# audeering/opensmile

Measured on AMD Instinct MI355X. Metric: MFCC frames/sec (16kHz, 25ms/10ms), higher is better.
Workload: dtype f32

## Files before the change

include/smilehip.h:

```cpp
#ifndef SMILEHIP_H
#define SMILEHIP_H

#include <stdint.h>

#ifdef __cplusplus
extern "C" {
#endif

#define SMILEHIP_VERSION 0x000100

typedef enum smilehip_status {
  SMILEHIP_OK = 0,
  SMILEHIP_ERR_INVALID = -1,
  SMILEHIP_ERR_NO_DEVICE = -2,
  SMILEHIP_ERR_HIP = -3,
  SMILEHIP_ERR_NOMEM = -4
} smilehip_status;

typedef enum smilehip_winfunc {
  SMILEHIP_WIN_RECT = 0, SMILEHIP_WIN_HANN = 1, SMILEHIP_WIN_HAMM = 2,
  SMILEHIP_WIN_GAUSS = 3, SMILEHIP_WIN_SINE = 4, SMILEHIP_WIN_TRI = 5,
  SMILEHIP_WIN_BARTLETT = 6, SMILEHIP_WIN_LANCZOS = 7
} smilehip_winfunc;

// ... 89 lines not shown
void smilehip_config_plp_0_d_a(smilehip_lld_config *c);
void smilehip_config_compare16_ab(smilehip_lld_config *c);
int smilehip_config_htk_variant(smilehip_lld_config *c, const char *name);
void smilehip_config_compare16_f0(smilehip_lld_config *c);
void smilehip_config_compare16(smilehip_lld_config *c);
void smilehip_config_is13_compare(smilehip_lld_config *c);

void smilehip_config_egemapsv02(smilehip_lld_config *c);
void smilehip_config_egemapsv01a(smilehip_lld_config *c);

int smilehip_specscale_frames(smilehip_plan *plan, const float *d_mag, int64_t ld_src, float *d_dst, int64_t ld_dst,
                              int64_t n_frames, void *stream);
int smilehip_pitchshs_frames(smilehip_plan *plan, const float *d_hps, int64_t ld_src, float *d_dst, int64_t ld_dst,
                             int64_t n_frames, void *stream);

int smilehip_batch_f0_taps(smilehip_batch *b, float *d_hps_dst, const float **d_shs, const float **d_e60);
int smilehip_batch_f0_pending(smilehip_batch *b, const int32_t **d_pending);

#define SMILEHIP_FUNC_MAX          (1u << 0)
#define SMILEHIP_FUNC_MIN          (1u << 1)
#define SMILEHIP_FUNC_RANGE        (1u << 2)
#define SMILEHIP_FUNC_MAXPOS       (1u << 3)
#define SMILEHIP_FUNC_MINPOS       (1u << 4)
#define SMILEHIP_FUNC_AMEAN        (1u << 5)
#define SMILEHIP_FUNC_MAXAMEANDIST (1u << 6)
#define SMILEHIP_FUNC_MINAMEANDIST (1u << 7)
#define SMILEHIP_FUNC_LINREGC1     (1u << 8)
#define SMILEHIP_FUNC_LINREGC2     (1u << 9)
#define SMILEHIP_FUNC_LINREGERRA   (1u << 10)
#define SMILEHIP_FUNC_LINREGERRQ   (1u << 11)
#define SMILEHIP_FUNC_VARIANCE     (1u << 12)
#define SMILEHIP_FUNC_STDDEV       (1u << 13)
#define SMILEHIP_FUNC_SKEWNESS     (1u << 14)
#define SMILEHIP_FUNC_KURTOSIS     (1u << 15)
#define SMILEHIP_FUNC_AMEAN_M      (1u << 16)
#define SMILEHIP_FUNC_ALL          0x1ffffu
uint32_t smilehip_functionals_is09_mask(void);
int smilehip_functionals_count(uint32_t mask);
int smilehip_batch_func_rows(const smilehip_batch *batch, int64_t *rows);
int smilehip_batch_functionals(smilehip_plan *plan, smilehip_batch *batch, const float *d_lld, int64_t ld_lld,
                               uint32_t mask, float *d_func, int64_t ld_func, void *stream);

int smilehip_functionals_matrix(smilehip_context *ctx, const float *d_x, int64_t ld_x, int64_t rows, int32_t cols,
                                uint32_t mask, float *d_out, void *stream);

enum {
  SMILEHIP_FAM_EXTREMES = 0, SMILEHIP_FAM_MEANS, SMILEHIP_FAM_MOMENTS, SMILEHIP_FAM_REGRESSION, SMILEHIP_FAM_PERCENTILES,
  SMILEHIP_FAM_TIMES, SMILEHIP_FAM_SEGMENTS, SMILEHIP_FAM_LPC, SMILEHIP_FAM_PEAKS2, SMILEHIP_FAM_ONSET, SMILEHIP_FAM_PEAKS, SMILEHIP_FAM_CROSSINGS, SMILEHIP_FAM_DCT,
  SMILEHIP_FAM_SAMPLES, SMILEHIP_FAM_MODULATION, SMILEHIP_FAM_COUNT
};
enum { SMILEHIP_NORM_SEGMENT = 0, SMILEHIP_NORM_SECOND = 1, SMILEHIP_NORM_FRAME = 2 };
enum { SMILEHIP_SEG_RELTH = 0, SMILEHIP_SEG_NONX = 1, SMILEHIP_SEG_EQX = 2, SMILEHIP_SEG_MRELTH = 3, SMILEHIP_SEG_ABSTH = 4,
       SMILEHIP_SEG_NARELTH = 5, SMILEHIP_SEG_NAMRELTH = 6, SMILEHIP_SEG_NAABSTH = 7, SMILEHIP_SEG_DELTA = 8,
       SMILEHIP_SEG_DELTA2 = 9, SMILEHIP_SEG_CHX = 10 };

typedef struct smilehip_func_spec {
  int32_t n_fam;
  int32_t fam[12];
  int32_t non_zero_functs;
  int32_t reserved0;
  double period;
  uint32_t ext_mask; int32_t ext_norm;
  uint32_t means_mask; int32_t means_norm;
  uint32_t mom_mask; int32_t mom_stddev_norm; int32_t mom_ratio_limit; int32_t reserved1;
  uint32_t reg_mask; int32_t reg_centroid_norm, reg_norm_coeff, reg_norm_inputs, reg_centroid_abs,
      reg_centroid_limit, reg_ratio_limit, reg_old_buggy_qerr;
  uint32_t pct_mask; int32_t pct_interp, n_pctl, n_range;
  double pctl[8]; int32_t range_a[8], range_b[8];
  uint32_t times_mask; int32_t times_norm, times_buggy_sec_norm, reserved2;
  uint32_t seg_mask; int32_t seg_norm, seg_algo, seg_max_num, seg_min_lng, seg_auto_min_lng, seg_pause_min_lng,
      seg_x_is_rel, seg_n_thresholds, seg_ravg_lng;
  float seg_x; float seg_thresholds[8]; float seg_range_rel_threshold;
  int32_t lpc_gain, lpc_coeffs, lpc_first, lpc_order;
  uint32_t pk_mask; int32_t pk_norm, pk_ratio_limit, pk_dyn_rel, pk_use_abs, reserved5;
  float pk_rel_thresh, pk_abs_thresh;
  uint32_t ons_mask; int32_t ons_norm, ons_use_abs, reserved6;
  float ons_thr_on, ons_thr_off;
  uint32_t pko_mask; int32_t pko_norm;
  uint32_t crs_mask; int32_t dct_first, dct_last, n_samples;
  double sample_pos[8];
  int32_t n_quot, quot_a[8], quot_b[8];
  int32_t n_ul, n_dl, reserved7;
  double ul[8], dl[8];
  int32_t mod_win_frames, mod_step_frames, mod_n_bins, mod_win_func, mod_remove_nz_mean, reserved8;
  double mod_min_freq, mod_max_freq;
} smilehip_func_spec;

int smilehip_funcspec_count(const smilehip_func_spec *spec);
int smilehip_funcspec_compare16(const char *instance, smilehip_func_spec *spec);
int smilehip_funcspec_is13_compare(const char *instance, smilehip_func_spec *spec);
int smilehip_funcspec_matrix(smilehip_context *ctx, const smilehip_func_spec *spec, const float *d_x, int64_t ld_x,
                             int64_t rows, int32_t cols, float *d_out, void *stream);
int smilehip_batch_funcspec(smilehip_plan *plan, smilehip_batch *batch, const smilehip_func_spec *spec,
                            const float *d_lld, int64_t ld_lld, int32_t col_first, int32_t n_cols, int32_t rows_cut,
                            const float *d_extra, int64_t ld_extra, float *d_func, int64_t ld_func, void *stream);

int smilehip_functionals_compare16_count(void);
int smilehip_batch_functionals_compare16(smilehip_plan *plan, smilehip_batch *batch, const float *d_lld, int64_t ld_lld,
                                         float *d_func, int64_t ld_func, void *stream);
int smilehip_batch_functionals_is13_compare(smilehip_plan *plan, smilehip_batch *batch, const float *d_lld, int64_t ld_lld,
                                            float *d_func, int64_t ld_func, void *stream);
int smilehip_batch_compare_b_extra(smilehip_batch *batch, const float **d_extra);

int smilehip_funcspec_egemaps(const char *instance, smilehip_func_spec *spec);
int smilehip_functionals_egemaps_count(void);
int smilehip_batch_functionals_egemaps(smilehip_plan *plan, smilehip_batch *batch, float *d_func, int64_t ld_func, void *stream);
int smilehip_batch_egemaps_taps(smilehip_batch *batch, const float **d_raw20, const float **d_lpc, const float **d_formants,
                                const float **d_pitch3, const float **d_jit4, const float **d_shim_db, const float **d_harm6,
                                const float **d_func_in, const int32_t **d_pending, int64_t *h_frame_off60);

int  smilehip_alloc(smilehip_context *ctx, uint64_t bytes, void **d_ptr);
int  smilehip_free(smilehip_context *ctx, void *d_ptr);
int  smilehip_copy_to_device(smilehip_context *ctx, void *d_dst, const void *h_src, uint64_t bytes, void *stream);
int  smilehip_copy_to_host(smilehip_context *ctx, void *h_dst, const void *d_src, uint64_t bytes, void *stream);
int  smilehip_stream_synchronize(smilehip_context *ctx, void *stream);
int  smilehip_alloc_cache(smilehip_context *ctx, uint64_t bytes);
int  smilehip_stream_create(smilehip_context *ctx, void **stream);
int  smilehip_stream_destroy(smilehip_context *ctx, void *stream);
int  smilehip_event_create(smilehip_context *ctx, void **event);
int  smilehip_event_destroy(smilehip_context *ctx, void *event);
int  smilehip_event_record(smilehip_context *ctx, void *event, void *stream);
int  smilehip_stream_wait_event(smilehip_context *ctx, void *stream, void *event);
int  smilehip_copy_to_device_2d(smilehip_context *ctx, void *d_dst, uint64_t d_pitch, const void *h_src, uint64_t h_pitch,
                                uint64_t width_bytes, uint64_t rows, void *stream);
int  smilehip_copy_to_host_2d(smilehip_context *ctx, void *h_dst, uint64_t h_pitch, const void *d_src, uint64_t d_pitch,
                              uint64_t width_bytes, uint64_t rows, void *stream);
int  smilehip_alloc_host(smilehip_context *ctx, uint64_t bytes, void **h_ptr);
int  smilehip_free_host(smilehip_context *ctx, void *h_ptr);
int  smilehip_host_register(smilehip_context *ctx, void *h_ptr, uint64_t bytes);
int  smilehip_host_unregister(smilehip_context *ctx, void *h_ptr);
int  smilehip_htk_rows_be(smilehip_context *ctx, const float *d_src, int64_t n, void *d_dst, void *stream);

void smilehip_config_mfcc12_0_d_a(smilehip_lld_config *c);

int  smilehip_plan_create(smilehip_context *ctx, const smilehip_lld_config *cfg, smilehip_plan **plan);
int  smilehip_plan_create_host_only(const smilehip_lld_config *cfg, smilehip_plan **plan);
void smilehip_plan_destroy(smilehip_plan *plan);
int  smilehip_plan_geometry(const smilehip_plan *plan, smilehip_geometry *g);
int64_t smilehip_num_frames(const smilehip_plan *plan, int64_t n_samples);
double  smilehip_frame_time(const smilehip_plan *plan, int64_t t);
double  smilehip_row_time(const smilehip_plan *plan, int64_t n_frames, int64_t row);
int64_t smilehip_plan_get_window(const smilehip_plan *plan, float *out, int64_t cap);
int64_t smilehip_plan_get_mel_weights(const smilehip_plan *plan, float *out, int64_t cap);
int64_t smilehip_plan_get_mel_chanmap(const smilehip_plan *plan, int32_t *out, int64_t cap);
int64_t smilehip_plan_get_dct(const smilehip_plan *plan, float *out, int64_t cap);
int64_t smilehip_plan_get_lifter(const smilehip_plan *plan, float *out, int64_t cap);

int  smilehip_batch_create(smilehip_plan *plan, const int64_t *h_sample_offsets, int32_t n_utt,
                           smilehip_batch **batch);
void smilehip_batch_destroy(smilehip_batch *batch);
int64_t smilehip_batch_total_frames(const smilehip_batch *batch);
int64_t smilehip_batch_total_rows(const smilehip_batch *batch);
int  smilehip_batch_delta_fused(const smilehip_batch *batch);
int  smilehip_batch_frame_offsets(const smilehip_batch *batch, int64_t *h_row_offsets);

int  smilehip_mfcc_run(smilehip_plan *plan, smilehip_batch *batch, const int16_t *d_pcm,
                       float *d_out, int64_t ld_out, void *stream);

int  smilehip_lld_run(smilehip_plan *plan, smilehip_batch *batch, const int16_t *d_pcm,
                      float *d_out, int64_t ld_out, void *stream);
int  smilehip_lld_run_f32(smilehip_plan *plan, smilehip_batch *batch, const float *d_pcm_f32,
                          float *d_out, int64_t ld_out, void *stream);
int  smilehip_lld_run_host(smilehip_plan *plan, smilehip_batch *batch, const int16_t *h_pcm,
                           int64_t n_samples, float *h_out);

int  smilehip_mfcc_run_host(smilehip_plan *plan, smilehip_batch *batch, const int16_t *h_pcm,
                            int64_t n_samples, float *h_out);

int  smilehip_plan_set_timing(smilehip_plan *plan, int enable);
int  smilehip_plan_last_timing(smilehip_plan *plan, float *ms_main, float *ms_delta);
int  smilehip_kernel_timing(int enable);
int64_t smilehip_kernel_timing_report(char *buf, int64_t buflen);


int smilehip_pcm16_to_float(smilehip_context *ctx, const int16_t *d_pcm, int64_t n, float *d_out, void *stream);
int smilehip_pcm_convert(smilehip_context *ctx, const void *d_raw, int n_bps, int n_bits, int n_chan, int mono_mixdown,
                         int64_t n, float *d_out, void *stream);
int smilehip_pcm_convert_float(smilehip_context *ctx, const float *d_raw, int n_chan, int mono_mixdown, int64_t n, float *d_out,
                               void *stream);
int smilehip_irfft_frames(smilehip_plan *plan, const float *d_src, int64_t ld_src, float *d_dst, int64_t ld_dst, int64_t n_frames,
                          void *stream);
#define SMILEHIP_MAGPHASE_MAGNITUDE 1
#define SMILEHIP_MAGPHASE_PHASE 2
#define SMILEHIP_MAGPHASE_NORMALISE 4
#define SMILEHIP_MAGPHASE_POWER 8
#define SMILEHIP_MAGPHASE_DBPSD 16
int smilehip_fftmagphase_frames(smilehip_context *ctx, const float *d_src, int64_t ld_src, int64_t nfft, int32_t flags, float dbp_norm,
                                float min_dbp, float *d_dst, int64_t ld_dst, int64_t n_frames, void *stream);
int smilehip_melspec_table_frames(smilehip_context *ctx, const float *d_src, int64_t ld_src, int64_t K, int32_t n_bands, int32_t dense,
                                  const float *d_coef, const int32_t *d_chanmap, int32_t n_lo, int32_t n_hi, int32_t use_power,
                                  float htk_scale, float *d_dst, int64_t ld_dst, int64_t n_frames, void *stream);
int smilehip_melspec_inverse_table_frames(smilehip_context *ctx, const float *d_src, int64_t ld_src, int32_t n_src, int64_t K,
                                          const float *d_coef, const int32_t *d_chanmap, int32_t n_lo, int32_t n_hi, int32_t use_power,
                                          float htk_div, float *d_dst, int64_t ld_dst, int64_t n_frames, void *stream);
int smilehip_pitchacf_zcr_frames(smilehip_context *ctx, const float *d_src, int64_t ld_src, int64_t n, int64_t n_frames, double fs_sec,
                                 double max_pitch, double *d_zcr, void *stream);
#define SMILEHIP_MZCR_ZCR 1
#define SMILEHIP_MZCR_MCR 2
#define SMILEHIP_MZCR_AMAX 4
#define SMILEHIP_MZCR_MAXMIN 8
#define SMILEHIP_MZCR_DC 16
int smilehip_mzcr_frames(smilehip_context *ctx, const float *d_src, int64_t ld_src, int64_t N, int64_t n_frames, int32_t flags,
                         float *d_dst, int64_t ld_dst, void *stream);
int smilehip_frame_rows(smilehip_context *ctx, const float *d_samples, int64_t frame_size, int64_t frame_step, int64_t n_frames,
                        float *d_dst, int64_t ld_dst, void *stream);
int smilehip_preemphasis_frames(smilehip_context *ctx, const float *d_src, int64_t ld_src, float *d_dst,
                                int64_t ld_dst, int64_t n_frames, int64_t N, float k, int de, void *stream);
int smilehip_window_frames(smilehip_plan *plan, const float *d_src, int64_t ld_src, float *d_dst,
                           int64_t ld_dst, int64_t n_frames, void *stream);
int smilehip_rfft_frames(smilehip_plan *plan, const float *d_src, int64_t ld_src, float *d_dst,
                         int64_t ld_dst, int64_t n_frames, void *stream);
int smilehip_fftmag_frames(smilehip_plan *plan, const float *d_src, int64_t ld_src, float *d_dst,
                           int64_t ld_dst, int64_t n_frames, void *stream);
int smilehip_melspec_frames(smilehip_plan *plan, const float *d_src, int64_t ld_src, float *d_dst,
                            int64_t ld_dst, int64_t n_frames, void *stream);
int smilehip_mfcc_frames(smilehip_plan *plan, const float *d_src, int64_t ld_src, float *d_dst,
                         int64_t ld_dst, int64_t n_frames, void *stream);
int  smilehip_mfcc_inverse_frames(smilehip_plan *plan, const float *d_src, int64_t ld_src, float *d_dst, int64_t ld_dst,
                                  int64_t n_frames, int do_log, void *stream);
int smilehip_sumsq_frames(smilehip_context *ctx, const float *d_src, int64_t ld_src, int64_t N, int64_t n_frames,
                          double *d_out, void *stream);
int smilehip_zcr_count_frames(smilehip_context *ctx, const float *d_src, int64_t ld_src, int64_t N, int64_t n_frames,
                              int32_t *d_out, void *stream);
int smilehip_acf_frames(smilehip_plan *plan, const float *d_src, int64_t ld_src, float *d_dst, int64_t ld_dst, int64_t n_out,
                        int64_t n_frames, int use_power, int cepstrum, int norm_output, int abs_cepstrum, void *stream);
int smilehip_pitchacf_frames(smilehip_context *ctx, const float *d_src, int64_t ld_src, int64_t n, int64_t n_frames,
                             double fs_sec, double max_pitch, double *d_voicing, int32_t *d_max_idx, void *stream);
int smilehip_pitchacf_contour_step(smilehip_context *ctx, const double *d_voicing, const int32_t *d_max_idx, double t_samp,
                                   double voicing_cutoff, float *d_state, float *d_out4, void *stream);
int smilehip_pitchacf_contour_frames(smilehip_context *ctx, const double *d_voicing, const int32_t *d_max_idx, double t_samp,
                                     double voicing_cutoff, float *d_state, float *d_out4, int64_t n_frames, void *stream);
int smilehip_spectral_frames(smilehip_plan *plan, const float *d_mag, int64_t ld_src, float *d_state, int first,
                             float *d_dst, int64_t ld_dst, int64_t n_frames, void *stream);
typedef struct smilehip_spectral_opts {
  int32_t n_bands;
  int32_t band_lo[16], band_hi[16];
  int32_t n_rolloff;
  double  rolloff[16];
  int32_t flux, centroid, max_pos, min_pos, entropy, variance, skewness, kurtosis, slope, sharpness, harmonicity;
  int32_t flatness, log_flatness;
  int32_t spec_diff, spec_pos_diff, flux_centroid, flux_at_flux_centroid, standard_deviation;
  int32_t n_slopes;
  int32_t slope_lo[16], slope_hi[16];
} smilehip_spectral_opts;
typedef struct smilehip_spectral_op smilehip_spectral_op;
int smilehip_spectral_opts_count(const smilehip_spectral_opts *opts);
int smilehip_spectral_op_create(smilehip_context *ctx, const smilehip_spectral_opts *opts, int64_t K, double frame_size_sec,
                                smilehip_spectral_op **op);
int smilehip_spectral_op_n_out(const smilehip_spectral_op *op);
int smilehip_spectral_op_frames(smilehip_spectral_op *op, const float *d_mag, int64_t ld_src, float *d_state, int first,
                                float *d_dst, int64_t ld_dst, int64_t n_frames, void *stream);
int smilehip_spectral_op_destroy(smilehip_spectral_op *op);
typedef struct smilehip_spectral_axis_opts {
  smilehip_spectral_opts base;
  int32_t square_input, use_log_spectrum, norm_band_energies, alpha_ratio, hammarberg_index, old_slope_scale, buggy_roll_off, tonality;
  double  spec_floor;
  int32_t freq_lo, freq_hi;
  int32_t frq_scale, reserved;
  double  frq_scale_param;
} smilehip_spectral_axis_opts;
typedef struct smilehip_spectral_axis_op smilehip_spectral_axis_op;
int smilehip_spectral_axis_opts_count(const smilehip_spectral_axis_opts *opts);
int smilehip_spectral_axis_tables(const smilehip_spectral_axis_opts *opts, int64_t K, double frame_size_sec, const double *frq,
                                  int64_t n_scale, int32_t *geo, double *edges, double *sums, double *sharp);
int smilehip_spectral_axis_op_create(smilehip_context *ctx, const smilehip_spectral_axis_opts *opts, int64_t K, double frame_size_sec,
                                     const double *frq, int64_t n_scale, smilehip_spectral_axis_op **op);
int smilehip_spectral_axis_op_n_out(const smilehip_spectral_axis_op *op);
int smilehip_spectral_axis_op_frames(smilehip_spectral_axis_op *op, const float *d_src, int64_t ld_src, float *d_state, int first,
                                     float *d_dst, int64_t ld_dst, int64_t n_frames, void *stream);
int smilehip_spectral_axis_op_destroy(smilehip_spectral_axis_op *op);
int smilehip_plp_audspec_frames(smilehip_context *ctx, const float *d_mel, int64_t ld_src, int n_bands, const float *d_eql,
                                float melfloor, float compression, int new_rasta, const float *rasta_coef, float *d_state,
                                float *d_dst, int64_t ld_dst, int64_t n_frames, void *stream);
int smilehip_plp_cc_frames(smilehip_context *ctx, const float *d_mel, int64_t ld_src, int n_bands, const float *d_eql,
                           float melfloor, float compression, int lp_order, const float *d_cos, const float *d_sin,
                           float *d_dst, int64_t ld_dst, int64_t n_frames, void *stream);
int smilehip_plp_stage_frames(smilehip_context *ctx, const float *d_mel, int64_t ld_src, int n_bands, const float *d_eql,
                              float melfloor, float compression, int lp_order, const float *d_cos, int out_stage,
                              float *d_dst, int64_t ld_dst, int64_t n_frames, void *stream);
int smilehip_window_op_row(smilehip_context *ctx, const float *d_x, float *d_y, int64_t n_t, int kind, int W, void *stream);
int smilehip_window_op_row_ex(smilehip_context *ctx, const float *d_x, float *d_y, int64_t n_t, int kind, int W, float *d_norm_io,
                              void *stream);
#define SMILEHIP_DELTA_RELATIVE 1
#define SMILEHIP_DELTA_HALFWAVE 2
#define SMILEHIP_DELTA_ABS 4
#define SMILEHIP_DELTA_SEGMENTS 8
int smilehip_delta_op_row(smilehip_context *ctx, const float *d_x, float *d_y, int64_t n_t, int W, int flags, float *d_norm_io,
                          void *stream);
int smilehip_window_op_block(smilehip_context *ctx, const float *d_x, int64_t ld_x, float *d_y, int64_t ld_y, int64_t n_t,
                             int32_t n_cols, int op, int W, int delta_flags, void *stream);
int smilehip_delta_segments_block(smilehip_context *ctx, const float *d_x, int64_t ld_x, float *d_y, int64_t ld_y, int64_t n_ticks,
                                  int32_t tick_frames, int32_t n_cols, int W, int delta_flags, float *d_norm_io, void *stream);
int smilehip_spectral_gemaps_frames(smilehip_plan *plan, const float *d_mag, int64_t ld_src, float *d_state, int first,
                                    float *d_dst, int64_t ld_dst, int64_t n_frames, void *stream);
int smilehip_specresample_frames(smilehip_plan *plan, const float *d_spec, int64_t ld_src, float *d_dst, int64_t ld_dst,
                                 int64_t n_frames, void *stream);
int smilehip_lpc_frames(smilehip_plan *plan, const float *d_x, int64_t ld_src, float *d_lpc, int64_t ld_dst, int64_t n_frames,
                        void *stream);
int smilehip_specresample_geometry(int64_t n_in, double fs_sec, double last_fs_sec, double base_period, double target_fs,
                                   int64_t *n_out, int64_t *k_max, double *nd);
int smilehip_specresample_tables(int64_t n_in, int64_t n_out, int64_t k_max, double nd, float *cos_table, float *sin_table);
int smilehip_specresample_table_frames(smilehip_context *ctx, const float *d_src, int64_t ld_src, int64_t n_in, int64_t n_out,
                                       int64_t k_max, const float *d_cos, const float *d_sin, float *d_dst, int64_t ld_dst,
                                       int64_t n_frames, void *stream);
int smilehip_lpc_acf_frames(smilehip_context *ctx, const float *d_x, int64_t ld_src, int64_t n, int32_t p, float *d_lpc,
                            int64_t ld_dst, int64_t n_frames, void *stream);
// ... 77 lines not shown
```

opensmile_amd/capi.py:

```python
import ctypes as C
import os

import numpy as np

HERE = os.path.dirname(os.path.abspath(__file__))
LIB_PATH = os.path.join(HERE, "libsmilehip.so")

WINFUNC = {"rec": 0, "rect": 0, "han": 1, "hann": 1, "ham": 2, "hamming": 2, "gau": 3,
           "gauss": 3, "sin": 4, "sine": 4, "tri": 5, "bar": 6, "bartlett": 6, "lac": 7}


class SmileHipError(RuntimeError):
    pass


class LldConfig(C.Structure):
    _fields_ = [
        ("struct_size", C.c_uint32),
        ("sample_rate", C.c_double), ("frame_size_sec", C.c_double), ("frame_step_sec", C.c_double),
        ("preemph", C.c_int32), ("preemph_k", C.c_float), ("preemph_de", C.c_int32),
        ("win_func", C.c_int32), ("win_sigma", C.c_double), ("win_gain", C.c_double),
        ("win_offset", C.c_double),
        ("zero_pad_symmetric", C.c_int32),
        ("n_bands", C.c_int32), ("lofreq", C.c_float), ("hifreq", C.c_float),
        ("use_power", C.c_int32), ("mel_htk_compatible", C.c_int32),
        ("first_mfcc", C.c_int32), ("last_mfcc", C.c_int32), ("cep_lifter", C.c_float),
        ("mfcc_htk_compatible", C.c_int32), ("melfloor", C.c_float),
        ("n_delta", C.c_int32), ("delta_win", C.c_int32),
        ("chain_kind", C.c_int32), ("plp_lp_order", C.c_int32), ("plp_compression", C.c_float), ("pitch_max", C.c_double), ("voicing_cutoff", C.c_double),
        ("sma_win", C.c_int32),
        ("force_frame_size", C.c_int64), ("force_fft_frame_size_sec", C.c_double),
        ("stage_mask", C.c_uint32),
        ("pitch_min", C.c_double), ("shs_n_harmonics", C.c_int32), ("shs_compression", C.c_float),
        ("f0_min_energy", C.c_float), ("append_log_energy", C.c_int32), ("cms", C.c_int32), ("jitter_broken_thresh", C.c_int32),
        ("vit_buffer_len", C.c_int32), ("jitter_search_range", C.c_double), ("formant_max_freq", C.c_double), ("specscale_min_f", C.c_double), ("shs_n_candidates", C.c_int32), ("shs_old_peak_algo", C.c_int32),
        ("spectral_band_lo", C.c_int32 * 2), ("spectral_band_hi", C.c_int32 * 2), ("specscale_off", C.c_int32),
    ]


STAGE_WINDOW, STAGE_FFT, STAGE_MEL, STAGE_MFCC, STAGE_ALL = 1, 2, 4, 8, 15


class FuncSpec(C.Structure):
    _fields_ = [
        ("n_fam", C.c_int32), ("fam", C.c_int32 * 12), ("non_zero_functs", C.c_int32), ("reserved0", C.c_int32),
        ("period", C.c_double),
        ("ext_mask", C.c_uint32), ("ext_norm", C.c_int32),
        ("means_mask", C.c_uint32), ("means_norm", C.c_int32),
        ("mom_mask", C.c_uint32), ("mom_stddev_norm", C.c_int32), ("mom_ratio_limit", C.c_int32), ("reserved1", C.c_int32),
        ("reg_mask", C.c_uint32), ("reg_centroid_norm", C.c_int32), ("reg_norm_coeff", C.c_int32),
        ("reg_norm_inputs", C.c_int32), ("reg_centroid_abs", C.c_int32), ("reg_centroid_limit", C.c_int32),
        ("reg_ratio_limit", C.c_int32), ("reg_old_buggy_qerr", C.c_int32),
        ("pct_mask", C.c_uint32), ("pct_interp", C.c_int32), ("n_pctl", C.c_int32), ("n_range", C.c_int32),
        ("pctl", C.c_double * 8), ("range_a", C.c_int32 * 8), ("range_b", C.c_int32 * 8),
        ("times_mask", C.c_uint32), ("times_norm", C.c_int32), ("times_buggy_sec_norm", C.c_int32), ("reserved2", C.c_int32),
        ("seg_mask", C.c_uint32), ("seg_norm", C.c_int32), ("seg_algo", C.c_int32), ("seg_max_num", C.c_int32),
        ("seg_min_lng", C.c_int32), ("seg_auto_min_lng", C.c_int32), ("seg_pause_min_lng", C.c_int32),
        ("seg_x_is_rel", C.c_int32), ("seg_n_thresholds", C.c_int32), ("seg_ravg_lng", C.c_int32),
        ("seg_x", C.c_float), ("seg_thresholds", C.c_float * 8), ("seg_range_rel_threshold", C.c_float),
        ("lpc_gain", C.c_int32), ("lpc_coeffs", C.c_int32), ("lpc_first", C.c_int32), ("lpc_order", C.c_int32),
        ("pk_mask", C.c_uint32), ("pk_norm", C.c_int32), ("pk_ratio_limit", C.c_int32), ("pk_dyn_rel", C.c_int32),
        ("pk_use_abs", C.c_int32), ("reserved5", C.c_int32),
        ("pk_rel_thresh", C.c_float), ("pk_abs_thresh", C.c_float),
        ("ons_mask", C.c_uint32), ("ons_norm", C.c_int32), ("ons_use_abs", C.c_int32), ("reserved6", C.c_int32),
        ("ons_thr_on", C.c_float), ("ons_thr_off", C.c_float),
        ("pko_mask", C.c_uint32), ("pko_norm", C.c_int32),
        ("crs_mask", C.c_uint32), ("dct_first", C.c_int32), ("dct_last", C.c_int32), ("n_samples", C.c_int32),
        ("sample_pos", C.c_double * 8),
        ("n_quot", C.c_int32), ("quot_a", C.c_int32 * 8), ("quot_b", C.c_int32 * 8),
        ("n_ul", C.c_int32), ("n_dl", C.c_int32), ("reserved7", C.c_int32),
        ("ul", C.c_double * 8), ("dl", C.c_double * 8),
        ("mod_win_frames", C.c_int32), ("mod_step_frames", C.c_int32), ("mod_n_bins", C.c_int32), ("mod_win_func", C.c_int32),
        ("mod_remove_nz_mean", C.c_int32), ("reserved8", C.c_int32),
        ("mod_min_freq", C.c_double), ("mod_max_freq", C.c_double),
    ]


class SpectralOpts(C.Structure):
    _fields_ = [("n_bands", C.c_int32), ("band_lo", C.c_int32 * 16), ("band_hi", C.c_int32 * 16), ("n_rolloff", C.c_int32),
                ("rolloff", C.c_double * 16)] + [(k, C.c_int32) for k in ("flux", "centroid", "max_pos", "min_pos", "entropy", "variance",
                                                                          "skewness", "kurtosis", "slope", "sharpness", "harmonicity", "flatness",
                                                                          "log_flatness", "spec_diff", "spec_pos_diff", "flux_centroid",
                                                                          "flux_at_flux_centroid", "standard_deviation", "n_slopes")] + [
                   ("slope_lo", C.c_int32 * 16), ("slope_hi", C.c_int32 * 16)]


def spectral_opts(bands, rolloff=(0.25, 0.5, 0.75, 0.9), slopes=(), **flags):
    o = SpectralOpts()
    o.n_slopes = len(slopes)
    for i, (a, b) in enumerate(slopes):
        o.slope_lo[i], o.slope_hi[i] = a, b
    o.n_bands = len(bands)
    for i, (a, b) in enumerate(bands):
        o.band_lo[i], o.band_hi[i] = a, b
    o.n_rolloff = len(rolloff)
    for i, r in enumerate(rolloff):
        o.rolloff[i] = r
    for k, v in flags.items():
        setattr(o, k, int(v))
    return o


class SpectralAxisOpts(C.Structure):
    _fields_ = [("base", SpectralOpts)] + [(k, C.c_int32) for k in ("square_input", "use_log_spectrum", "norm_band_energies", "alpha_ratio",
                                                                     "hammarberg_index", "old_slope_scale", "buggy_roll_off", "tonality")] + [
                   ("spec_floor", C.c_double), ("freq_lo", C.c_int32), ("freq_hi", C.c_int32), ("frq_scale", C.c_int32),
                   ("reserved", C.c_int32), ("frq_scale_param", C.c_double)]


def spectral_axis_opts(bands=(), rolloff=(), slopes=(), square_input=1, use_log_spectrum=0, norm_band_energies=0, alpha_ratio=0,
                       hammarberg_index=0, old_slope_scale=1, buggy_roll_off=0, tonality=0, spec_floor=0.0000001, freq_range=(0, 0),
                       frq_scale=0, frq_scale_param=0.0, **flags):
    o = SpectralAxisOpts()
    o.base = spectral_opts(bands, rolloff, slopes, **flags)
    o.square_input, o.use_log_spectrum, o.norm_band_energies = int(square_input), int(use_log_spectrum), int(norm_band_energies)
    o.alpha_ratio, o.hammarberg_index, o.old_slope_scale = int(alpha_ratio), int(hammarberg_index), int(old_slope_scale)
    o.buggy_roll_off, o.tonality, o.spec_floor = int(buggy_roll_off), int(tonality), float(spec_floor)
    o.freq_lo, o.freq_hi = int(freq_range[0]), int(freq_range[1])
    o.frq_scale = SPECSCALE[frq_scale] if isinstance(frq_scale, str) else int(frq_scale)
    o.frq_scale_param = float(frq_scale_param)
    return o


class SpecScaleOpts(C.Structure):
    _fields_ = [("scale", C.c_int32), ("param", C.c_double), ("min_f", C.c_double), ("max_f", C.c_double), ("n_points_target", C.c_int32),
                ("spec_enhance", C.c_int32), ("spec_smooth", C.c_int32), ("auditory_weighting", C.c_int32)]


SPECSCALE = {"lin": 0, "log": 1, "bark": 2, "mel": 3, "sem": 4, "bao": 7}


def specscale_opts(scale, param=0.0, min_f=25.0, max_f=-1.0, n_points_target=0, spec_enhance=0, spec_smooth=0, auditory_weighting=0):
    o = SpecScaleOpts()
    o.scale = SPECSCALE[scale] if isinstance(scale, str) else int(scale)
    o.param, o.min_f, o.max_f, o.n_points_target = float(param), float(min_f), float(max_f), int(n_points_target)
    o.spec_enhance, o.spec_smooth, o.auditory_weighting = int(spec_enhance), int(spec_smooth), int(auditory_weighting)
    return o


class Geometry(C.Structure):
    _fields_ = [("frame_size", C.c_int64), ("frame_step", C.c_int64), ("fft_size", C.c_int64),
                ("n_bins", C.c_int64), ("n_static", C.c_int32), ("n_out", C.c_int32),
                ("frame_period", C.c_double), ("fft_frame_size_sec", C.c_double)]


_vp, _i32, _i64, _f32, _dbl = C.c_void_p, C.c_int32, C.c_int64, C.c_float, C.c_double
SYMBOLS = {
    "smilehip_version": (C.c_int, []),
    "smilehip_last_error": (C.c_char_p, []),
    "smilehip_init": (C.c_int, [C.c_int, C.POINTER(_vp)]),
    "smilehip_shutdown": (None, [_vp]),
    "smilehip_device_name": (C.c_int, [_vp, C.c_char_p, C.c_int]),
    "smilehip_config_is09_lld": (None, [C.POINTER(LldConfig)]),
    "smilehip_config_compare16_ab": (None, [C.POINTER(LldConfig)]),
    "smilehip_config_compare16_f0": (None, [C.POINTER(LldConfig)]),
    "smilehip_config_htk_variant": (C.c_int, [C.POINTER(LldConfig), C.c_char_p]),
    "smilehip_config_compare16": (None, [C.POINTER(LldConfig)]),
    "smilehip_specscale_frames": (C.c_int, [_vp, _vp, _i64, _vp, _i64, _i64, _vp]),
    "smilehip_pitchshs_frames": (C.c_int, [_vp, _vp, _i64, _vp, _i64, _i64, _vp]),
    "smilehip_batch_f0_taps": (C.c_int, [_vp, _vp, C.POINTER(_vp), C.POINTER(_vp)]),
    "smilehip_config_plp_0_d_a": (None, [C.POINTER(LldConfig)]),
    "smilehip_batch_total_rows": (_i64, [_vp]),
    "smilehip_batch_delta_fused": (C.c_int, [_vp]),
    "smilehip_functionals_is09_mask": (C.c_uint32, []),
    "smilehip_functionals_count": (C.c_int, [C.c_uint32]),
    "smilehip_functionals_matrix": (C.c_int, [_vp, _vp, _i64, _i64, C.c_int32, C.c_uint32, _vp, _vp]),
    "smilehip_batch_func_rows": (C.c_int, [_vp, _vp]),
    "smilehip_batch_functionals": (C.c_int, [_vp, _vp, _vp, _i64, C.c_uint32, _vp, _i64, _vp]),
    "smilehip_functionals_compare16_count": (C.c_int, []),
    "smilehip_batch_functionals_compare16": (C.c_int, [_vp, _vp, _vp, _i64, _vp, _i64, _vp]),
    "smilehip_batch_compare_b_extra": (C.c_int, [_vp, _vp]),
    "smilehip_funcspec_count": (C.c_int, [_vp]),
    "smilehip_funcspec_compare16": (C.c_int, [C.c_char_p, _vp]),
    "smilehip_funcspec_is13_compare": (C.c_int, [C.c_char_p, _vp]),
    "smilehip_batch_functionals_is13_compare": (C.c_int, [_vp, _vp, _vp, _i64, _vp, _i64, _vp]),
    "smilehip_config_is13_compare": (None, [_vp]),
    "smilehip_config_egemapsv02": (None, [C.POINTER(LldConfig)]),
    "smilehip_config_egemapsv01a": (None, [C.POINTER(LldConfig)]),
    "smilehip_funcspec_egemaps": (C.c_int, [C.c_char_p, _vp]),
    "smilehip_functionals_egemaps_count": (C.c_int, []),
    "smilehip_batch_functionals_egemaps": (C.c_int, [_vp, _vp, _vp, _i64, _vp]),
    "smilehip_batch_egemaps_taps": (C.c_int, [_vp] + [C.POINTER(_vp)] * 9 + [_vp]),
    "smilehip_spectral_gemaps_frames": (C.c_int, [_vp, _vp, _i64, _vp, C.c_int, _vp, _i64, _i64, _vp]),
    "smilehip_specresample_frames": (C.c_int, [_vp, _vp, _i64, _vp, _i64, _i64, _vp]),
    "smilehip_lpc_frames": (C.c_int, [_vp, _vp, _i64, _vp, _i64, _i64, _vp]),
    "smilehip_formantlpc_frames": (C.c_int, [_vp, _vp, _i64, _vp, _i64, _i64, _vp]),
    "smilehip_formantlpc_rows": (C.c_int, [_vp, _vp, _i64, _vp, _i64, _i64, _vp, _i32, _vp]),
    "smilehip_harmonics_frames": (C.c_int, [_vp, _vp, _vp, _i64, _vp, _i64, _vp, _i64, _i64, _vp]),
    "smilehip_valbased_select_frames": (C.c_int, [_vp, _vp, _i64, _i64, _i64, _i32, _f32, _i32, _i32, _i32, _i32, _f32, _vp, _i64, _vp, _vp]),
    "smilehip_jitter_stream_create": (C.c_int, [_vp, _dbl, _i64, _i64, _dbl, _dbl, _i32, C.POINTER(_vp)]),
    "smilehip_jitter_stream_push": (C.c_int, [_vp, _f32, _vp, _i64, _i64, _vp, _vp, _vp]),
    "smilehip_jitter_stream_set_time_offset": (C.c_int, [_vp, _i64]),
    "smilehip_jitter_stream_destroy": (C.c_int, [_vp]),
    "smilehip_viterbi_stream_create": (C.c_int, [_vp, _i32, _f32, _vp, C.POINTER(_vp)]),
    "smilehip_viterbi_stream_push": (C.c_int, [_vp, _vp, _vp, _vp, _vp, _vp, _i32]),
    "smilehip_viterbi_stream_set_candidates": (C.c_int, [_vp, _i32]),
    "smilehip_viterbi_stream_flush": (C.c_int, [_vp, _vp, _vp, _vp, _i32]),
    "smilehip_viterbi_stream_destroy": (C.c_int, [_vp]),
    "smilehip_funcspec_matrix": (C.c_int, [_vp, _vp, _vp, _i64, _i64, C.c_int32, _vp, _vp]),
    "smilehip_batch_funcspec": (C.c_int, [_vp, _vp, _vp, _vp, _i64, C.c_int32, C.c_int32, C.c_int32, _vp, _i64, _vp, _i64, _vp]),
    "smilehip_lld_run": (C.c_int, [_vp, _vp, _vp, _vp, _i64, _vp]),
    "smilehip_lld_run_f32": (C.c_int, [_vp, _vp, _vp, _vp, _i64, _vp]),
    "smilehip_lld_run_host": (C.c_int, [_vp, _vp, _vp, _i64, _vp]),
    "smilehip_alloc": (C.c_int, [_vp, C.c_uint64, C.POINTER(_vp)]),
    "smilehip_free": (C.c_int, [_vp, _vp]),
    "smilehip_alloc_host": (C.c_int, [_vp, C.c_uint64, C.POINTER(_vp)]),
    "smilehip_free_host": (C.c_int, [_vp, _vp]),
    "smilehip_htk_rows_be": (C.c_int, [_vp, _vp, _i64, _vp, _vp]),
    "smilehip_copy_to_device": (C.c_int, [_vp, _vp, _vp, C.c_uint64, _vp]),
    "smilehip_copy_to_host": (C.c_int, [_vp, _vp, _vp, C.c_uint64, _vp]),
    "smilehip_alloc_cache": (C.c_int, [_vp, C.c_uint64]),
    "smilehip_stream_create": (C.c_int, [_vp, C.POINTER(_vp)]),
    "smilehip_stream_destroy": (C.c_int, [_vp, _vp]),
    "smilehip_event_create": (C.c_int, [_vp, C.POINTER(_vp)]),
    "smilehip_event_destroy": (C.c_int, [_vp, _vp]),
    "smilehip_event_record": (C.c_int, [_vp, _vp, _vp]),
    "smilehip_stream_wait_event": (C.c_int, [_vp, _vp, _vp]),
    "smilehip_kernel_timing": (C.c_int, [C.c_int]),
    "smilehip_kernel_timing_report": (C.c_int64, [_vp, _i64]),
    "smilehip_copy_to_device_2d": (C.c_int, [_vp, _vp, C.c_uint64, _vp, C.c_uint64, C.c_uint64, C.c_uint64, _vp]),
    "smilehip_copy_to_host_2d": (C.c_int, [_vp, _vp, C.c_uint64, _vp, C.c_uint64, C.c_uint64, C.c_uint64, _vp]),
    "smilehip_host_register": (C.c_int, [_vp, _vp, C.c_uint64]),
    "smilehip_host_unregister": (C.c_int, [_vp, _vp]),
    "smilehip_frame_rows": (C.c_int, [_vp, _vp, _i64, _i64, _i64, _vp, _i64, _vp]),
    "smilehip_window_op_block": (C.c_int, [_vp, _vp, _i64, _vp, _i64, _i64, _i32, C.c_int, C.c_int, C.c_int, _vp]),
    "smilehip_delta_segments_block": (C.c_int, [_vp, _vp, _i64, _vp, _i64, _i64, _i32, _i32, C.c_int, C.c_int, _vp, _vp]),
    "smilehip_pitchacf_contour_frames": (C.c_int, [_vp, _vp, _vp, _dbl, _dbl, _vp, _vp, _i64, _vp]),
    "smilehip_viterbi_stream_push_frames": (C.c_int, [_vp, _vp, _vp, _i64, _i32, _vp, _vp, _vp, _i32]),
    "smilehip_jitter_stream_push_frames": (C.c_int, [_vp, _vp, _i32, _vp, _i64, _i64, _vp, _vp, _vp]),
    "smilehip_stream_synchronize": (C.c_int, [_vp, _vp]),
    "smilehip_config_mfcc12_0_d_a": (None, [C.POINTER(LldConfig)]),
    "smilehip_plan_create": (C.c_int, [_vp, C.POINTER(LldConfig), C.POINTER(_vp)]),
    "smilehip_plan_create_host_only": (C.c_int, [C.POINTER(LldConfig), C.POINTER(_vp)]),
    "smilehip_plan_destroy": (None, [_vp]),
    "smilehip_plan_geometry": (C.c_int, [_vp, C.POINTER(Geometry)]),
    "smilehip_num_frames": (_i64, [_vp, _i64]),
    "smilehip_frame_time": (_dbl, [_vp, _i64]),
    "smilehip_row_time": (_dbl, [_vp, _i64, _i64]),
    "smilehip_plan_get_window": (_i64, [_vp, _vp, _i64]),
    "smilehip_plan_get_mel_weights": (_i64, [_vp, _vp, _i64]),
    "smilehip_plan_get_mel_chanmap": (_i64, [_vp, _vp, _i64]),
    "smilehip_plan_get_dct": (_i64, [_vp, _vp, _i64]),
    "smilehip_plan_get_lifter": (_i64, [_vp, _vp, _i64]),
    "smilehip_batch_f0_pending": (C.c_int, [_vp, _vp]),
    "smilehip_batch_create": (C.c_int, [_vp, _vp, _i32, C.POINTER(_vp)]),
    "smilehip_batch_destroy": (None, [_vp]),
    "smilehip_batch_total_frames": (_i64, [_vp]),
    "smilehip_batch_frame_offsets": (C.c_int, [_vp, _vp]),
    "smilehip_mfcc_run": (C.c_int, [_vp, _vp, _vp, _vp, _i64, _vp]),
    "smilehip_mfcc_run_host": (C.c_int, [_vp, _vp, _vp, _i64, _vp]),
    "smilehip_plan_set_timing": (C.c_int, [_vp, C.c_int]),
    "smilehip_plan_last_timing": (C.c_int, [_vp, C.POINTER(_f32), C.POINTER(_f32)]),
    "smilehip_sumsq_frames": (C.c_int, [_vp, _vp, _i64, _i64, _i64, _vp, _vp]),
    "smilehip_zcr_count_frames": (C.c_int, [_vp, _vp, _i64, _i64, _i64, _vp, _vp]),
    "smilehip_acf_frames": (C.c_int, [_vp, _vp, _i64, _vp, _i64, _i64, _i64, C.c_int, C.c_int, C.c_int, C.c_int, _vp]),
    "smilehip_pitchacf_frames": (C.c_int, [_vp, _vp, _i64, _i64, _i64, _dbl, _dbl, _vp, _vp, _vp]),
    "smilehip_pitchacf_contour_step": (C.c_int, [_vp, _vp, _vp, _dbl, _dbl, _vp, _vp, _vp]),
    "smilehip_spectral_frames": (C.c_int, [_vp, _vp, _i64, _vp, C.c_int, _vp, _i64, _i64, _vp]),
    "smilehip_spectral_opts_count": (C.c_int, [_vp]),
    "smilehip_spectral_op_create": (C.c_int, [_vp, _vp, _i64, C.c_double, _vp]),
    "smilehip_spectral_op_n_out": (C.c_int, [_vp]),
    "smilehip_spectral_op_frames": (C.c_int, [_vp, _vp, _i64, _vp, C.c_int, _vp, _i64, _i64, _vp]),
    "smilehip_spectral_op_destroy": (C.c_int, [_vp]),
    "smilehip_spectral_axis_opts_count": (C.c_int, [_vp]),
    "smilehip_spectral_axis_tables": (C.c_int, [_vp, _i64, C.c_double, _vp, _i64, _vp, _vp, _vp, _vp]),
    "smilehip_spectral_axis_op_create": (C.c_int, [_vp, _vp, _i64, C.c_double, _vp, _i64, _vp]),
    "smilehip_spectral_axis_op_n_out": (C.c_int, [_vp]),
    "smilehip_spectral_axis_op_frames": (C.c_int, [_vp, _vp, _i64, _vp, C.c_int, _vp, _i64, _i64, _vp]),
    "smilehip_spectral_axis_op_destroy": (C.c_int, [_vp]),
    "smilehip_plp_audspec_frames": (C.c_int, [_vp, _vp, _i64, C.c_int, _vp, C.c_float, C.c_float, C.c_int, _vp, _vp, _vp, _i64,
                                             _i64, _vp]),
    "smilehip_plp_cc_frames": (C.c_int, [_vp, _vp, _i64, C.c_int, _vp, C.c_float, C.c_float, C.c_int, _vp, _vp, _vp, _i64, _i64,
                                        _vp]),
    "smilehip_mfcc_inverse_frames": (C.c_int, [_vp, _vp, _i64, _vp, _i64, _i64, C.c_int, _vp]),
    "smilehip_plp_stage_frames": (C.c_int, [_vp, _vp, _i64, C.c_int, _vp, C.c_float, C.c_float, C.c_int, _vp, C.c_int, _vp, _i64, _i64,
                                           _vp]),
    "smilehip_window_op_row": (C.c_int, [_vp, _vp, _vp, _i64, C.c_int, C.c_int, _vp]),
    "smilehip_window_op_row_ex": (C.c_int, [_vp, _vp, _vp, _i64, C.c_int, C.c_int, _vp, _vp]),
    "smilehip_delta_op_row": (C.c_int, [_vp, _vp, _vp, _i64, C.c_int, C.c_int, _vp, _vp]),
    "smilehip_pcm_convert": (C.c_int, [_vp, _vp, C.c_int, C.c_int, C.c_int, C.c_int, _i64, _vp, _vp]),
    "smilehip_pcm_convert_float": (C.c_int, [_vp, _vp, C.c_int, C.c_int, _i64, _vp, _vp]),
    "smilehip_pcm16_to_float": (C.c_int, [_vp, _vp, _i64, _vp, _vp]),
    "smilehip_preemphasis_frames": (C.c_int, [_vp, _vp, _i64, _vp, _i64, _i64, _i64, _f32, C.c_int, _vp]),
    "smilehip_window_frames": (C.c_int, [_vp, _vp, _i64, _vp, _i64, _i64, _vp]),
    "smilehip_rfft_frames": (C.c_int, [_vp, _vp, _i64, _vp, _i64, _i64, _vp]),
    "smilehip_fftmag_frames": (C.c_int, [_vp, _vp, _i64, _vp, _i64, _i64, _vp]),
    "smilehip_irfft_frames": (C.c_int, [_vp, _vp, _i64, _vp, _i64, _i64, _vp]),
    "smilehip_fftmagphase_frames": (C.c_int, [_vp, _vp, _i64, _i64, _i32, _f32, _f32, _vp, _i64, _i64, _vp]),
    "smilehip_melspec_table_frames": (C.c_int, [_vp, _vp, _i64, _i64, _i32, _i32, _vp, _vp, _i32, _i32, _i32, _f32, _vp, _i64, _i64, _vp]),
    "smilehip_melspec_inverse_table_frames": (C.c_int, [_vp, _vp, _i64, _i32, _i64, _vp, _vp, _i32, _i32, _i32, _f32, _vp, _i64, _i64, _vp]),
    "smilehip_pitchacf_zcr_frames": (C.c_int, [_vp, _vp, _i64, _i64, _i64, _dbl, _dbl, _vp, _vp]),
    "smilehip_mzcr_frames": (C.c_int, [_vp, _vp, _i64, _i64, _i64, _i32, _vp, _i64, _vp]),
    "smilehip_melspec_frames": (C.c_int, [_vp, _vp, _i64, _vp, _i64, _i64, _vp]),
    "smilehip_mfcc_frames": (C.c_int, [_vp, _vp, _i64, _vp, _i64, _i64, _vp]),
    "smilehip_delta_chain": (C.c_int, [_vp, _vp, _vp, _i64, _i32, _i32, _i32, _vp]),
    "smilehip_specresample_geometry": (C.c_int, [_i64, _dbl, _dbl, _dbl, _dbl, _vp, _vp, _vp]),
    "smilehip_specresample_tables": (C.c_int, [_i64, _i64, _i64, _dbl, _vp, _vp]),
    "smilehip_specresample_table_frames": (C.c_int, [_vp, _vp, _i64, _i64, _i64, _i64, _vp, _vp, _vp, _i64, _i64, _vp]),
    "smilehip_lpc_acf_frames": (C.c_int, [_vp, _vp, _i64, _i64, _i32, _vp, _i64, _i64, _vp]),
    "smilehip_lsp_frames": (C.c_int, [_vp, _vp, _i64, _i32, _vp, _i64, _i64, _vp]),
    "smilehip_intensity_frames": (C.c_int, [_vp, _vp, _i64, _i64, _i32, _vp, _i64, _i64, _vp]),
    "smilehip_vecop_frames": (C.c_int, [_vp, _i32, _f32, _f32, _vp, _i64, _i32, _vp, _i64, _i64, _vp]),
    "smilehip_pitch_smoother_rows": (C.c_int, [_vp, _i32, _f32, _i32, _i32, _i32, _vp, _i64, _vp, _i32, _i64, _vp, _i32, _vp, _i64, _vp, _vp]),
    "smilehip_specscale_op_create": (C.c_int, [_vp, _vp, _i64, _dbl, _vp]),
    "smilehip_specscale_op_n_out": (C.c_int, [_vp]),
    "smilehip_specscale_op_frames": (C.c_int, [_vp, _vp, _i64, _vp, _i64, _i64, _vp]),
    "smilehip_specscale_op_destroy": (C.c_int, [_vp]),
    "smilehip_specscale_tables": (C.c_int, [_vp, _i64, _dbl, _vp, _vp, _vp, _vp]),
}

_lib = None


def load():
    global _lib
    if _lib is None:
# ... 170 lines not shown
    s = FuncSpec()
    _check(load().smilehip_funcspec_is13_compare(instance.encode(), C.byref(s)))
    return s


def compare16_f0_config():
    c = LldConfig()
    load().smilehip_config_compare16_f0(C.byref(c))
    return c


def funcspec_compare16(instance):
    s = FuncSpec()
    _check(load().smilehip_funcspec_compare16(instance.encode(), C.byref(s)))
    return s


def funcspec_count(spec):
    n = load().smilehip_funcspec_count(C.byref(spec))
    if n < 0:
        _check(n)
    return n


def funcspec_matrix_host(ctx, spec, x):
    L = load()
    x = np.ascontiguousarray(x, dtype=np.float32)
    rows, cols = x.shape
    per = funcspec_count(spec)
    out = np.zeros((cols, per), np.float32)
    d_x, d_out = _vp(), _vp()
    _check(L.smilehip_alloc(ctx._h, max(x.nbytes, 4), C.byref(d_x)))
    _check(L.smilehip_alloc(ctx._h, max(out.nbytes, 4), C.byref(d_out)))
    try:
        _check(L.smilehip_copy_to_device(ctx._h, d_x, x.ctypes.data, x.nbytes, None))
        _check(L.smilehip_funcspec_matrix(ctx._h, C.byref(spec), d_x, cols, rows, cols, d_out, None))
        _check(L.smilehip_stream_synchronize(ctx._h, None))
        _check(L.smilehip_copy_to_host(ctx._h, out.ctypes.data, d_out, out.nbytes, None))
    finally:
        L.smilehip_free(ctx._h, d_x)
        L.smilehip_free(ctx._h, d_out)
    return out


def is09_lld_config():
    c = LldConfig()
    load().smilehip_config_is09_lld(C.byref(c))
    return c


def mfcc12_0_d_a_config():
    c = LldConfig()
    load().smilehip_config_mfcc12_0_d_a(C.byref(c))
    return c


class Context:
    def __init__(self, device=0):
        self._h = _vp()
        _check(load().smilehip_init(device, C.byref(self._h)))

    def name(self):
        buf = C.create_string_buffer(256)
        _check(load().smilehip_device_name(self._h, buf, 256))
        return buf.value.decode()

    def close(self):
        if self._h:
            load().smilehip_shutdown(self._h)
            self._h = _vp()

    def __del__(self):
        try:
            self.close()
        except Exception:
            pass


class Plan:

    def __init__(self, ctx, cfg=None):
        self.ctx = ctx
        self.cfg = cfg if cfg is not None else mfcc12_0_d_a_config()
        self._h = _vp()
        if ctx is None:
            _check(load().smilehip_plan_create_host_only(C.byref(self.cfg), C.byref(self._h)))
        else:
            _check(load().smilehip_plan_create(ctx._h, C.byref(self.cfg), C.byref(self._h)))
        g = Geometry()
        _check(load().smilehip_plan_geometry(self._h, C.byref(g)))
        self.geometry = g

    def num_frames(self, n_samples):
        return int(load().smilehip_num_frames(self._h, n_samples))

    def frame_time(self, t):
        return float(load().smilehip_frame_time(self._h, t))

    def _table(self, fn, dtype):
        n = fn(self._h, None, 0)
        a = np.zeros(n, dtype)
        fn(self._h, a.ctypes.data, n)
        return a

    def window(self):
        return self._table(load().smilehip_plan_get_window, np.float32)

    def mel_weights(self):
        return self._table(load().smilehip_plan_get_mel_weights, np.float32)

    def mel_chanmap(self):
        return self._table(load().smilehip_plan_get_mel_chanmap, np.int32)

    def dct(self):
        g = self.geometry
        return self._table(load().smilehip_plan_get_dct, np.float32).reshape(g.n_static, self.cfg.n_bands)

    def lifter(self):
        return self._table(load().smilehip_plan_get_lifter, np.float32)

    def set_timing(self, on=True):
        _check(load().smilehip_plan_set_timing(self._h, 1 if on else 0))

    def last_timing(self):
        a, b = _f32(), _f32()
        _check(load().smilehip_plan_last_timing(self._h, C.byref(a), C.byref(b)))
        return a.value, b.value

    def close(self):
        if self._h:
            load().smilehip_plan_destroy(self._h)
            self._h = _vp()

    def __del__(self):
        try:
            self.close()
        except Exception:
            pass


class Batch:

    def __init__(self, plan, sample_offsets):
        self.plan = plan
        off = np.ascontiguousarray(sample_offsets, dtype=np.int64)
        assert off.ndim == 1 and len(off) >= 1
        self.n_utt = len(off) - 1
        self.sample_offsets = off
        self._h = _vp()
        _check(load().smilehip_batch_create(plan._h, off.ctypes.data, self.n_utt, C.byref(self._h)))
        self.total_frames = int(load().smilehip_batch_total_frames(self._h))
        self.total_rows = int(load().smilehip_batch_total_rows(self._h))
        self.delta_fused = bool(load().smilehip_batch_delta_fused(self._h))
        fo = np.zeros(self.n_utt + 1, np.int64)
        _check(load().smilehip_batch_frame_offsets(self._h, fo.ctypes.data))
        self.frame_offsets = fo

    def run_device(self, d_pcm_ptr, d_out_ptr, ld_out, stream=None):
        _check(load().smilehip_lld_run(self.plan._h, self._h, d_pcm_ptr, d_out_ptr, ld_out, stream))

    def run_device_f32(self, d_pcm_f32_ptr, d_out_ptr, ld_out, stream=None):
        _check(load().smilehip_lld_run_f32(self.plan._h, self._h, d_pcm_f32_ptr, d_out_ptr, ld_out, stream))

    def run_host(self, pcm):
        pcm = np.ascontiguousarray(pcm, dtype=np.int16)
        out = np.zeros((self.total_rows, self.plan.geometry.n_out), np.float32)
        _check(load().smilehip_lld_run_host(self.plan._h, self._h, pcm.ctypes.data, len(pcm),
                                            out.ctypes.data))
        return out

    def f0_run_host_taps(self, pcm):
        L = load()
        ctx = self.plan.ctx._h
        pcm = np.ascontiguousarray(pcm, dtype=np.int16)
        K = self.plan.geometry.n_bins
        nf = self.total_frames
        out = np.zeros((self.total_rows, self.plan.geometry.n_out), np.float32)
        taps = {"hps": np.zeros((nf, K), np.float32), "shs": np.zeros((nf, 21), np.float32), "e60": np.zeros((nf, 1), np.float32)}
        d_pcm, d_out, d_hps = _vp(), _vp(), _vp()
        _check(L.smilehip_alloc(ctx, max(pcm.nbytes, 4), C.byref(d_pcm)))
        _check(L.smilehip_alloc(ctx, max(out.nbytes, 4), C.byref(d_out)))
        _check(L.smilehip_alloc(ctx, max(taps["hps"].nbytes, 4), C.byref(d_hps)))
        try:
            if pcm.nbytes:
                _check(L.smilehip_copy_to_device(ctx, d_pcm, pcm.ctypes.data, pcm.nbytes, None))
            d_shs, d_e60 = _vp(), _vp()
            _check(L.smilehip_batch_f0_taps(self._h, d_hps, C.byref(d_shs), C.byref(d_e60)))
            _check(L.smilehip_lld_run(self.plan._h, self._h, d_pcm, d_out, self.plan.geometry.n_out, None))
            _check(L.smilehip_stream_synchronize(ctx, None))
            if out.nbytes:
                _check(L.smilehip_copy_to_host(ctx, out.ctypes.data, d_out, out.nbytes, None))
            if nf:
                _check(L.smilehip_copy_to_host(ctx, taps["hps"].ctypes.data, d_hps, taps["hps"].nbytes, None))
                _check(L.smilehip_copy_to_host(ctx, taps["shs"].ctypes.data, d_shs, taps["shs"].nbytes, None))
                _check(L.smilehip_copy_to_host(ctx, taps["e60"].ctypes.data, d_e60, taps["e60"].nbytes, None))
            _check(L.smilehip_batch_f0_taps(self._h, None, None, None))
        finally:
            L.smilehip_free(ctx, d_pcm)
            L.smilehip_free(ctx, d_out)
            L.smilehip_free(ctx, d_hps)
        return out, taps

    def func_rows(self):
        r = np.zeros(self.n_utt, np.int64)
        _check(load().smilehip_batch_func_rows(self._h, r.ctypes.data))
        return r

    def functionals_device(self, d_lld_ptr, ld_lld, d_func_ptr, ld_func, mask=None, stream=None):
        L = load()
        mask = L.smilehip_functionals_is09_mask() if mask is None else mask
        _check(L.smilehip_batch_functionals(self.plan._h, self._h, d_lld_ptr, ld_lld, mask, d_func_ptr, ld_func, stream))

    def functionals_host(self, lld, mask=None):
        L = load()
        mask = L.smilehip_functionals_is09_mask() if mask is None else mask
        per = L.smilehip_functionals_count(mask)
        n_out = self.plan.geometry.n_out
        lld = np.ascontiguousarray(lld, dtype=np.float32)
        assert lld.shape == (self.total_rows, n_out)
        out = np.zeros((self.n_utt, n_out * per), np.float32)
        ctx = self.plan.ctx._h
        d_lld, d_out = _vp(), _vp()
        _check(L.smilehip_alloc(ctx, max(lld.nbytes, 4), C.byref(d_lld)))
        _check(L.smilehip_alloc(ctx, max(out.nbytes, 4), C.byref(d_out)))
        try:
            if lld.nbytes:
                _check(L.smilehip_copy_to_device(ctx, d_lld, lld.ctypes.data, lld.nbytes, None))
            _check(L.smilehip_batch_functionals(self.plan._h, self._h, d_lld, n_out, mask, d_out, n_out * per, None))
            _check(L.smilehip_stream_synchronize(ctx, None))
            if out.nbytes:
                _check(L.smilehip_copy_to_host(ctx, out.ctypes.data, d_out, out.nbytes, None))
        finally:
            L.smilehip_free(ctx, d_lld)
            L.smilehip_free(ctx, d_out)
        return out

    def run_host_with_functionals16(self, pcm):
        L = load()
        pcm = np.ascontiguousarray(pcm, dtype=np.int16)
        n_out = self.plan.geometry.n_out
        nf = L.smilehip_functionals_compare16_count()
        lld = np.zeros((self.total_rows, n_out), np.float32)
        func = np.zeros((self.n_utt, nf), np.float32)
        ex = np.zeros((self.n_utt, 110), np.float32)
        ctx = self.plan.ctx._h
        d_pcm, d_lld, d_func = _vp(), _vp(), _vp()
        _check(L.smilehip_alloc(ctx, max(pcm.nbytes, 4), C.byref(d_pcm)))
        _check(L.smilehip_alloc(ctx, max(lld.nbytes, 4), C.byref(d_lld)))
        _check(L.smilehip_alloc(ctx, max(func.nbytes, 4), C.byref(d_func)))
        try:
            if pcm.nbytes:
                _check(L.smilehip_copy_to_device(ctx, d_pcm, pcm.ctypes.data, pcm.nbytes, None))
            _check(L.smilehip_lld_run(self.plan._h, self._h, d_pcm, d_lld, n_out, None))
            fn = L.smilehip_batch_functionals_is13_compare if self.plan.cfg.jitter_broken_thresh else L.smilehip_batch_functionals_compare16
            _check(fn(self.plan._h, self._h, d_lld, n_out, d_func, nf, None))
            _check(L.smilehip_stream_synchronize(ctx, None))
            if lld.nbytes:
                _check(L.smilehip_copy_to_host(ctx, lld.ctypes.data, d_lld, lld.nbytes, None))
            if func.nbytes:
                _check(L.smilehip_copy_to_host(ctx, func.ctypes.data, d_func, func.nbytes, None))
            d_ex = _vp()
            _check(L.smilehip_batch_compare_b_extra(self._h, C.byref(d_ex)))
            if ex.nbytes:
                _check(L.smilehip_copy_to_host(ctx, ex.ctypes.data, d_ex, ex.nbytes, None))
        finally:
            L.smilehip_free(ctx, d_pcm)
            L.smilehip_free(ctx, d_lld)
            L.smilehip_free(ctx, d_func)
        return lld, func, ex

    def run_host_egemaps(self, pcm, functionals=True, taps=False):
        L = load()
        pcm = np.ascontiguousarray(pcm, dtype=np.int16)
        n_out = self.plan.geometry.n_out
        lld = np.zeros((self.total_rows, n_out), np.float32)
        func = np.zeros((self.n_utt, 88), np.float32) if functionals else None
        ctx = self.plan.ctx._h
        d_pcm, d_lld, d_func = _vp(), _vp(), _vp()
        _check(L.smilehip_alloc(ctx, max(pcm.nbytes, 4), C.byref(d_pcm)))
        _check(L.smilehip_alloc(ctx, max(lld.nbytes, 4), C.byref(d_lld)))
        _check(L.smilehip_alloc(ctx, max(self.n_utt * 88 * 4, 4), C.byref(d_func)))
        out_taps = {}
        try:
            if pcm.nbytes:
                _check(L.smilehip_copy_to_device(ctx, d_pcm, pcm.ctypes.data, pcm.nbytes, None))
            _check(L.smilehip_lld_run(self.plan._h, self._h, d_pcm, d_lld, n_out, None))
            if functionals:
                _check(L.smilehip_batch_functionals_egemaps(self.plan._h, self._h, d_func, 88, None))
            _check(L.smilehip_stream_synchronize(ctx, None))
            if lld.nbytes:
                _check(L.smilehip_copy_to_host(ctx, lld.ctypes.data, d_lld, lld.nbytes, None))
            if functionals and func.nbytes:
                _check(L.smilehip_copy_to_host(ctx, func.ctypes.data, d_func, func.nbytes, None))
            if taps:
                ptrs = [_vp() for _ in range(9)]
                fo60 = np.zeros(self.n_utt + 1, np.int64)
                _check(L.smilehip_batch_egemaps_taps(self._h, *[C.byref(q) for q in ptrs], fo60.ctypes.data))
                nf, nf60 = self.total_frames, int(fo60[-1])
                T20 = np.diff(self.frame_offsets_frames())
                T60 = np.diff(fo60)
                nfin = int(np.where(T60 >= 1, T20 + 1, 0).sum())
                shapes = [("raw20", (nf, 12)), ("lpc", (nf, 12)), ("formants", (nf, 10)), ("pitch3", (nf60, 3)), ("jit4", (nf60, 4)),
                          ("shim_db", (nf60, 1)), ("harm6", (nf60, 6)), ("func_in", (nfin, 36))]
                for (name, shp), q in zip(shapes, ptrs):
                    a = np.zeros(shp, np.float32)
                    if a.nbytes:
# ... 179 lines not shown
```

opensmile_amd/csrc/batch_layout.hpp:

```cpp
#pragma once
#include <algorithm>
#include <cmath>
#include <cstdint>
#include <map>
#include <vector>

#include "../../include/smilehip.h"
#include "lld_tile_rec.hpp"

namespace smilehip {

struct BatchLayoutSpec {
  int chain_kind = SMILEHIP_CHAIN_MFCC;
  int64_t N = 0, H = 0;
  double period = 0.0;
  int row_extra = 0;
  bool fused_delta_eligible = false;
  int64_t fast_slots = 8;
  int64_t tile_frames = 0;
  int64_t dtile_rows = 0;
  int short_T = 0;
  int jitter_chunk = 0;
  int run_frames_override = 0;
};

struct BatchLayout {
  std::vector<int64_t> samp_off, frame_off, row_off;
  std::vector<int64_t> fin_off;
  std::vector<int32_t> short_utts;
  bool all_even = true;
  int64_t total_frames = 0, total_rows = 0;
  std::vector<int32_t> tile_utt, tile_t0, dtile_utt, dtile_t0;
  std::vector<TileRec> tile_rec;
  std::vector<int32_t> run_utt, run_t0;
  int32_t run_frames = 8;
  std::vector<FTileRec> ftiles;
  std::vector<int32_t> jit_utt, jit_t0;
  std::vector<int32_t> frame_utt;
};

constexpr int kRunFramesMin = 8;

inline int compare_run_frames(int64_t total_frames) {
  int L = kRunFramesMin;
  while (L < 64 && total_frames / (2 * L) >= 65536) L *= 2;
  return L;
}

inline int64_t layout_num_frames(int64_t len, int64_t N, int64_t H) { return len < N ? 0 : (len - N) / H + 1; }
inline int64_t samples_60ms(double period) { return std::lround(0.060 / period); }

inline int64_t layout_rows(const BatchLayoutSpec &s, int64_t len, int64_t T) {
  const bool compare = s.chain_kind == SMILEHIP_CHAIN_COMPARE_AB || s.chain_kind == SMILEHIP_CHAIN_COMPARE;
  if (!compare && s.chain_kind != SMILEHIP_CHAIN_EGEMAPS) return T > 0 ? T + s.row_extra : 0;
  const int64_t T60 = layout_num_frames(len, samples_60ms(s.period), s.H);
  return T60 >= (compare ? 4 : 1) ? T60 + 1 : 0;
}

inline void layout_fused_tiles(const BatchLayoutSpec &s, const int64_t *h_off, int32_t n_utt, BatchLayout &out) {
  const auto parts_of = [&](int64_t T, int64_t L) { return (T + L - 1) / L; };
  int64_t bestL = 32;
  double best = 1e300;
  std::map<int64_t, int64_t> hist;
  for (int32_t u = 0; u < n_utt; ++u) {
    const int64_t T = out.frame_off[u + 1] - out.frame_off[u];
    if (T > 0) hist[T]++;
  }
  for (int64_t L = 32; L <= 2048; L += 4) {
    int64_t n = 0;
    for (const auto &h : hist) n += h.second * ((h.first <= s.short_T) ? 1 : parts_of(h.first, L));
    const double cost = double((n + s.fast_slots - 1) / s.fast_slots) * double(L / 4 + 2);
    if (cost <= best) { best = cost; bestL = L; }
  }
  for (int32_t u = 0; u < n_utt; ++u) {
    const int64_t T = out.frame_off[u + 1] - out.frame_off[u];
    if (T <= 0) continue;
    const int64_t parts = (T <= s.short_T) ? 1 : parts_of(T, bestL);
    const int64_t len = (((T + parts - 1) / parts) + 3) & ~int64_t(3);
    for (int64_t t0 = 0; t0 < T; t0 += len) {
      const int64_t t1 = std::min<int64_t>(T, t0 + len), p0 = t0 > 0 ? t0 - 4 : 0;
      FTileRec r;
      r.samp0 = h_off[u] + p0 * s.H;
      r.row0 = out.frame_off[u] + p0;
      const int64_t last = (t1 + 3) & ~int64_t(3);
      r.n_frames = (int32_t)(last - p0 + 4);
      r.live_n = (int32_t)(T - p0);
      r.e0 = (int32_t)(t0 - p0);
      r.e1 = (int32_t)(t1 - p0);
      r.lo = (int32_t)(-p0);
      r.delta_on = T > s.short_T;
      out.ftiles.push_back(r);
    }
  }
  std::stable_sort(out.ftiles.begin(), out.ftiles.end(), [](const FTileRec &a, const FTileRec &c) { return a.n_frames > c.n_frames; });
}

inline int batch_layout(const BatchLayoutSpec &s, const int64_t *h_off, int32_t n_utt, BatchLayout &out) {
  out = BatchLayout();
  out.samp_off.assign(h_off, h_off + (n_utt ? n_utt + 1 : 0));
  if (n_utt == 0) out.samp_off.assign(1, 0);
  out.frame_off.assign(size_t(n_utt) + 1, 0);
  out.row_off.assign(size_t(n_utt) + 1, 0);
  const bool compare = s.chain_kind == SMILEHIP_CHAIN_COMPARE_AB || s.chain_kind == SMILEHIP_CHAIN_COMPARE;
  const bool egemaps = s.chain_kind == SMILEHIP_CHAIN_EGEMAPS;
  if (egemaps) out.fin_off.assign(size_t(n_utt) + 1, 0);
  {
    int64_t total_T = 0;
    for (int32_t u = 0; u < n_utt; ++u) total_T += layout_num_frames(h_off[u + 1] - h_off[u], s.N, s.H);
    out.run_frames = s.run_frames_override >= 1 ? s.run_frames_override : compare_run_frames(total_T);
  }
  for (int32_t u = 0; u < n_utt; ++u) {
    const int64_t len = h_off[u + 1] - h_off[u];
    if (len < 0) return u + 1;
    const int64_t T = layout_num_frames(len, s.N, s.H);
    const int64_t rows = layout_rows(s, len, T);
    if (compare || egemaps)
      for (int64_t t0 = 0; t0 < T; t0 += out.run_frames) {
        out.run_utt.push_back(u);
        out.run_t0.push_back((int32_t)t0);
      }
    if (egemaps) out.fin_off[u + 1] = out.fin_off[u] + (rows > 0 ? T + 1 : 0);
    out.frame_off[u + 1] = out.frame_off[u] + T;
    out.row_off[u + 1] = out.row_off[u] + rows;
    if (T > 0 && T <= s.short_T) out.short_utts.push_back(u);
    if (T > 0 && (h_off[u] & 1)) out.all_even = false;
    for (int64_t t0 = 0; t0 < T; t0 += s.tile_frames) {
      out.tile_utt.push_back(u);
      out.tile_t0.push_back((int32_t)t0);
      TileRec r;
      r.samp0 = h_off[u] + t0 * s.H;
      r.row0 = out.frame_off[u] + t0;
      r.n_frames = (int32_t)std::min<int64_t>(s.tile_frames, T - t0);
      r.pad = 0;
      out.tile_rec.push_back(r);
    }
    for (int64_t t0 = 0; t0 < rows; t0 += s.dtile_rows) {
      out.dtile_utt.push_back(u);
      out.dtile_t0.push_back((int32_t)t0);
    }
  }
  out.total_frames = out.frame_off[n_utt];
  out.total_rows = out.row_off[n_utt];
  if (s.chain_kind == SMILEHIP_CHAIN_IS09 && out.total_frames > 0) {
    out.frame_utt.resize((size_t)out.total_frames);
    for (int32_t u = 0; u < n_utt; ++u) std::fill(out.frame_utt.begin() + out.frame_off[u], out.frame_utt.begin() + out.frame_off[u + 1], u);
  }
  if (s.fused_delta_eligible && out.total_frames > 0 && out.all_even)
    layout_fused_tiles(s, h_off, n_utt, out);
  if (s.chain_kind == SMILEHIP_CHAIN_COMPARE_F0) {
    int64_t maxT = 0;
    for (int32_t u = 0; u < n_utt; ++u) maxT = std::max(maxT, out.frame_off[u + 1] - out.frame_off[u]);
    for (int64_t t0 = 0; t0 < maxT; t0 += s.jitter_chunk)
      for (int32_t u = 0; u < n_utt; ++u)
        if (t0 < out.frame_off[u + 1] - out.frame_off[u]) { out.jit_utt.push_back(u); out.jit_t0.push_back((int32_t)t0); }
  }
  return 0;
}

}
```

opensmile_amd/csrc/lld_launch.hpp:

```cpp
#pragma once
#include <hip/hip_runtime.h>

#include <vector>

#include "lld_params.hpp"
#include "tables.hpp"

namespace smilehip {
inline int current_device_cus() {
  static int cache[64] = {0};
  int dev = 0;
  if (hipGetDevice(&dev) != hipSuccess) return 0;
  if (dev >= 0 && dev < 64 && __atomic_load_n(&cache[dev], __ATOMIC_RELAXED) > 0) return __atomic_load_n(&cache[dev], __ATOMIC_RELAXED);
  int n = 0;
  if (hipDeviceGetAttribute(&n, hipDeviceAttributeMultiprocessorCount, dev) != hipSuccess) return 0;
  if (dev >= 0 && dev < 64) __atomic_store_n(&cache[dev], n, __ATOMIC_RELAXED);
  return n;
}

struct Fast512Host {
  std::vector<float2> tw256, tw512, win;
  std::vector<float4> melw;
  std::vector<uint32_t> melo;
  std::vector<float> dct28;
  std::vector<int32_t> lane_bands;
  int mel_units = 0, n_slots = 0, mp = 13;
  int mel_conflict_steps = 0;
  float mel_scale = 1.0f;
  int max_blocks = 512;
  bool force_padded = false;
};
bool fast512_applicable(int Nfft, int N);
int fast512_tile_frames();
int fast512_build_host(const smilehip_lld_config &cfg, const Geometry &geo, const std::vector<float> &window,
                       const MelBank &mel, const DctTables &dct, Fast512Host &h);
hipError_t launch_mfcc512(const LldParams &P, const Fast512Tables &F, const Fast512Host &h, bool aligned, bool fused_delta, hipStream_t s);
hipError_t launch_mfcc_generic(const LldParams &P, hipStream_t s);
hipError_t launch_chain(const ChainParams &P, hipStream_t s);
hipError_t launch_log_energy(const LldParams &P, const int32_t *d_tile_utt, const int32_t *d_tile_t0, int n_tiles, float *dst,
                             int64_t ld, int col, hipStream_t s);
hipError_t launch_cms(const int64_t *d_frame_off, int n_utt, const float *x, int64_t ld_x, float *out, int64_t ld_out, int n_cols,
                      hipStream_t s);
hipError_t launch_compare(const LldParams &P, const CompareParams &Q, int n_runs, const int64_t *d_row_off,
                          int64_t total_rows, float *d_out, int64_t ld_out, int de_col, hipStream_t s);
hipError_t launch_compare_b_extra(const int64_t *d_frame_off, const int64_t *d_row_off, int n_utt, const float *rawB, float *out110,
                                  hipStream_t s);
struct F0Pipe {
  hipStream_t spec = nullptr, sweep = nullptr;
  hipEvent_t start = nullptr, spec_done[2] = {nullptr, nullptr}, sweep_done[2] = {nullptr, nullptr}, cand_done[2] = {nullptr, nullptr};
  double *ab2 = nullptr;
};
hipError_t launch_f0(const LldParams &P, const F0Params &Q, int max_blocks, float *d_out, int64_t ld_out, hipStream_t s,
                     hipEvent_t frames_done = nullptr, const F0Pipe *pipe = nullptr);
int f0_chunk_tiles();
int f0_tile_frames();
hipError_t launch_f0_viterbi_steps(const F0Params &Q, const float *d_frames, int *d_st, double *d_dstate, int *d_paths, int *d_decided,
                                   int n_steps, hipStream_t s);
hipError_t launch_f0_viterbi_step(const F0Params &Q, const float *d_frames, int *d_st, double *d_dstate, int *d_paths, int *d_decided,
                                  int flush, hipStream_t s);
int f0_viterbi_max_buffer();
int f0_viterbi_states();
int64_t f0_scratch_rows(int64_t n_tiles);
int64_t f0_scratch_doubles(int64_t n_tiles, int K);
hipError_t launch_f0_rows(const F0Params &Q, int max_blocks, hipStream_t s);
hipError_t launch_f0_lld(const LldParams &P, const F0Params &Q, const int64_t *d_row_off, const float *d_pitch2, float *d_jit4,
                         float *d_out, int64_t ld_out, int col_sma, int col_de, hipStream_t s);
hipError_t launch_is09(const LldParams &P, const Is09Params &Q, hipStream_t s);
hipError_t launch_pitch_contour_frames(const double *d_voicing, const int32_t *d_max_idx, double Tsamp, double cutoff, float *d_state,
                                       float *d_out4, int64_t n_frames, hipStream_t s);
hipError_t launch_pitch_contour_step(const double *d_voicing, const int32_t *d_max_idx, double Tsamp, double cutoff, float *d_state,
                                     float *d_out4, hipStream_t s);
hipError_t launch_funcspec(const FsParams &P, int n_utt, const int *fam_off, const int *fam_want, hipStream_t s);
hipError_t launch_gemaps_frames(const LldParams &P, const GemapsParams &G, int n_runs, hipStream_t s);
hipError_t launch_gemaps_harm(const LldParams &P, const F0Params &Q, const GemapsParams &G, int max_blocks, hipStream_t s);
hipError_t launch_gemaps_tail(const int64_t *d_frame_off20, const int64_t *d_row_off, int n_utt, const GemapsParams &G, float *d_out,
                              int64_t ld_out, hipStream_t s);
hipError_t launch_gemaps_spectral_rows(const float *src, int64_t lds, float *state, bool first, float *dst, int64_t ldd, int64_t nF,
                                       int K, const GemapsParams &G, hipStream_t s);
hipError_t launch_gemaps_lpc_rows(const GemapsParams &G, hipStream_t s);
hipError_t launch_gemaps_formant_rows(const GemapsParams &G, hipStream_t s);
hipError_t launch_gemaps_dbp(float *d_x, int64_t ld, int n_utt, const int64_t *d_row_off, hipStream_t s);
int jitter_wave_capacity(double Tw, int64_t N, double min_pitch, double search_range);
int jitter_chunk_frames();
hipError_t launch_f0_jitter(const LldParams &P, const F0Params &Q, const float *d_f0, int64_t ld_f0, float *d_jit4, hipStream_t s);
int fs_sort_lds_rows();
int chain_tile_rows();
int chain_short_max();
}
```

opensmile_amd/csrc/lld_mfcc512.hip:

```cpp
#include <hip/hip_runtime.h>
#include "kernel_timing.hpp"
#include "phase_timing.hpp"

#include <algorithm>
#include <cmath>
#include <cstdio>
#include <cstdlib>
#include <cstring>
#include <type_traits>
#include <vector>

#include "lld_device.hpp"
#include "lld_launch.hpp"
#include "lld_params.hpp"
#include "tables.hpp"

namespace smilehip {

namespace {

constexpr int kWavesPerBlock = 8;
constexpr int kTileFrames = 32;
constexpr int kTB2Row = 65;
constexpr int kTB2Floats = 2 * (15 * kTB2Row + 3 * 16 + 16);
constexpr int kLmelFloats = 68;
constexpr int kOctetFloats = 12;
constexpr int kPbFloats = 448;
constexpr int kWaveFloats = 2080;

static_assert(kWaveFloats >= kTB2Floats && kWaveFloats >= 4 * (kLmelFloats + kPbFloats) && kWaveFloats % 4 == 0, "per-wave LDS region");
static_assert(kPbFloats % 64 == 0 && kPbFloats >= 33 * kOctetFloats, "power buffer");
static_assert(kLmelFloats >= 64 && kLmelFloats % 4 == 0 && (kLmelFloats / 4) % 2 == 1,
              "band vectors: room for the PLP vectors at +32 and +48, 16-byte aligned, neighbouring groups on different bank quads");

constexpr float C1 = 0.92387953251128673848f;
constexpr float S1 = 0.38268343236508978178f;
constexpr float R2 = 0.70710678118654752440f;

__device__ __forceinline__ void wave_lds_fence() {
  __builtin_amdgcn_fence(__ATOMIC_ACQ_REL, "wavefront");
  __builtin_amdgcn_wave_barrier();
}

__host__ __device__ constexpr int pb_pos(int k) { return k + (kOctetFloats - 8) * (k >> 3); }

__device__ __forceinline__ void dft4(float &r0, float &i0, float &r1, float &i1, float &r2, float &i2,
                                     float &r3, float &i3) {
  const float t0r = r0 + r2, t0i = i0 + i2;
  const float t1r = r0 - r2, t1i = i0 - i2;
  const float t2r = r1 + r3, t2i = i1 + i3;
  const float t3r = r1 - r3, t3i = i1 - i3;
  r0 = t0r + t2r; i0 = t0i + t2i;
  r2 = t0r - t2r; i2 = t0i - t2i;
  r1 = t1r + t3i; i1 = t1i - t3r;
  r3 = t1r - t3i; i3 = t1i + t3r;
}

__device__ __forceinline__ void cmul(float &r, float &i, float c, float s) {
  const float nr = fmaf(r, c, -i * s);
  const float ni = fmaf(r, s, i * c);
  r = nr; i = ni;
}
__device__ __forceinline__ void cmul_ns(float &r, float &i, float c, float s, float ns) {
  const float nr = fmaf(r, c, i * ns);
  const float ni = fmaf(r, s, i * c);
  r = nr; i = ni;
}

struct Dft16K {
  float c1, s1, r2, nc1, ns1, nr2;
  __device__ __forceinline__ Dft16K() : c1(C1), s1(S1), r2(R2), nc1(-C1), ns1(-S1), nr2(-R2) {
    asm volatile("" : "+s"(c1), "+s"(s1), "+s"(r2), "+s"(nc1), "+s"(ns1), "+s"(nr2));
  }
};

__device__ __forceinline__ void dft16_first(float (&re)[16], float (&im)[16], int m0) {
  dft4(re[m0], im[m0], re[m0 + 4], im[m0 + 4], re[m0 + 8], im[m0 + 8], re[m0 + 12], im[m0 + 12]);
}
__device__ __forceinline__ void dft16_twiddles(float (&re)[16], float (&im)[16], const Dft16K &K) {
  cmul_ns(re[1 + 4], im[1 + 4], K.c1, K.ns1, K.s1);
  { const float a = re[1 + 8], b = im[1 + 8]; re[1 + 8] = K.r2 * (a + b); im[1 + 8] = K.r2 * (b - a); }
  cmul_ns(re[1 + 12], im[1 + 12], K.s1, K.nc1, K.c1);
  { const float a = re[2 + 4], b = im[2 + 4]; re[2 + 4] = K.r2 * (a + b); im[2 + 4] = K.r2 * (b - a); }
  { const float a = re[2 + 8], b = im[2 + 8]; re[2 + 8] = b; im[2 + 8] = -a; }
  { const float a = re[2 + 12], b = im[2 + 12]; re[2 + 12] = K.r2 * (b - a); im[2 + 12] = K.nr2 * (a + b); }
  cmul_ns(re[3 + 4], im[3 + 4], K.s1, K.nc1, K.c1);
  { const float a = re[3 + 8], b = im[3 + 8]; re[3 + 8] = K.r2 * (b - a); im[3 + 8] = K.nr2 * (a + b); }
  cmul_ns(re[3 + 12], im[3 + 12], K.nc1, K.s1, K.ns1);
}
__device__ __forceinline__ void dft16_last(float (&re)[16], float (&im)[16], int q) {
  dft4(re[4 * q], im[4 * q], re[4 * q + 1], im[4 * q + 1], re[4 * q + 2], im[4 * q + 2], re[4 * q + 3], im[4 * q + 3]);
}
__device__ __forceinline__ void dft16_rename(float (&re)[16], float (&im)[16]) {
  float tr[16], ti[16];
#pragma unroll
  for (int q = 0; q < 4; ++q)
#pragma unroll
    for (int p = 0; p < 4; ++p) { tr[q + 4 * p] = re[4 * q + p]; ti[q + 4 * p] = im[4 * q + p]; }
#pragma unroll
  for (int k = 0; k < 16; ++k) { re[k] = tr[k]; im[k] = ti[k]; }
}
__device__ __forceinline__ void dft16(float (&re)[16], float (&im)[16], const Dft16K &K) {
#pragma unroll
  for (int m0 = 0; m0 < 4; ++m0) dft16_first(re, im, m0);
  dft16_twiddles(re, im, K);
#pragma unroll
  for (int q = 0; q < 4; ++q) dft16_last(re, im, q);
  dft16_rename(re, im);
}

template <int CTRL>
__device__ __forceinline__ float dpp_f(float v) {
  return __int_as_float(__builtin_amdgcn_update_dpp(0, __float_as_int(v), CTRL, 0xf, 0xf, true));
}

}

template <int MP, bool PLP, bool DELTA>
constexpr bool typed_loads() {
  return !PLP && !(MP == 16 && DELTA);
}
typedef float float2v __attribute__((ext_vector_type(2)));
__device__ float2v tbuffer_load_xy(__amdgpu_buffer_rsrc_t rsrc, int voffset, int soffset, int format, int aux)
    __asm("llvm.amdgcn.raw.ptr.tbuffer.load.v2f32");
__device__ float tbuffer_load_x(__amdgpu_buffer_rsrc_t rsrc, int voffset, int soffset, int format, int aux)
    __asm("llvm.amdgcn.raw.ptr.tbuffer.load.f32");
constexpr int kFmt16x2Sscaled = 5 | (3 << 4);
constexpr int kFmt16Sscaled = 2 | (3 << 4);
constexpr int kRsrcWord3 = 0x00020000, kRsrcWord3Typed = 0x00020000 | 4 | (5 << 3);

template <int MP, bool ALIGNED, bool TYPED>
struct FrameRegs {
  uint32_t v[ALIGNED && !TYPED ? MP : 2 * MP];
};

template <int MP, bool ALIGNED, bool TYPED>
__device__ __forceinline__ void pcm_prefetch(const int16_t *pcm, int64_t pcm_total, int64_t base, int H, int lane,
                                             FrameRegs<MP, ALIGNED, TYPED> &R) {
  const int64_t b0 = base < 0 ? 0 : base;
  int64_t left = (pcm_total - b0) * 2;
  left = left < 0 ? 0 : (left > 0xfffffffcLL ? 0xfffffffcLL : left);
  const __amdgpu_buffer_rsrc_t rsrc = __builtin_amdgcn_make_buffer_rsrc(const_cast<int16_t *>(pcm + b0), 0, (int)(uint32_t)left,
                                                                        TYPED ? kRsrcWord3Typed : kRsrcWord3);
  uint32_t lo = ((uint32_t)(lane >> 4) * (uint32_t)H + 2u * (uint32_t)(lane & 15)) * 2u + (uint32_t)((base - b0) * 2);
  asm volatile("" : "+v"(lo));
#pragma unroll
  for (int m = 0; m < MP; ++m) {
    if constexpr (TYPED && ALIGNED) {
      const float2v f = tbuffer_load_xy(rsrc, (int)lo + 64 * m, 0, kFmt16x2Sscaled, 0);
      R.v[2 * m] = __float_as_uint(f.x);
      R.v[2 * m + 1] = __float_as_uint(f.y);
    } else if constexpr (TYPED) {
      R.v[2 * m] = __float_as_uint(tbuffer_load_x(rsrc, (int)lo + 64 * m, 0, kFmt16Sscaled, 0));
      R.v[2 * m + 1] = __float_as_uint(tbuffer_load_x(rsrc, (int)lo + 64 * m + 2, 0, kFmt16Sscaled, 0));
    } else if constexpr (ALIGNED) {
      R.v[m] = (uint32_t)__builtin_amdgcn_raw_buffer_load_b32(rsrc, (int)lo + 64 * m, 0, 0);
    } else {
      R.v[2 * m] = (uint32_t)(int32_t)(int16_t)__builtin_amdgcn_raw_buffer_load_b16(rsrc, (int)lo + 64 * m, 0, 0);
      R.v[2 * m + 1] = (uint32_t)(int32_t)(int16_t)__builtin_amdgcn_raw_buffer_load_b16(rsrc, (int)lo + 64 * m + 2, 0, 0);
    }
  }
}

SMILEHIP_PHASE_COUNTERS(g_phase, 16, smilehip_debug_phase)

template <int MP, bool PREEMPH, bool USE_POWER, bool ALIGNED, bool PLP, int UC, bool DELTA, bool PAD0>
__device__ __forceinline__ void lld_mfcc512_body(const LldParams &P, const Fast512Tables &F) {
  extern __shared__ __attribute__((aligned(16))) float smem[];
  const int lane = threadIdx.x & 63;
  const int wave = __builtin_amdgcn_readfirstlane(threadIdx.x >> 6);
  const int g = lane >> 4;
  const int j = lane & 15;

  float2 *s_tw512 = reinterpret_cast<float2 *>(smem);
  float2 *s_win = s_tw512 + 256;
  float2 *s_tw256 = s_win + MP * 16;
  float4 *s_melw0 = reinterpret_cast<float4 *>(s_tw256 + 256);
  float4 *s_melw1 = s_melw0 + UC * 16;
  float *s_dct = reinterpret_cast<float *>(s_melw1 + UC * 16);
  float *s_plp = s_dct + 16 * 28;
  constexpr int shared_floats = 256 * 2 + MP * 16 * 2 + 256 * 2 + UC * 16 * 8 + 16 * 28 + 48;
  float *wbase = smem + shared_floats + wave * kWaveFloats;
  float *s_lmel = wbase + g * kLmelFloats;
  float *s_cep = s_lmel + 48;
  float *s_pb = wbase + 4 * kLmelFloats + g * kPbFloats;

  for (int i = threadIdx.x; i < 256; i += blockDim.x) { s_tw512[i] = F.tw512[i]; s_tw256[i] = F.tw256[i]; }
  for (int i = threadIdx.x; i < MP * 16; i += blockDim.x) s_win[i] = F.win[i];
  for (int i = threadIdx.x; i < UC * 16; i += blockDim.x) { s_melw0[i] = F.melw[2 * i]; s_melw1[i] = F.melw[2 * i + 1]; }
  for (int i = threadIdx.x; i < 16 * 28; i += blockDim.x) s_dct[i] = F.dct28[i];
  if (PLP) {
    for (int i = threadIdx.x; i < 32; i += blockDim.x) s_plp[i] = F.plp_eql[i];
    for (int i = threadIdx.x; i < 16; i += blockDim.x) s_plp[32 + i] = F.plp_sin[i];
  }
  __syncthreads();

  uint32_t mo[UC];
#pragma unroll
  for (int i = 0; i < UC; ++i) mo[i] = F.melo[i * 16 + j];
  const uint32_t lane_bands = (uint32_t)F.lane_bands[j];
  const int band0 = (int)((lane_bands >> 8) & 0xffu), band1 = (int)((lane_bands >> 16) & 0xffu);
  float uf0[UC], uf1[UC];
#pragma unroll
  for (int i = 0; i < UC; ++i) { uf0[i] = ((lane_bands >> i) & 1u) ? 1.0f : 0.0f; uf1[i] = 1.0f - uf0[i]; }
  const uint32_t out_off = (uint32_t)(g * (int)P.ld_out + j) * 4u;
  const uint32_t out_off_d = out_off + (uint32_t)P.n_mfcc * 4u;
  const uint32_t out_off_dd = out_off + (uint32_t)P.n_mfcc * 8u;
  const float nkpre = P.de ? P.k : -P.k;
  const int m0 = P.pad_left >> 5, j0 = (P.pad_left >> 1) & 15;
  float *pb_k = s_pb + pb_pos(j);
  float *pb_m = s_pb + pb_pos(256 - j);

  const Dft16K dk;
  PhaseTimer<12> PH;
  const int tile_stride = __builtin_amdgcn_readfirstlane((int)gridDim.x) * kWavesPerBlock;
  int tile = blockIdx.x * kWavesPerBlock + wave;
  const int n_tiles = DELTA ? P.n_ftiles : P.n_tiles;
  if (tile >= n_tiles) return;
  typedef typename std::conditional<DELTA, FTileRec, TileRec>::type Rec;
  typedef const __attribute__((address_space(4))) Rec *ConstRecPtr;
  const ConstRecPtr recs = DELTA ? (ConstRecPtr)(uintptr_t)P.ftile_rec : (ConstRecPtr)(uintptr_t)P.tile_rec;
  int64_t cur_samp0 = recs[tile].samp0, cur_row0 = recs[tile].row0;
  int cur_n = recs[tile].n_frames;
  int cur_live = 0, cur_e0 = 0, cur_e1 = 0, cur_lo = 0, cur_don = 0;
  if constexpr (DELTA) {
    cur_live = recs[tile].live_n; cur_e0 = recs[tile].e0; cur_e1 = recs[tile].e1; cur_lo = recs[tile].lo; cur_don = recs[tile].delta_on;
  }
  bool has_next = tile + tile_stride < n_tiles;
  int64_t nxt_samp0 = cur_samp0;
  if (has_next) nxt_samp0 = recs[tile + tile_stride].samp0;
  int tp = 0;
  constexpr bool TYPED = typed_loads<MP, PLP, DELTA>();
  FrameRegs<MP, ALIGNED, TYPED> R;
  pcm_prefetch<MP, ALIGNED, TYPED>(P.pcm, P.pcm_total, cur_samp0 - P.pad_left, P.H, lane, R);
  unsigned char *pend_row = nullptr;
  float pend_val = 0.0f;
  bool pend_live = false;
  float s_prev = 0.0f, d_cur = 0.0f;
  int b_tp = 0, b_lo = 0, b_live = 0, b_e0 = 0, b_e1 = 0, b_don = 0;
  const auto from_group = [&](int grp, float v) {
    return __int_as_float(__builtin_amdgcn_ds_bpermute(4 * ((grp << 4) | j), __float_as_int(v)));
  };
  const auto regress = [](float vm2, float vm1, float vp1, float vp2) {
    float num = 0.0f;
    num += 1.0f * (vp1 - vm1);
    num += 2.0f * (vp2 - vm2);
    return num;
  };
  const auto div10 = [](float a, bool &plain) {
    const float y = 0.1f, b = 10.0f;
    plain |= div_needs_division(a);
    return div_markstein(a, b, y);
  };
  const auto delta_fast = [&](float s_cur, float dp, float &dn, float &ddn, float &drow, bool &plain) {
    const float s1 = from_group((g + 1) & 3, g == 0 ? s_cur : s_prev);
    const float s3 = from_group((g + 3) & 3, g == 3 ? s_prev : s_cur);
    dn = div10(regress(s_prev, s1, s3, s_cur), plain);
    const float d1 = from_group((g + 1) & 3, g == 0 ? dn : dp);
    const float d3 = from_group((g + 3) & 3, g == 3 ? dp : dn);
    ddn = div10(regress(dp, d1, d3, dn), plain);
    drow = from_group((g + 2) & 3, g >= 2 ? dp : dn);
  };
  const auto delta_exact = [&](float s_cur, float dp, int btp, int lo, int live_n, float &dn, float &ddn, float &drow) {
    const auto fetch = [&](int x, int hi_c, int base, float cur, float prev) {
      x = x < lo ? lo : (x > hi_c ? hi_c : x);
      const int dd = x - base;
      const float c = from_group(dd & 3, cur), p = from_group(dd & 3, prev);
      return dd >= 0 ? c : p;
    };
    const float norm = 10.0f;
    const int fd = btp - 2 + g, fdd = btp - 4 + g, hi0 = live_n - 1, hi1 = live_n + 1;
    dn = regress(fetch(fd - 2, hi0, btp, s_cur, s_prev), fetch(fd - 1, hi0, btp, s_cur, s_prev), fetch(fd + 1, hi0, btp, s_cur, s_prev),
                 fetch(fd + 2, hi0, btp, s_cur, s_prev)) / norm;
    ddn = regress(fetch(fdd - 2, hi1, btp - 2, dn, dp), fetch(fdd - 1, hi1, btp - 2, dn, dp), fetch(fdd + 1, hi1, btp - 2, dn, dp),
                  fetch(fdd + 2, hi1, btp - 2, dn, dp)) / norm;
    drow = from_group((g + 2) & 3, g >= 2 ? dp : dn);
  };

  for (;;) {
    const bool live = tp + g < (DELTA ? cur_live : cur_n);
    PH(0);
    if constexpr (!DELTA) {
      if (pend_row != nullptr && pend_live) {
        uint32_t oo = out_off;
        asm volatile("" : "+v"(oo));
        *reinterpret_cast<float *>(pend_row + oo) = pend_val;
      }
    }
    float st_dn = 0.0f, st_ddn = 0.0f, st_drow = 0.0f;
    bool st_plain = false;
    if constexpr (DELTA) delta_fast(pend_val, d_cur, st_dn, st_ddn, st_drow, st_plain);
    float re[16], im[16];
    {
      float tprev = 0.0f;
      (void)tprev;
#pragma unroll
      for (int m = 0; m < 16; ++m) {
        if (m < MP) {
          float a, b;
          if constexpr (TYPED) {
            a = __uint_as_float(R.v[2 * m]);
            b = __uint_as_float(R.v[2 * m + 1]);
          } else if constexpr (ALIGNED) {
            a = (float)(int16_t)(R.v[m] & 0xffffu);
            b = (float)(int16_t)(R.v[m] >> 16);
          } else {
            a = (float)(int32_t)R.v[2 * m];
            b = (float)(int32_t)R.v[2 * m + 1];
          }
          float ya = a, yb = b;
          if (PREEMPH) {
            const float t = dpp_f<0x121>(b);
            const float pa = (j == 0) ? tprev : t;
            tprev = t;
            yb = fmaf(nkpre, a, b);
            ya = fmaf(nkpre, pa, a);
            if (PAD0 ? (m == 0 && j == 0) : (m == m0 && j == j0)) ya = P.one_minus_k * a;
          }
          const float2 w = s_win[m * 16 + j];
          re[m] = ya * w.x;
          im[m] = yb * w.y;
        } else {
          re[m] = 0.0f; im[m] = 0.0f;
        }
      }
    }
    PH(1);
    if constexpr (DELTA) {
      const bool clamped = !(b_tp - 6 >= b_lo && b_tp + 3 <= b_live - 1);
      if (clamped || __builtin_amdgcn_ballot_w64(st_plain && j < P.n_mfcc) != 0) delta_exact(pend_val, d_cur, b_tp, b_lo, b_live, st_dn, st_ddn, st_drow);
      const int fdd = b_tp - 4 + g;
      const bool row_live = pend_row != nullptr && j < P.n_mfcc && fdd >= b_e0 && fdd < b_e1;
      if (row_live) {
        uint32_t oo = out_off;
        asm volatile("" : "+v"(oo));
        *reinterpret_cast<float *>(pend_row + oo) = s_prev;
      }
      if (row_live && b_don) {
        uint32_t oo = out_off_d;
        asm volatile("" : "+v"(oo));
        *reinterpret_cast<float *>(pend_row + oo) = st_drow;
        oo = out_off_dd;
        asm volatile("" : "+v"(oo));
        *reinterpret_cast<float *>(pend_row + oo) = st_ddn;
      }
      s_prev = pend_val;
      d_cur = st_dn;
    }

    float2 *tbw = reinterpret_cast<float2 *>(wbase) + g * 16 + j;
    const float2 *tbr = reinterpret_cast<const float2 *>(wbase) + g * 16 + j * kTB2Row;
    {
      float2 w[4], wn[4];
#pragma unroll
      for (int p = 1; p < 4; ++p) w[p] = s_tw256[(4 * p) * 16 + j];
      w[0] = make_float2(1.0f, 0.0f);
#pragma unroll
      for (int m0 = 0; m0 < 4; ++m0) dft16_first(re, im, m0);
      dft16_twiddles(re, im, dk);
#pragma unroll
      for (int q = 0; q < 4; ++q) {
        if (q < 3) {
#pragma unroll
          for (int p = 0; p < 4; ++p) wn[p] = s_tw256[(q + 1 + 4 * p) * 16 + j];
        }
        dft16_last(re, im, q);
#pragma unroll
        for (int p = 0; p < 4; ++p) {
          const int k1 = q + 4 * p;
          if (k1 > 0) cmul(re[4 * q + p], im[4 * q + p], w[p].x, w[p].y);
          tbw[k1 * kTB2Row] = make_float2(re[4 * q + p], im[4 * q + p]);
        }
#pragma unroll
        for (int p = 0; p < 4; ++p) w[p] = wn[p];
      }
    }
    PH(3);
    {
      wave_lds_fence();
#pragma unroll
      for (int jj = 0; jj < 16; ++jj) {
        typedef const volatile __attribute__((address_space(3))) unsigned long long *LdsU64;
        const unsigned long long v = ((LdsU64)tbr)[jj];
        re[jj] = __int_as_float((int)(uint32_t)v); im[jj] = __int_as_float((int)(uint32_t)(v >> 32));
      }
      wave_lds_fence();
    }
    PH(4);
    dft16(re, im, dk);
    PH(5);

    float zr[8], zi[8];
#pragma unroll
    for (int q = 0; q < 8; ++q) {
      const float pr = q > 0 ? dpp_f<0x12f>(re[(16 - q) & 15]) : re[15];
      const float pi = q > 0 ? dpp_f<0x12f>(im[(16 - q) & 15]) : im[15];
      const float tr = __int_as_float(__builtin_amdgcn_update_dpp(__float_as_int(pr), __float_as_int(re[15 - q]), 0x101, 0xf, 0xf, false));
      const float ti = __int_as_float(__builtin_amdgcn_update_dpp(__float_as_int(pi), __float_as_int(im[15 - q]), 0x101, 0xf, 0xf, false));
      zr[q] = dpp_f<0x140>(tr);
      zi[q] = dpp_f<0x140>(ti);
    }
    float2 tw5[8];
#pragma unroll
    for (int q = 0; q < 8; ++q) tw5[q] = s_tw512[j + 16 * q];
#pragma unroll
    for (int q = 0; q < 8; ++q) {
      const float2 w = tw5[q];
      const float a = re[q], b = im[q];
      const float c = zr[q], d = zi[q];
      const float sr = a + c, si = b - d, dr = a - c, di = b + d;
      const float ur = fmaf(w.x, dr, -w.y * di);
      const float ui = fmaf(w.x, di, w.y * dr);
      const float xr = sr + ui, xi = si - ur;
      const float yr = sr - ui, yi = si + ur;
      float pk = fmaf(xi, xi, xr * xr);
      float pm = fmaf(yi, yi, yr * yr);
      if (q == 0 && j == 0) {
        const float v0 = 2.0f * (a + b), v1 = 2.0f * (a - b);
        pk = v0 * v0; pm = v1 * v1;
      }
      if (!USE_POWER) { pk = sqrtf(pk); pm = sqrtf(pm); }
      pb_k[(2 * kOctetFloats) * q] = pk;
      pb_m[-(2 * kOctetFloats) * q] = pm;
    }
    if (j == 0) {
      const float a = re[8], b = im[8];
      const float s = 4.0f * fmaf(b, b, a * a);
      s_pb[pb_pos(128)] = USE_POWER ? s : sqrtf(s);
    } else if (j < 8) {
      s_pb[pb_pos(256) + j] = 0.0f;
    }
    wave_lds_fence();

    PH(6);
    int ntp = tp + 4;
    const bool advance = ntp >= cur_n;
    const bool more = !advance || has_next;
    if (advance) ntp = 0;
    if (more)
      pcm_prefetch<MP, ALIGNED, TYPED>(P.pcm, P.pcm_total, (advance ? nxt_samp0 : cur_samp0) + (int64_t)ntp * P.H - P.pad_left, P.H, lane, R);
    else if constexpr (TYPED) {
#pragma unroll
      for (int m = 0; m < 2 * MP; ++m) R.v[m] = 0u;
    }

    PH(7);
    {
      float a0 = 0.0f, a1 = 0.0f;
#pragma unroll
      for (int i = 0; i < UC; ++i) {
        const float4 *pp = reinterpret_cast<const float4 *>(reinterpret_cast<const unsigned char *>(s_pb) + mo[i]);
        const float4 p0 = pp[0], p1 = pp[1];
        const float4 w0 = s_melw0[i * 16 + j], w1 = s_melw1[i * 16 + j];
        float acc = p0.x * w0.x;
        acc = fmaf(p0.y, w0.y, acc); acc = fmaf(p0.z, w0.z, acc); acc = fmaf(p0.w, w0.w, acc);
        acc = fmaf(p1.x, w1.x, acc); acc = fmaf(p1.y, w1.y, acc); acc = fmaf(p1.z, w1.z, acc); acc = fmaf(p1.w, w1.w, acc);
        a0 = fmaf(acc, uf0[i], a0);
        a1 = fmaf(acc, uf1[i], a1);
      }
      PH(8);
#pragma unroll
      for (int h = 0; h < 2; ++h) {
        const int b = h ? band1 : band0;
        const float acc = h ? a1 : a0;
        if (b != 0xff) {
          if (PLP) {
            float v = acc * F.mel_scale;
            v = v < P.melfloor ? P.melfloor : v;
            s_lmel[b] = __expf(P.plp_compression * __logf(v * s_plp[b]));
          } else {
            s_lmel[b] = log_mel_fast(acc * F.mel_scale, P.melfloor, P.log_floor);
          }
        }
      }
      if (j + 16 >= P.n_bands) s_lmel[j + 16] = 0.0f;
      if (j >= P.n_bands) s_lmel[j] = 0.0f;
    }
    wave_lds_fence();

    PH(9);
    if (PLP) {
      float *s_acf = s_lmel + 32;
      if (j <= P.plp_order) s_acf[j] = plp_acf_lag(s_lmel, s_dct + j * 28, P.n_bands);
      wave_lds_fence();
      if (j == 0) plp_cc_serial(s_acf, P.plp_order, s_plp + 32, s_cep);
      wave_lds_fence();
      if (j < P.n_mfcc) pend_val = s_cep[j];
    } else
    if (j < P.n_mfcc) {
      const float4 *row_c = reinterpret_cast<const float4 *>(s_dct + j * 28);
      const float4 *lm = reinterpret_cast<const float4 *>(s_lmel);
      float acc = 0.0f, dgain = 0.0f;
#pragma unroll
      for (int q = 0; q < 7; ++q) {
        const float4 l = lm[q], c = row_c[q];
        acc = fmaf(l.x, c.x, acc); acc = fmaf(l.y, c.y, acc); acc = fmaf(l.z, c.z, acc);
        if (q < 6) acc = fmaf(l.w, c.w, acc); else dgain = c.w;
      }
      pend_val = acc * dgain;
    }
    pend_live = live && j < P.n_mfcc;
    pend_row = reinterpret_cast<unsigned char *>(P.out + (cur_row0 + tp - (DELTA ? 4 : 0)) * P.ld_out);
    if constexpr (DELTA) { b_tp = tp; b_lo = cur_lo; b_live = cur_live; b_e0 = cur_e0; b_e1 = cur_e1; b_don = cur_don; }
    wave_lds_fence();
    PH(10);
    if (!more) break;
    if (advance) {
      tile += tile_stride;
      cur_samp0 = nxt_samp0; cur_row0 = recs[tile].row0; cur_n = recs[tile].n_frames;
      if constexpr (DELTA) {
        cur_live = recs[tile].live_n; cur_e0 = recs[tile].e0; cur_e1 = recs[tile].e1; cur_lo = recs[tile].lo; cur_don = recs[tile].delta_on;
      }
      has_next = tile + tile_stride < n_tiles;
      if (has_next) nxt_samp0 = recs[tile + tile_stride].samp0;
    }
    tp = ntp;
  }
  if constexpr (DELTA) {
    float dn, ddn, drow;
    delta_exact(pend_val, d_cur, b_tp, b_lo, b_live, dn, ddn, drow);
    const int fdd = b_tp - 4 + g;
    if (j < P.n_mfcc && fdd >= b_e0 && fdd < b_e1) {
      *reinterpret_cast<float *>(pend_row + out_off) = s_prev;
      if (b_don) {
        *reinterpret_cast<float *>(pend_row + out_off_d) = drow;
        *reinterpret_cast<float *>(pend_row + out_off_dd) = ddn;
      }
    }
  } else if (pend_live) {
    uint32_t oo = out_off;
    asm volatile("" : "+v"(oo));
    *reinterpret_cast<float *>(pend_row + oo) = pend_val;
  }
  PH.flush(g_phase);
}

template <int MP, bool PREEMPH, bool USE_POWER, bool ALIGNED, bool PLP, int UC, bool DELTA = false>
__global__ void __launch_bounds__(kWavesPerBlock * 64, 4) lld_mfcc512(LldParams P, Fast512Tables F) {
  lld_mfcc512_body<MP, PREEMPH, USE_POWER, ALIGNED, PLP, UC, DELTA, true>(P, F);
}
template <int MP, bool PREEMPH, bool USE_POWER, bool ALIGNED, bool PLP, int UC, bool DELTA = false>
__global__ void __launch_bounds__(kWavesPerBlock * 64, 4) lld_mfcc512_padded(LldParams P, Fast512Tables F) {
  lld_mfcc512_body<MP, PREEMPH, USE_POWER, ALIGNED, PLP, UC, DELTA, false>(P, F);
}

bool fast512_applicable(int Nfft, int N) { return Nfft == 512 && N <= 512 && N >= 2; }

int fast512_tile_frames() { return kTileFrames; }

int fast512_build_host(const smilehip_lld_config &cfg, const Geometry &geo, const std::vector<float> &window,
                       const MelBank &mel, const DctTables &dct, Fast512Host &h) {
  const int pad_left = cfg.zero_pad_symmetric ? (int)((geo.Nfft - geo.N) / 2) : 0;
  const int H = (int)geo.H, N = (int)geo.N;
  if (mel.n_bands > 27 || dct.n_mfcc > 16 || cfg.win_offset != 0.0 || (pad_left & 1) || (H & 1) || H < 2) return -1;
  h.mp = (pad_left + N) <= 13 * 32 ? 13 : 16;
  const char *fp = getenv("SMILEHIP_MFCC512_FORCE_PADDED");
  h.force_padded = fp != nullptr && fp[0] == '1';
  h.tw256.resize(256);
  for (int k1 = 0; k1 < 16; ++k1)
    for (int j = 0; j < 16; ++j) {
      const double a = -2.0 * M_PI * double(j * k1) / 256.0;
      h.tw256[k1 * 16 + j] = make_float2(float(cos(a)), float(sin(a)));
    }
  h.tw512.resize(256);
  for (int k = 0; k < 256; ++k) {
    const double a = -2.0 * M_PI * double(k) / 512.0;
    h.tw512[k] = make_float2(float(cos(a)), float(sin(a)));
  }
  h.win.assign(size_t(h.mp) * 16, make_float2(0.f, 0.f));
  for (int m = 0; m < h.mp; ++m)
    for (int j = 0; j < 16; ++j) {
      const int n = 2 * (j + 16 * m) - pad_left;
      float a = 0.f, b = 0.f;
      if (n >= 0 && n < N) a = float(double(window[n]) / 32767.0);
      if (n + 1 >= 0 && n + 1 < N) b = float(double(window[n + 1]) / 32767.0);
      h.win[size_t(m) * 16 + j] = make_float2(a, b);
    }
  struct Unit { int octet; float w[8]; };
  std::vector<Unit> units;
  const int nb = mel.n_bands;
  std::vector<int> first_unit(nb + 1, 0);
  for (int b = 0; b < nb; ++b) {
    int lo = -1, hi = -1;
    if (mel.rise_hi[b] > mel.rise_lo[b]) { lo = mel.rise_lo[b]; hi = mel.rise_hi[b]; }
    if (mel.fall_hi[b] > mel.fall_lo[b]) { if (lo < 0) lo = mel.fall_lo[b]; hi = mel.fall_hi[b]; }
    first_unit[b] = int(units.size());
    if (lo >= 0) {
      for (int o = lo / 8; o <= (hi - 1) / 8; ++o) {
        Unit un;
        un.octet = o;
        for (int e = 0; e < 8; ++e) {
          const int n = 8 * o + e;
          float w = 0.0f;
          if (n >= mel.rise_lo[b] && n < mel.rise_hi[b]) w = 1.0f - mel.coef[n];
          else if (n >= mel.fall_lo[b] && n < mel.fall_hi[b]) w = mel.coef[n];
          un.w[e] = w;
        }
        units.push_back(un);
      }
    }
  }
  first_unit[nb] = int(units.size());
  h.n_slots = int(units.size());
  std::vector<int> size(nb), order(nb);
  for (int b = 0; b < nb; ++b) { size[b] = first_unit[b + 1] - first_unit[b]; order[b] = b; }
  std::stable_sort(order.begin(), order.end(), [&](int x, int y) { return size[x] > size[y]; });
  int cap = 0;
  std::vector<std::pair<int, int>> lanes;
  for (int c : {6, 8}) {
    lanes.clear();
    std::vector<char> used(nb, 0);
    bool ok = true;
    for (int oi = 0; oi < nb && ok; ++oi) {
      const int a = order[oi];
      if (used[a]) continue;
      used[a] = 1;
      if (size[a] > c) { ok = false; break; }
      int partner = -1;
      for (int oj = oi + 1; oj < nb; ++oj)
        if (!used[order[oj]] && size[a] + size[order[oj]] <= c) { partner = order[oj]; break; }
      if (partner >= 0) used[partner] = 1;
      lanes.push_back({a, partner});
    }
    if (ok && (int)lanes.size() <= 16) { cap = c; break; }
  }
  if (cap == 0) return -1;
  h.mel_units = cap;
  std::vector<std::vector<int>> slot(16, std::vector<int>(cap, -1));
  for (size_t l = 0; l < lanes.size(); ++l) {
    int pos = 0;
    for (int which = 0; which < 2; ++which) {
      const int b = which ? lanes[l].second : lanes[l].first;
      if (b < 0) continue;
      for (int c = first_unit[b]; c < first_unit[b + 1]; ++c) slot[l][pos++] = c;
    }
  }
  auto step_cost = [&](int i, int &worst, int &coll) {
    int cnt[16] = {0};
    for (int l = 0; l < 16; ++l)
      if (slot[l][i] >= 0) ++cnt[units[slot[l][i]].octet & 15];
    worst = 1; coll = 0;
    for (int r = 0; r < 16; ++r) { worst = std::max(worst, cnt[r]); coll += std::max(0, cnt[r] - 1); }
  };
  auto total_cost = [&](long &primary, long &secondary) {
    primary = secondary = 0;
    for (int i = 0; i < cap; ++i) { int w, c; step_cost(i, w, c); primary += w; secondary += c; }
  };
  long best_p, best_s;
  total_cost(best_p, best_s);
  for (bool improved = true; improved;) {
    improved = false;
    for (int l = 0; l < 16; ++l)
      for (int a = 0; a < cap; ++a)
        for (int b = a + 1; b < cap; ++b) {
          if (slot[l][a] == slot[l][b]) continue;
          std::swap(slot[l][a], slot[l][b]);
          long p, s2;
          total_cost(p, s2);
          if (p < best_p || (p == best_p && s2 < best_s)) { best_p = p; best_s = s2; improved = true; }
          else std::swap(slot[l][a], slot[l][b]);
        }
  }
  h.mel_conflict_steps = int(best_p - cap);
  if (getenv("SMILEHIP_DEBUG_TABLES"))
    fprintf(stderr, "fast512: %d mel units on %zu lanes, %d per lane, bank model: %ld extra cycles over %d steps (%ld colliding lanes)\n",
            h.n_slots, lanes.size(), cap, best_p - cap, cap, best_s);
  h.melw.assign(size_t(cap) * 16 * 2, make_float4(0.f, 0.f, 0.f, 0.f));
  h.melo.assign(size_t(cap) * 16, 0u);
  h.lane_bands.assign(16, int32_t(0xffff00));
  for (int i = 0; i < cap; ++i) {
    bool taken[16] = {false};
    for (int l = 0; l < 16; ++l)
      if (slot[l][i] >= 0) taken[units[slot[l][i]].octet & 15] = true;
    for (int l = 0; l < 16; ++l) {
      const size_t idx = size_t(i) * 16 + l;
      if (slot[l][i] >= 0) {
        const Unit &un = units[slot[l][i]];
        h.melw[2 * idx] = make_float4(un.w[0], un.w[1], un.w[2], un.w[3]);
        h.melw[2 * idx + 1] = make_float4(un.w[4], un.w[5], un.w[6], un.w[7]);
        h.melo[idx] = uint32_t(un.octet) * uint32_t(kOctetFloats * 4);
      } else {
        int o = 0;
        for (int r = 0; r < 16; ++r)
          if (!taken[r]) { o = r; taken[r] = true; break; }
        h.melo[idx] = uint32_t(o) * uint32_t(kOctetFloats * 4);
      }
    }
  }
  if (getenv("SMILEHIP_DEBUG_TABLES")) {
    fprintf(stderr, "fast512: unit octets [step][lane]:");
    for (size_t idx = 0; idx < h.melo.size(); ++idx) fprintf(stderr, " %u", h.melo[idx] / uint32_t(kOctetFloats * 4));
    fprintf(stderr, "\n");
  }
  for (size_t l = 0; l < lanes.size(); ++l) {
    uint32_t mask = 0;
    const int b0 = lanes[l].first;
    for (int i = 0; i < cap; ++i)
      if (slot[l][i] >= first_unit[b0] && slot[l][i] < first_unit[b0 + 1]) mask |= 1u << i;
    h.lane_bands[l] = int32_t(mask | (uint32_t(b0) << 8) | (uint32_t(lanes[l].second < 0 ? 0xff : lanes[l].second) << 16));
  }
  h.mel_scale = mel.scale * (cfg.use_power ? 0.25f : 0.5f);
  h.dct28.assign(16 * 28, 0.0f);
  for (int r = 0; r < dct.n_mfcc; ++r)
    for (int m = 0; m < mel.n_bands; ++m) h.dct28[size_t(r) * 28 + m] = dct.cos_rows[size_t(r) * mel.n_bands + m];
  for (int r = 0; r < dct.n_mfcc; ++r) h.dct28[size_t(r) * 28 + 27] = dct.gain[r];
  return 0;
}

template <int MP, bool PREEMPH, bool USE_POWER, bool ALIGNED, bool PLP, int UC, bool DELTA = false>
static hipError_t launch_mfcc512_one(bool padded, unsigned grid, size_t lds, hipStream_t s, const LldParams &P, const Fast512Tables &F) {
  if constexpr (PREEMPH) {
    if (padded) {
      hipError_t e = hipFuncSetAttribute(reinterpret_cast<const void *>(&lld_mfcc512_padded<MP, PREEMPH, USE_POWER, ALIGNED, PLP, UC, DELTA>),
                                         hipFuncAttributeMaxDynamicSharedMemorySize, (int)lds);
      if (e != hipSuccess) return e;
      SMILEHIP_KLAUNCH((lld_mfcc512_padded<MP, PREEMPH, USE_POWER, ALIGNED, PLP, UC, DELTA>), dim3(grid), dim3(kWavesPerBlock * 64), lds, s, P, F);
      return hipSuccess;
    }
  }
  hipError_t e = hipFuncSetAttribute(reinterpret_cast<const void *>(&lld_mfcc512<MP, PREEMPH, USE_POWER, ALIGNED, PLP, UC, DELTA>),
                                     hipFuncAttributeMaxDynamicSharedMemorySize, (int)lds);
  if (e != hipSuccess) return e;
  SMILEHIP_KLAUNCH((lld_mfcc512<MP, PREEMPH, USE_POWER, ALIGNED, PLP, UC, DELTA>), dim3(grid), dim3(kWavesPerBlock * 64), lds, s, P, F);
  return hipSuccess;
}

hipError_t launch_mfcc512(const LldParams &P, const Fast512Tables &F, const Fast512Host &h, bool aligned, bool fused_delta, hipStream_t s) {
  const int shared_floats = 256 * 2 + h.mp * 16 * 2 + 256 * 2 + h.mel_units * 16 * 8 + 16 * 28 + 48;
  const size_t lds = sizeof(float) * (size_t(shared_floats) + size_t(kWavesPerBlock) * kWaveFloats);
  if (fused_delta && (!aligned || !P.ftile_rec || P.n_ftiles <= 0)) return hipErrorInvalidValue;
  unsigned grid = (unsigned)(((fused_delta ? P.n_ftiles : P.n_tiles) + kWavesPerBlock - 1) / kWavesPerBlock);
  if (grid > (unsigned)h.max_blocks) grid = (unsigned)h.max_blocks;
#ifdef SMILEHIP_DEBUG_KNOBS
  if (const char *e = getenv("SMILEHIP_DEBUG_GRID")) grid = (unsigned)atoi(e);
#endif
  bool launched = false;
  const bool padded = P.pad_left != 0 || h.force_padded;
#define SMILEHIP_LAUNCH(...)                                                                                    \
  {                                                                                                             \
    hipError_t e = launch_mfcc512_one<__VA_ARGS__>(padded, grid, lds, s, P, F);                                 \
    if (e != hipSuccess) return e;                                                                              \
    launched = true;                                                                                            \
  }
#define SMILEHIP_MATCH(MPV, PE, UP, AL, PL, UCV)                                                                \
  (!launched && h.mp == MPV && (P.preemph != 0) == PE && (P.use_power != 0) == UP && aligned == AL && (P.plp != 0) == PL && h.mel_units == UCV)
#define SMILEHIP_PICK_UD(MPV, PE, UP, PL, UCV) \
  if (fused_delta && SMILEHIP_MATCH(MPV, PE, UP, true, PL, UCV)) SMILEHIP_LAUNCH(MPV, PE, UP, true, PL, UCV, true)
#define SMILEHIP_PICK_U(MPV, PE, UP, AL, PL, UCV) \
  if (!fused_delta && SMILEHIP_MATCH(MPV, PE, UP, AL, PL, UCV)) SMILEHIP_LAUNCH(MPV, PE, UP, AL, PL, UCV)
#define SMILEHIP_PICK(MPV, PE, UP, AL, PL) SMILEHIP_PICK_U(MPV, PE, UP, AL, PL, 6) SMILEHIP_PICK_U(MPV, PE, UP, AL, PL, 8)
#define SMILEHIP_PICKD(MPV, PE, UP, PL) SMILEHIP_PICK_UD(MPV, PE, UP, PL, 6) SMILEHIP_PICK_UD(MPV, PE, UP, PL, 8)
#define SMILEHIP_PICK2(MPV, PE, UP) SMILEHIP_PICK(MPV, PE, UP, true, false) SMILEHIP_PICK(MPV, PE, UP, false, false) SMILEHIP_PICKD(MPV, PE, UP, false)
#define SMILEHIP_PICK4(MPV) SMILEHIP_PICK2(MPV, true, true) SMILEHIP_PICK2(MPV, true, false) \
                            SMILEHIP_PICK2(MPV, false, true) SMILEHIP_PICK2(MPV, false, false) \
                             \
                            SMILEHIP_PICK(MPV, true, true, true, true) SMILEHIP_PICK(MPV, true, true, false, true) \
                            SMILEHIP_PICK(MPV, false, true, true, true) SMILEHIP_PICK(MPV, false, true, false, true) \
                            SMILEHIP_PICKD(MPV, true, true, true) SMILEHIP_PICKD(MPV, false, true, true)
  SMILEHIP_PICK4(13)
  SMILEHIP_PICK4(16)
#undef SMILEHIP_PICK4
#undef SMILEHIP_PICK2
#undef SMILEHIP_PICKD
#undef SMILEHIP_PICK
#undef SMILEHIP_PICK_U
#undef SMILEHIP_PICK_UD
#undef SMILEHIP_MATCH
#undef SMILEHIP_LAUNCH
  if (!launched) return hipErrorInvalidConfiguration;
  return hipGetLastError();
}

}
```

opensmile_amd/csrc/lld_params.hpp:

```cpp
#pragma once
#include "lld_device.hpp"
#include "lld_ooura.hpp"
#include "lld_ooura_wave.hpp"
#include "lld_tile_rec.hpp"
#include <hip/hip_runtime.h>

#include <cstdint>

#include "../../include/smilehip.h"

namespace smilehip {

struct LldParams {
  const int16_t *pcm;
  const float *pcm_f32;
  int64_t pcm_total;
  const int64_t *samp_off;
  const int64_t *frame_off;
  const int32_t *frame_utt;
  const int32_t *tile_utt;
  const int32_t *tile_t0;
  const TileRec *tile_rec;
  int32_t n_utt;
  int32_t n_tiles;
  const FTileRec *ftile_rec;
  int32_t n_ftiles;
  int64_t total_frames;
  float *out;
  int64_t ld_out;
  int32_t N, H, Nfft, K, pad_left;
  int32_t preemph, de;
  float k, one_minus_k, win_offset;
  const float *window;
  OouraTab oo;
  const float *mel_coef;
  const int32_t *mel_rng;
  float mel_scale;
  int32_t use_power, n_bands;
  const float *dct_rows;
  const float *dct_gain;
  int32_t n_mfcc;
  float melfloor, log_floor;
  int32_t plp;
  int32_t plp_order;
  float plp_compression;
  const float *plp_eql;
  const float *plp_cos;
  const float *plp_sin;
};

__device__ __forceinline__ PcmIn pcm_in(const LldParams &P) { PcmIn r; r.s = P.pcm; r.f = P.pcm_f32; return r; }

struct Fast512Tables {
  const float2 *tw256;
  const float2 *tw512;
  const float2 *win;
  const float4 *melw;
  const uint32_t *melo;
  const float *dct28;
  const int32_t *lane_bands;
  int32_t mel_units;
  float mel_scale;
  const float *plp_eql;
  const float *plp_sin;
};

struct Is09Params {
  float *raw16;
  float fsSec;
  double maxPitch;
  double voicingCutoff;
};

struct CompareParams {
  const int32_t *run_utt;
  const int32_t *run_t0;
  int32_t run_frames;
  float *rawA;
  float *rawB;
  float *mel1;
  const float *eql;
  const float *eql_log;
  const double *sharp_w;
  float plp_melfloor, compression, rasta_iir;
  float rasta_fir[5];
  double fsSec;
  int32_t N60;
  int64_t max_utt_samples;
  int32_t band_iL[2], band_iR[2];
  double band_wL[2], band_wR[2];
  double slope_Sf, slope_S2f;
};

struct F0Params {
  int32_t N, H, Nfft, K, pad_left;
  const float *window;
  OouraTab oo;
  const double *sp_rec;
  const double *sp_d1, *sp_d2;
  const int32_t *ip_k;
  const double *ip_co;
  const double *audw;
  const double *ip_rec;
  const int32_t *ip_cnt;
  const double *sw_rec;
  int32_t n_harm;
  int32_t shift[16];
  float scale[16];
  float Fmint, Fstept;
  double log_base;
  double min_pitch, max_pitch;
  float voicing_cutoff;
  float min_energy;
  double jit_Tw;
  int32_t jit_broken_thresh;
  double jit_step_sec;
  double vit_w[6];
  float *shs;
  float *e60;
  float *hps_tap;
  float *mag_keep;
  int64_t mag_ld;
  int32_t mode;
  double *ab;
  int64_t ab_rows;
  int32_t tile0, n_tiles_chunk;
  int64_t n_rows;
  const float *in_rows;
  int64_t ld_in, ld_tap, ld_shs;
  int32_t *pending;
  int32_t vit_buf;
  int32_t vit_log_out;
  double jit_search_range;
  int32_t n_cand;
  int32_t old_peaks;
  int64_t jit_t_shift;
  float *jit_shim_db;
  double *jit_stream;
  const int32_t *jit_item_utt, *jit_item_t0;
  int32_t n_jit_items;
  int32_t *jit_redo;
  int32_t scale_off;
  int32_t jit_cap;
  int32_t *jit_ctl;
};

struct GemapsParams {
  const int32_t *run_utt, *run_t0;
  int32_t run_frames;
  float *raw20;
  float *spec220;
  const float *eql;
  float plp_melfloor, compression;
  double fsSec;
  int32_t sl_iL[2], sl_iR[2];
  double sl_wL[2], sl_wR[2], sl_Nind[2];
  int32_t rng_lo, rng_hi;
  int32_t ar_n1, ar_n2;
  float spec_floor, log_spec_floor, log_spec_factor;
  const float *rs_cos, *rs_sin;
  float rs_norm;
  float *lpc;
  float *formants;
  int64_t total_frames20;
  double fm_T, fm_min, fm_max;
  uint64_t *fm_flags;
  const int64_t *frame_off20;
  int32_t n_utt20;
  int32_t fm_resume;
  double *fm_state;
  double fsSec60;
  const float *pitch3;
  const float *jit4;
  const float *shim_db;
  float *harm6;
  const float *mag60;
  int64_t mag60_ld;
  const int64_t *frame_off60;
  const TileRec *tile60;
// ... 83 lines not shown
```

opensmile_amd/csrc/lld_tile_rec.hpp:

```cpp
#pragma once
#include <cstdint>

namespace smilehip {

struct TileRec {
  int64_t samp0;
  int64_t row0;
  int32_t n_frames;
  int32_t pad;
};

struct FTileRec {
  int64_t samp0;
  int64_t row0;
  int32_t n_frames;
  int32_t live_n;
  int32_t e0, e1;
  int32_t lo;
  int32_t delta_on;
};

}
```

opensmile_amd/csrc/phase_timing.hpp:

```cpp
#pragma once
#include <hip/hip_runtime.h>

namespace smilehip {

#ifdef SMILEHIP_PHASE_TIMING
#define SMILEHIP_PHASE_COUNTERS(array, len, entry)                                                                   \
  __device__ unsigned long long array[len];                                                                         \
  extern "C" int entry(unsigned long long *out, int reset) {                                                        \
    if (out && hipMemcpyFromSymbol(out, HIP_SYMBOL(array), sizeof(unsigned long long) * (len)) != hipSuccess) return -1; \
    if (reset) {                                                                                                    \
      unsigned long long z[len] = {0};                                                                              \
      if (hipMemcpyToSymbol(HIP_SYMBOL(array), z, sizeof(z)) != hipSuccess) return -1;                              \
    }                                                                                                               \
    return 0;                                                                                                       \
  }
template <int N>
struct PhaseTimer {
  unsigned long long acc[N] = {};
  unsigned long long last = __builtin_amdgcn_s_memtime();
  __device__ __forceinline__ void operator()(int i) {
    const unsigned long long t = __builtin_amdgcn_s_memtime();
    acc[i] += t - last;
    last = t;
  }
  __device__ __forceinline__ void count(int i) { acc[i] += 1; }
  __device__ __forceinline__ void flush(unsigned long long *counters, int first = 0) {
    if ((threadIdx.x & 63) == 0)
      for (int i = 0; i < N; ++i) atomicAdd(&counters[first + i], acc[i]);
  }
};
__device__ __forceinline__ void phase_wait_vm() { asm volatile("s_waitcnt vmcnt(0)" ::: "memory"); }
#else
#define SMILEHIP_PHASE_COUNTERS(array, len, entry) constexpr unsigned long long *array = nullptr;
template <int N>
struct PhaseTimer {
  __device__ __forceinline__ void operator()(int) {}
  __device__ __forceinline__ void count(int) {}
  __device__ __forceinline__ void flush(unsigned long long *, int = 0) {}
};
__device__ __forceinline__ void phase_wait_vm() {}
#endif

}
```

opensmile_amd/csrc/smilehip_batch.cpp:

```cpp
#include "smilehip_internal.hpp"
#include "batch_layout.hpp"

smilehip_batch::~smilehip_batch() { delete f0_batch; }

static inline bool mfcc_like(const smilehip_plan *p) {
  return p->cfg.chain_kind == SMILEHIP_CHAIN_MFCC || p->cfg.chain_kind == SMILEHIP_CHAIN_PLP;
}

static BatchLayoutSpec layout_spec(const smilehip_plan *plan) {
  const smilehip_lld_config &c = plan->cfg;
  BatchLayoutSpec s;
  s.chain_kind = c.chain_kind;
  s.N = plan->geo.N; s.H = plan->geo.H; s.period = plan->geo.period;
  s.row_extra = plan_row_extra(plan);
  s.fused_delta_eligible = plan->use_fast && mfcc_like(plan) && c.n_delta == 2 && c.delta_win == 2 && !c.append_log_energy && !c.cms &&
                           !getenv("SMILEHIP_NO_FUSED_DELTA");
  s.fast_slots = std::max<int64_t>(1, plan->fast.max_blocks) * 8;
  s.tile_frames = plan->use_fast ? fast512_tile_frames() : (c.chain_kind == SMILEHIP_CHAIN_COMPARE_F0 ? f0_tile_frames() : (int64_t(1) << 40));
  s.dtile_rows = chain_tile_rows(); s.short_T = chain_short_max(); s.jitter_chunk = jitter_chunk_frames();
  if (const char *rf = getenv("SMILEHIP_RUN_FRAMES")) { const int v = atoi(rf); if (v >= 1 && v <= 4096) s.run_frames_override = v; }
  return s;
}

static inline size_t at_least_one(int64_t n) { return size_t(n ? n : 1); }

static int alloc_mfcc_scratch(const smilehip_plan *plan, smilehip_batch *b, const BatchLayout &L) {
  b->n_ftiles = (int32_t)L.ftiles.size();
  if (b->n_ftiles) return b->d_ftile_rec.upload(L.ftiles);
  if (plan->cfg.n_delta > 0 && b->total_frames > 0 && b->d_static.alloc(size_t(b->total_frames) * size_t(plan_n_static(plan))))
    return fail(SMILEHIP_ERR_HIP, "hipMalloc of the static-block scratch failed");
  return SMILEHIP_OK;
}

static int alloc_is09_scratch(smilehip_batch *b, const BatchLayout &L) {
  int rc;
  if (b->total_frames > 0 && (rc = b->d_frame_utt.upload(L.frame_utt))) return rc;
  if (b->d_raw16.alloc(size_t(b->total_frames) * 16)) return fail(SMILEHIP_ERR_HIP, "hipMalloc of the IS09 scratch matrix failed");
  return SMILEHIP_OK;
}

static int alloc_compare_ab_scratch(smilehip_batch *b, const BatchLayout &L) {
  int rc;
  b->n_runs = (int32_t)L.run_utt.size();
  if ((rc = b->d_run_utt.upload(L.run_utt)) || (rc = b->d_run_t0.upload(L.run_t0))) return rc;
  const size_t nf = at_least_one(b->total_frames);
  if (b->d_rawA.alloc(nf * 4) || b->d_rawB.alloc(nf * 55) || b->d_mel1.alloc(nf * 26) || b->d_b_extra.alloc(at_least_one(b->n_utt) * 110))
    return fail(SMILEHIP_ERR_HIP, "hipMalloc of the ComParE scratch matrices failed");
  (void)hipMemset(b->d_rawA.p, 0, nf * 4 * sizeof(float));
  return SMILEHIP_OK;
}

static int alloc_f0_scratch(const smilehip_plan *plan, smilehip_batch *b, const BatchLayout &L) {
  const size_t nf = at_least_one(b->total_frames);
  if (b->d_shs.alloc(nf * 21) || b->d_e60.alloc(nf)) return fail(SMILEHIP_ERR_HIP, "hipMalloc of the F0 scratch matrices failed");
  const size_t nab = (size_t)std::max<int64_t>(f0_scratch_doubles(b->n_tiles, (int)plan->geo.K), 1);
  if (b->d_f0_ab.alloc(nab)) return fail(SMILEHIP_ERR_HIP, "hipMalloc of the F0 row scratch (%zu MB) failed", nab * sizeof(double) >> 20);
  static const bool pipe_on = [] { const char *e = getenv("SMILEHIP_F0_PIPE"); return e && e[0] == '1'; }();
  if (pipe_on && b->n_tiles > f0_chunk_tiles()) {
    size_t free_b = 0, total_b = 0;
    if (hipMemGetInfo(&free_b, &total_b) != hipSuccess || free_b / 4 <= nab * sizeof(double) || b->d_f0_ab2.alloc(nab))
      (void)hipGetLastError();
  }
  int rc;
  const std::vector<int32_t> zp(at_least_one(b->n_utt), 0);
  if ((rc = b->d_pending.upload(zp)) || (rc = b->d_jit_redo.upload(zp)) || (rc = b->d_jit_utt.upload(L.jit_utt)) ||
      (rc = b->d_jit_t0.upload(L.jit_t0)) || (rc = b->d_jit_ctl.upload(std::vector<int32_t>(2, 0))))
    return rc;
  return SMILEHIP_OK;
}

static int alloc_compare_scratch(smilehip_plan *plan, smilehip_batch *b, const BatchLayout &L) {
  int rc;
  if ((rc = alloc_compare_ab_scratch(b, L)) || (rc = smilehip_batch_create(plan->f0_plan, b->h_samp_off.data(), b->n_utt, &b->f0_batch)))
    return rc;
  const size_t nf = at_least_one(b->f0_batch->total_frames);
  if (b->d_pitch2.alloc(nf * 2) || b->d_jit4.alloc(nf * 4)) return fail(SMILEHIP_ERR_HIP, "hipMalloc of the F0 group's scratch matrices failed");
  return SMILEHIP_OK;
}

static void try_keep_magnitudes(const smilehip_plan *f0_plan, smilehip_batch *fb) {
  if (fb->total_frames <= 0) return;
  const int64_t ld = (f0_plan->geo.K + 3) & ~int64_t(3);
  const size_t n = size_t(fb->total_frames) * size_t(ld);
  size_t free_b = 0, total_b = 0;
  const char *env = getenv("SMILEHIP_HARM_KEEP_MAG");
  bool keep = hipMemGetInfo(&free_b, &total_b) == hipSuccess && n * sizeof(float) <= free_b / 2;
  if (env && env[0] == '0') keep = false;
  if (env && env[0] == '1') keep = true;
  if (keep && fb->d_mag_keep.alloc(n) == SMILEHIP_OK)
    fb->mag_ld = ld;
  else
    (void)hipGetLastError();
}

static int alloc_egemaps_scratch(smilehip_plan *plan, smilehip_batch *b, const BatchLayout &L) {
  int rc;
  b->n_runs = (int32_t)L.run_utt.size();
  if ((rc = b->d_run_utt.upload(L.run_utt)) || (rc = b->d_run_t0.upload(L.run_t0)) || (rc = b->d_fin_off.upload(b->h_fin_off)) ||
      (rc = smilehip_batch_create(plan->f0_plan, b->h_samp_off.data(), b->n_utt, &b->f0_batch)))
    return rc;
  const size_t nf = at_least_one(b->total_frames), nf60 = at_least_one(b->f0_batch->total_frames), nfin = at_least_one(b->h_fin_off[b->n_utt]);
  if (b->d_raw20.alloc(nf * 12) || b->d_spec220.alloc(nf * 220) || b->d_lpc.alloc(nf * 12) || b->d_formants.alloc(nf * 10) ||
      b->d_pitch3.alloc(nf60 * 3) || b->d_jit4.alloc(nf60 * 4) || b->d_shim.alloc(nf60) || b->d_harm6.alloc(nf60 * 6) ||
      b->d_func_in.alloc(nfin * 36))
    return fail(SMILEHIP_ERR_HIP, "hipMalloc of the eGeMAPS scratch matrices failed (%.1f GB needed)",
                double(nf * 254 + nf60 * 14 + nfin * 36) * 4e-9);
  if ((rc = b->d_pending_j.upload(std::vector<int32_t>(at_least_one(b->n_utt), 0))) || (rc = b->d_harm_ctl.upload(std::vector<int32_t>(2, 0))) ||
      (rc = b->d_fm_flags.upload(std::vector<uint64_t>(2 * ((nf + 63) / 64), 0))))
    return rc;
  try_keep_magnitudes(plan->f0_plan, b->f0_batch);
  return SMILEHIP_OK;
}

extern "C" int smilehip_batch_create(smilehip_plan *plan, const int64_t *h_off, int32_t n_utt, smilehip_batch **out) {
  if (!plan || !out || n_utt < 0 || (n_utt > 0 && !h_off)) return fail(SMILEHIP_ERR_INVALID, "smilehip_batch_create: bad argument");
  *out = nullptr;
  if (!plan->ctx) return fail(SMILEHIP_ERR_NO_DEVICE, "host-only plan: no device attached (tables only)");
  if (plan->stage_mask != SMILEHIP_STAGE_ALL) return fail(SMILEHIP_ERR_INVALID, "single-component plan cannot run the fused chain");
  if (int rt = require_transform(plan, "smilehip_batch_create")) return rt;
  HIP_TRY(hipSetDevice(plan->ctx->device));
  std::unique_ptr<smilehip_batch> b(new (std::nothrow) smilehip_batch());
  if (!b) return fail(SMILEHIP_ERR_NOMEM, "out of host memory");
  BatchLayout L;
  if (const int bad = batch_layout(layout_spec(plan), h_off, n_utt, L))
    return fail(SMILEHIP_ERR_INVALID, "sample offsets must be non-decreasing (utterance %d)", bad - 1);
  b->plan = plan;
  b->n_utt = n_utt;
  b->total_frames = L.total_frames; b->total_rows = L.total_rows;
  b->n_tiles = (int32_t)L.tile_utt.size(); b->n_dtiles = (int32_t)L.dtile_utt.size();
  b->run_frames = L.run_frames; b->all_even = L.all_even;
  int rc;
  if ((rc = b->d_samp_off.upload(L.samp_off)) || (rc = b->d_frame_off.upload(L.frame_off)) || (rc = b->d_row_off.upload(L.row_off)) ||
      (rc = b->d_tile_utt.upload(L.tile_utt)) || (rc = b->d_tile_t0.upload(L.tile_t0)) || (rc = b->d_tile_rec.upload(L.tile_rec)) ||
      (rc = b->d_dtile_utt.upload(L.dtile_utt)) || (rc = b->d_dtile_t0.upload(L.dtile_t0)) || (rc = b->d_short.upload(L.short_utts)))
    return rc;
  b->h_samp_off = std::move(L.samp_off);
  b->h_frame_off = std::move(L.frame_off); b->h_row_off = std::move(L.row_off);
  b->h_fin_off = std::move(L.fin_off); b->h_short = std::move(L.short_utts);
  switch (plan->cfg.chain_kind) {
    case SMILEHIP_CHAIN_IS09: rc = alloc_is09_scratch(b.get(), L); break;
    case SMILEHIP_CHAIN_COMPARE_AB: rc = alloc_compare_ab_scratch(b.get(), L); break;
    case SMILEHIP_CHAIN_COMPARE_F0: rc = alloc_f0_scratch(plan, b.get(), L); break;
    case SMILEHIP_CHAIN_COMPARE: rc = alloc_compare_scratch(plan, b.get(), L); break;
    case SMILEHIP_CHAIN_EGEMAPS: rc = alloc_egemaps_scratch(plan, b.get(), L); break;
    case SMILEHIP_CHAIN_MFCC:
    case SMILEHIP_CHAIN_PLP: rc = alloc_mfcc_scratch(plan, b.get(), L); break;
  }
  if (rc) return rc;
  *out = b.release();
  return SMILEHIP_OK;
}

extern "C" void smilehip_batch_destroy(smilehip_batch *b) { delete b; }
extern "C" int64_t smilehip_batch_total_frames(const smilehip_batch *b) { return b ? b->total_frames : 0; }
extern "C" int64_t smilehip_batch_total_rows(const smilehip_batch *b) { return b ? b->total_rows : 0; }
extern "C" int smilehip_batch_delta_fused(const smilehip_batch *b) { return b && b->n_ftiles > 0 ? 1 : 0; }
extern "C" int smilehip_batch_frame_offsets(const smilehip_batch *b, int64_t *o) {
  if (!b || !o) return fail(SMILEHIP_ERR_INVALID, "smilehip_batch_frame_offsets: null argument");
  std::memcpy(o, b->h_row_off.data(), b->h_row_off.size() * sizeof(int64_t));
  return SMILEHIP_OK;
}

static bool serial_forced() {
  static const bool v = [] { const char *e = getenv("SMILEHIP_SERIAL"); return e && e[0] != '0'; }();
  return v;
}
static bool serial_streams(int64_t total_frames) {
  static const int forced = [] { const char *e = getenv("SMILEHIP_SERIAL"); return e ? (e[0] == '0' ? 0 : 1) : -1; }();
  return forced >= 0 ? forced != 0 : total_frames >= (int64_t)4000000;
}
static void fill_params(const smilehip_plan *p, const smilehip_batch *b, const int16_t *d_pcm, float *d_out,
                        int64_t ld, LldParams &P) {
  std::memset(&P, 0, sizeof(P));
  P.pcm = d_pcm;
  P.pcm_f32 = b->run_pcm_f32;
  P.pcm_total = b->h_samp_off.back();
  P.samp_off = b->d_samp_off.p;
  P.frame_off = b->d_frame_off.p;
  P.frame_utt = b->d_frame_utt.p;
  P.tile_utt = b->d_tile_utt.p;
  P.tile_t0 = b->d_tile_t0.p;
  P.tile_rec = b->d_tile_rec.p;
  P.ftile_rec = b->d_ftile_rec.p;
  P.n_ftiles = b->n_ftiles;
  P.n_utt = b->n_utt;
  P.n_tiles = b->n_tiles;
  P.total_frames = b->total_frames;
  P.out = d_out;
  P.ld_out = ld;
  P.N = (int32_t)p->geo.N;
  P.H = (int32_t)p->geo.H;
  P.Nfft = (int32_t)p->geo.Nfft;
  P.K = (int32_t)p->geo.K;
  P.pad_left = p->cfg.zero_pad_symmetric ? (int32_t)((p->geo.Nfft - p->geo.N) / 2) : 0;
  P.preemph = p->cfg.preemph;
  P.de = p->cfg.preemph_de;
  P.k = p->cfg.preemph_k;
  P.one_minus_k = 1 - p->cfg.preemph_k;
  P.win_offset = (float)p->cfg.win_offset;
  P.window = p->d_window.p;
  P.oo = p->oo.tab();
  P.mel_coef = p->d_mel_coef.p;
  P.mel_rng = p->d_mel_rng.p;
  P.mel_scale = p->mel.scale;
  P.use_power = p->cfg.use_power;
  P.n_bands = p->mel.n_bands;
  P.dct_rows = p->d_dct_rows.p;
  P.dct_gain = p->d_dct_gain.p;
  P.n_mfcc = p->dct.n_mfcc;
  P.melfloor = p->dct.melfloor;
  P.log_floor = p->dct.log_floor;
  P.plp = p->cfg.chain_kind == SMILEHIP_CHAIN_PLP;
  P.plp_order = p->cfg.plp_lp_order;
  P.plp_compression = p->cfg.plp_compression;
  P.plp_eql = p->d_plp_eql.p;
  P.plp_cos = p->d_plp_cos.p;
  P.plp_sin = p->d_plp_sin.p;
}

static ChainParams chain_params(const smilehip_batch *b, const float *x, int64_t ld_x, int32_t D, float *out, int64_t ld_out) {
  ChainParams Q;
  std::memset(&Q, 0, sizeof(Q));
  Q.frame_off = b->d_frame_off.p;
  Q.row_off = b->d_row_off.p;
  Q.tile_utt = b->d_dtile_utt.p;
  Q.tile_t0 = b->d_dtile_t0.p;
  Q.n_tiles = b->n_dtiles;
  Q.n_utt = b->n_utt;
  Q.x = x;
  Q.ld_x = ld_x;
  Q.out = out;
  Q.ld_out = ld_out;
  Q.D = D;
  Q.short_T = chain_short_max();
  Q.short_utts = b->d_short.p;
  Q.n_short = (int32_t)b->h_short.size();
  return Q;
}

static int delta_chain_from(smilehip_plan *plan, smilehip_batch *b, const float *d_x, int64_t ld_x, int copy_col, float *d_io,
                            int64_t ld, int32_t D, int32_t W, int32_t n_orders, void *stream) {
  if (!plan || !b || !d_io) return fail(SMILEHIP_ERR_INVALID, "smilehip_delta_chain: null argument");
  if (n_orders < 1 || n_orders > 2 || W < 1 || W > 4 || D < 1 || D > 64 || ld < (int64_t)D * (1 + n_orders))
    return fail(SMILEHIP_ERR_INVALID, "smilehip_delta_chain: unsupported D=%d W=%d orders=%d ld=%lld", D, W, n_orders, (long long)ld);
  if (b->total_frames == 0) return SMILEHIP_OK;
  if (b->total_rows != b->total_frames) return fail(SMILEHIP_ERR_INVALID, "smilehip_delta_chain: batch belongs to a chain with extra rows");
  ChainParams Q = chain_params(b, d_x, ld_x, D, d_io, ld);
  Q.copy_col = copy_col;
  Q.n_stages = n_orders;
  Q.kind[0] = Q.kind[1] = 0;
  Q.W[0] = Q.W[1] = W;
  Q.out_col[0] = D;
  Q.out_col[1] = 2 * D;
  hipError_t e = launch_chain(Q, (hipStream_t)stream);
  if (e != hipSuccess) return fail(SMILEHIP_ERR_HIP, "window-chain kernel launch failed: %s", hipGetErrorString(e));
  return SMILEHIP_OK;
}

extern "C" int smilehip_delta_chain(smilehip_plan *plan, smilehip_batch *b, float *d_io, int64_t ld, int32_t D,
                                    int32_t W, int32_t n_orders, void *stream) {
  return delta_chain_from(plan, b, d_io, ld, -1, d_io, ld, D, W, n_orders, stream);
}

extern "C" int smilehip_mfcc_run(smilehip_plan *plan, smilehip_batch *b, const int16_t *d_pcm, float *d_out,
                                 int64_t ld_out, void *stream) {
  if (!plan || !b || b->plan != plan) return fail(SMILEHIP_ERR_INVALID, "smilehip_mfcc_run: plan/batch mismatch");
  if (plan->cfg.chain_kind != SMILEHIP_CHAIN_MFCC && plan->cfg.chain_kind != SMILEHIP_CHAIN_PLP)
    return fail(SMILEHIP_ERR_INVALID, "smilehip_mfcc_run: plan is not an MFCC / PLP chain (use smilehip_lld_run)");
  const int n_static = plan_n_static(plan), n_cep = plan->dct.n_mfcc;
  const int n_out = n_static * (1 + plan->cfg.n_delta);
  if (ld_out < n_out) return fail(SMILEHIP_ERR_INVALID, "ld_out %lld < n_out %d", (long long)ld_out, n_out);
  if (b->total_frames == 0) return SMILEHIP_OK;
  if (!d_pcm || !d_out) return fail(SMILEHIP_ERR_INVALID, "smilehip_mfcc_run: null device pointer");
  hipStream_t s = (hipStream_t)stream;
  LldParams P;
  fill_params(plan, b, d_pcm, d_out, ld_out, P);
  const bool aligned_in = b->all_even && ((reinterpret_cast<uintptr_t>(d_pcm) & 3) == 0);
  const bool fused_delta = plan->use_fast && !b->run_pcm_f32 && b->n_ftiles > 0 && aligned_in;
  const bool compact = !fused_delta && plan->cfg.n_delta > 0 && b->d_static.p != nullptr;
  if (compact) {
    P.out = b->d_static.p;
    P.ld_out = n_static;
  }
  hipEvent_t *ev = plan->ev[plan->n_timed % smilehip_plan::kRing];
  if (plan->timing) {
    for (int i = 0; i < 3; ++i)
      if (!ev[i]) HIP_TRY(hipEventCreate(&ev[i]));
    HIP_TRY(hipEventRecord(ev[0], s));
  }
  hipError_t e;
  if (plan->use_fast && !b->run_pcm_f32) {
    Fast512Tables F;
    F.tw256 = plan->d_tw256.p;
    F.tw512 = plan->d_tw512.p;
    F.win = plan->d_fwin.p;
    F.melw = plan->d_melw.p;
    F.melo = plan->d_melo.p;
    F.dct28 = plan->d_dct28.p;
    F.lane_bands = plan->d_lane_bands.p;
    F.mel_units = plan->fast.mel_units;
    F.mel_scale = plan->fast.mel_scale;
    F.plp_eql = plan->d_plp_eql.p;
    F.plp_sin = plan->d_plp_sin.p;
    const bool aligned = aligned_in;
    e = launch_mfcc512(P, F, plan->fast, aligned, fused_delta, s);
  } else {
    e = launch_mfcc_generic(P, s);
  }
  if (e != hipSuccess) return fail(SMILEHIP_ERR_HIP, "mfcc kernel launch failed: %s", hipGetErrorString(e));
  if (plan->cfg.append_log_energy) {
    e = launch_log_energy(P, b->d_dtile_utt.p, b->d_dtile_t0.p, b->n_dtiles, P.out, P.ld_out, n_cep, s);
    if (e != hipSuccess) return fail(SMILEHIP_ERR_HIP, "log-energy kernel launch failed: %s", hipGetErrorString(e));
  }
  if (plan->timing) HIP_TRY(hipEventRecord(ev[1], s));
  if (fused_delta) {
    if (!b->h_short.empty()) {
      ChainParams Q = chain_params(b, d_out, ld_out, n_static, d_out, ld_out);
      Q.tile_utt = Q.tile_t0 = nullptr; Q.n_tiles = 0;
      Q.copy_col = -1;
      Q.n_stages = 2;
      Q.kind[0] = Q.kind[1] = 0;
      Q.W[0] = Q.W[1] = plan->cfg.delta_win;
      Q.out_col[0] = n_static;
      Q.out_col[1] = 2 * n_static;
      e = launch_chain(Q, s);
      if (e != hipSuccess) return fail(SMILEHIP_ERR_HIP, "window-chain kernel launch failed: %s", hipGetErrorString(e));
    }
  } else if (plan->cfg.n_delta > 0) {
    int rc = compact ? delta_chain_from(plan, b, b->d_static.p, n_static, 0, d_out, ld_out, n_static,
                                        plan->cfg.delta_win, plan->cfg.n_delta, stream)
                     : smilehip_delta_chain(plan, b, d_out, ld_out, n_static, plan->cfg.delta_win, plan->cfg.n_delta, stream);
    if (rc) return rc;
  }
  if (plan->cfg.cms) {
    e = launch_cms(b->d_frame_off.p, b->n_utt, P.out, P.ld_out, d_out, ld_out, n_cep, s);
    if (e != hipSuccess) return fail(SMILEHIP_ERR_HIP, "mean-subtraction kernel launch failed: %s", hipGetErrorString(e));
  }
// ... 471 lines not shown
```

opensmile_amd/csrc/smilehip_internal.hpp:

```cpp
#pragma once
#include <hip/hip_runtime.h>

#include <cmath>
#include <cstdarg>
#include <cstdio>
#include <cstring>
#include <algorithm>
#include <map>
#include <memory>
#include <mutex>
#include <new>
#include <string>
#include <vector>

#include "../../include/smilehip.h"
#include "lld_launch.hpp"
#include "lld_ooura.hpp"
#include "lld_params.hpp"
#include "ooura_tables.hpp"
#include "tables.hpp"

using namespace smilehip;


// ... 48 lines not shown
    release();
    if (smilehip::dev_malloc(reinterpret_cast<void **>(&p), (count ? count : 1) * sizeof(T)) != hipSuccess) {
      p = nullptr;
      return fail(SMILEHIP_ERR_HIP, "device allocation of %zu bytes failed", (count ? count : 1) * sizeof(T));
    }
    n = count;
    return SMILEHIP_OK;
  }
  int upload(const std::vector<T> &h) {
    release();
    n = h.size();
    const size_t bytes = (n ? n : 1) * sizeof(T);
    HIP_TRY(smilehip::dev_malloc(reinterpret_cast<void **>(&p), bytes));
    if (n) HIP_TRY(smilehip::dev_upload(p, h.data(), n * sizeof(T)));
    return SMILEHIP_OK;
  }
};

struct OouraDev {
  OouraHost h;
  DevBuf<float4> d_tw;
  DevBuf<float2> d_rft;
  int build(int n, bool upload_tables) {
    if (make_ooura(n, h)) return fail(SMILEHIP_ERR_INVALID, "reference-order FFT: length %d is not a power of two in [64, 8192]", n);
    if (!upload_tables) return SMILEHIP_OK;
    std::vector<float4> t4(h.tw.size() / 4);
    std::memcpy(t4.data(), h.tw.data(), t4.size() * sizeof(float4));
    std::vector<float2> r2(h.rft.size() / 2);
    std::memcpy(r2.data(), h.rft.data(), r2.size() * sizeof(float2));
    int rc;
    if ((rc = d_tw.upload(t4)) || (rc = d_rft.upload(r2))) return rc;
    return SMILEHIP_OK;
  }
  OouraTab tab() const {
    OouraTab T{};
    T.tw = d_tw.p; T.rft = d_rft.p;
    T.M = h.M; T.logM = h.logM; T.nlev = h.nlev; T.leaf8 = h.leaf8;
    T.n_tw = (int)(h.tw.size() / 4);
    T.wn4r = h.wn4r; T.wk1r = h.wk1r; T.wk1i = h.wk1i;
    return T;
  }
};

struct smilehip_plan;
struct smilehip_batch;
struct smilehip_plan {
  smilehip_context *ctx = nullptr;
  smilehip_lld_config cfg{};
  Geometry geo;
  std::vector<float> h_window;
  MelBank mel;
  DctTables dct;
  DevBuf<float> d_window, d_mel_coef, d_dct_rows, d_dct_gain;
  DevBuf<int32_t> d_mel_rng;
  DevBuf<float2> d_tw256, d_tw512, d_fwin;
  OouraDev oo;
  DevBuf<float4> d_melw;
  DevBuf<uint32_t> d_melo;
  DevBuf<float> d_dct28;
  DevBuf<int32_t> d_lane_bands;
  Fast512Host fast;
  bool use_fast = false;
  DevBuf<float> d_eql, d_eql_log;
  DevBuf<float> d_plp_eql, d_plp_cos, d_plp_sin;
  std::vector<float> h_plp_cos;
  DevBuf<double> d_sharp;
  smilehip_plan *f0_plan = nullptr;
  hipStream_t side_stream = nullptr;
  hipEvent_t ev_fork = nullptr, ev_join = nullptr;
  F0Pipe f0_pipe;
  hipStream_t bg_stream = nullptr;
  hipEvent_t ev_bg_fork = nullptr, ev_bg_join = nullptr;
  F0Host f0;
  DevBuf<double> d_f0_rec, d_f0_d1, d_f0_d2, d_f0_co, d_f0_audw;
  DevBuf<double> d_f0_iprec, d_f0_swrec;
  DevBuf<int32_t> d_f0_k, d_f0_ipcnt;
  float rasta_iir = 0.f, rasta_fir[5] = {0, 0, 0, 0, 0};
  DevBuf<float> d_rs_cos, d_rs_sin;
  DevBuf<uint64_t> d_fm_flags;
  int32_t gm_sl_iL[2] = {0, 0}, gm_sl_iR[2] = {0, 0}, gm_rng_lo = 0, gm_rng_hi = 0, gm_ar_n1 = 0, gm_ar_n2 = 0;
  double gm_sl_wL[2] = {0, 0}, gm_sl_wR[2] = {0, 0}, gm_sl_Nind[2] = {0, 0};
  float gm_spec_floor = 0.f, gm_log_spec_floor = 0.f, gm_log_spec_factor = 0.f;
  double gm_target_fs = 0.0;
  int32_t band_iL[2] = {0, 0}, band_iR[2] = {0, 0};
  double band_wL[2] = {0, 0}, band_wR[2] = {0, 0}, slope_Sf = 0, slope_S2f = 0;
  static constexpr int kRing = 128;
  bool timing = false;
  hipEvent_t ev[kRing][3] = {};
  int64_t n_timed = 0;
  int force_generic = 0;
  uint32_t stage_mask = SMILEHIP_STAGE_ALL;
  ~smilehip_plan() {
    delete f0_plan;
    if (side_stream) (void)hipStreamDestroy(side_stream);
    if (ev_fork) (void)hipEventDestroy(ev_fork);
    if (ev_join) (void)hipEventDestroy(ev_join);
    if (f0_pipe.spec) (void)hipStreamDestroy(f0_pipe.spec);
    if (f0_pipe.sweep) (void)hipStreamDestroy(f0_pipe.sweep);
    for (hipEvent_t ev_ : {f0_pipe.start, f0_pipe.spec_done[0], f0_pipe.spec_done[1], f0_pipe.sweep_done[0], f0_pipe.sweep_done[1],
                           f0_pipe.cand_done[0], f0_pipe.cand_done[1]})
      if (ev_) (void)hipEventDestroy(ev_);
    if (bg_stream) (void)hipStreamDestroy(bg_stream);
    if (ev_bg_fork) (void)hipEventDestroy(ev_bg_fork);
    if (ev_bg_join) (void)hipEventDestroy(ev_bg_join);
    for (auto &slot : ev)
      for (auto &e : slot)
        if (e) (void)hipEventDestroy(e);
  }
};
inline int require_transform(const smilehip_plan *p, const char *who) {
  if (p->oo.d_tw.p) return SMILEHIP_OK;
  return fail(SMILEHIP_ERR_INVALID, "%s: FFT length %lld: the reference-order transform is built for 64 .. 8192 points", who,
              (long long)p->geo.Nfft);
}

struct smilehip_batch {
  smilehip_plan *plan = nullptr;
  int32_t n_utt = 0;
  int64_t total_frames = 0;
  std::vector<int64_t> h_samp_off, h_frame_off, h_row_off;
  int64_t total_rows = 0;
  DevBuf<int64_t> d_row_off;
  DevBuf<float> d_raw16;
  DevBuf<float> d_static;
  DevBuf<float> d_rawA, d_rawB, d_mel1;
  DevBuf<float> d_b_extra;
  DevBuf<float> d_shs, d_e60;
  DevBuf<float> d_mag_keep;
  int64_t mag_ld = 0;
  DevBuf<double> d_f0_ab;
  DevBuf<double> d_f0_ab2;
  float *d_hps_tap = nullptr;
  DevBuf<int32_t> d_pending;
  DevBuf<int32_t> d_jit_utt, d_jit_t0, d_jit_redo, d_jit_ctl;
  DevBuf<float> d_pitch2, d_jit4;
  smilehip_batch *f0_batch = nullptr;
  DevBuf<float> d_raw20, d_spec220, d_lpc, d_formants, d_pitch3, d_shim, d_harm6, d_func_in;
  DevBuf<int32_t> d_pending_j;
  DevBuf<int32_t> d_harm_ctl;
  DevBuf<uint64_t> d_fm_flags;
  DevBuf<int64_t> d_fin_off;
  std::vector<int64_t> h_fin_off;
  bool gm_ran = false;
  const float *run_pcm_f32 = nullptr;
  ~smilehip_batch();
  DevBuf<int32_t> d_run_utt, d_run_t0;
  int32_t n_runs = 0;
  int32_t run_frames = 8;
  std::vector<int32_t> h_short;
  DevBuf<int64_t> d_samp_off, d_frame_off;
  DevBuf<int32_t> d_frame_utt;
  DevBuf<int32_t> d_tile_utt, d_tile_t0, d_short, d_dtile_utt, d_dtile_t0;
  DevBuf<TileRec> d_tile_rec;
  DevBuf<FTileRec> d_ftile_rec;
  int32_t n_ftiles = 0;
  int32_t n_tiles = 0, n_dtiles = 0;
  bool all_even = true;
};

int plan_n_static(const smilehip_plan *p);
int plan_n_out(const smilehip_plan *p);
int plan_row_extra(const smilehip_plan *p);
void fill_f0_params(const smilehip_plan *plan, smilehip::F0Params &Q);
void gemaps_plan_consts(const smilehip_plan *plan, smilehip::GemapsParams &G);

int smilehip_funcspec_from_mask(uint32_t mask, double period, smilehip_func_spec *spec);
```

opensmile_amd/csrc/smilehip_plan.cpp:

```cpp
#include "smilehip_internal.hpp"

extern "C" void smilehip_config_mfcc12_0_d_a(smilehip_lld_config *c) {
  std::memset(c, 0, sizeof(*c));
  c->struct_size = sizeof(*c);
  c->sample_rate = 16000.0;
  c->frame_size_sec = 0.0250;
  c->frame_step_sec = 0.010;
  c->preemph = 1;
  c->preemph_k = 0.97f;
  c->preemph_de = 0;
  c->win_func = SMILEHIP_WIN_HAMM;
  c->win_sigma = 0.4;
  c->win_gain = 1.0;
  c->win_offset = 0.0;
  c->zero_pad_symmetric = 0;
  c->n_bands = 26;
  c->lofreq = 0.0f;
  c->hifreq = 8000.0f;
  c->use_power = 1;
  c->mel_htk_compatible = 1;
  c->first_mfcc = 0;
  c->last_mfcc = 12;
  c->cep_lifter = 22.0f;
  c->mfcc_htk_compatible = 1;
// ... 70 lines not shown
  c->pitch_max = 620.0;
  c->voicing_cutoff = 0.7;
  c->shs_n_harmonics = 15;
  c->shs_compression = 0.85f;
  c->f0_min_energy = 0.001f;
}

extern "C" void smilehip_config_compare16(smilehip_lld_config *c) {
  smilehip_config_compare16_ab(c);
  c->chain_kind = SMILEHIP_CHAIN_COMPARE;
  c->pitch_min = 52.0;
  c->pitch_max = 620.0;
  c->voicing_cutoff = 0.7;
  c->shs_n_harmonics = 15;
  c->shs_compression = 0.85f;
  c->f0_min_energy = 0.001f;
  c->vit_buffer_len = 30;
  c->jitter_search_range = 0.25;
}

extern "C" void smilehip_config_is13_compare(smilehip_lld_config *c) {
  smilehip_config_compare16(c);
  c->zero_pad_symmetric = 0;
  c->jitter_broken_thresh = 1;
}

extern "C" void smilehip_config_egemapsv02(smilehip_lld_config *c) {
  smilehip_config_compare16_ab(c);
  c->chain_kind = SMILEHIP_CHAIN_EGEMAPS;
  c->first_mfcc = 1;
  c->last_mfcc = 4;
  c->n_delta = 0;
  c->sma_win = 3;
  c->pitch_min = 55.0;
  c->pitch_max = 1000.0;
  c->voicing_cutoff = 0.7;
  c->shs_n_harmonics = 15;
  c->shs_compression = 0.85f;
  c->f0_min_energy = 0.001f;
  c->vit_buffer_len = 40;
  c->jitter_search_range = 0.1;
}

extern "C" void smilehip_config_egemapsv01a(smilehip_lld_config *c) {
  smilehip_config_egemapsv02(c);
  c->zero_pad_symmetric = 0;
  c->jitter_broken_thresh = 1;
  c->formant_max_freq = 5500.0;
}

static inline bool is_compare_ab_like(const smilehip_lld_config &c) {
  return c.chain_kind == SMILEHIP_CHAIN_COMPARE_AB || c.chain_kind == SMILEHIP_CHAIN_COMPARE;
}

static int build_tables(smilehip_plan *p, bool upload = true) {
  int rc;
  if ((rc = make_geometry(p->cfg, p->geo)) != SMILEHIP_OK) return fail(rc, "invalid framing parameters");
  if (p->geo.Nfft > 8192) return fail(SMILEHIP_ERR_INVALID, "FFT length %lld > 8192 unsupported", (long long)p->geo.Nfft);
  const uint32_t mask = p->cfg.stage_mask ? p->cfg.stage_mask : SMILEHIP_STAGE_ALL;
  p->h_window.assign(size_t(p->geo.N), 1.0f);
  if ((mask & SMILEHIP_STAGE_WINDOW) && (rc = make_window(p->cfg, p->geo.N, p->h_window)) != SMILEHIP_OK)
    return fail(rc, "unknown window function %d", p->cfg.win_func);
  if (mask & SMILEHIP_STAGE_MEL) {
    if ((rc = make_mel(p->cfg, p->geo, p->mel)) != SMILEHIP_OK) return fail(rc, "invalid mel bank parameters");
  } else {
    p->mel = MelBank();
    p->mel.n_bands = p->cfg.n_bands;
  }
  if (mask & SMILEHIP_STAGE_MFCC) {
    if ((rc = make_dct(p->cfg, p->dct)) != SMILEHIP_OK) return fail(rc, "invalid MFCC range");
  } else {
    p->dct = DctTables();
  }
  p->stage_mask = mask;
  if (p->cfg.n_delta < 0 || p->cfg.n_delta > 2) return fail(SMILEHIP_ERR_INVALID, "n_delta must be 0..2");
  if (p->cfg.chain_kind == SMILEHIP_CHAIN_IS09) {
    if (mask != SMILEHIP_STAGE_ALL || p->dct.n_mfcc != 12 || p->cfg.n_delta != 1 || p->cfg.sma_win < 3 || !(p->cfg.sma_win & 1) ||
        p->cfg.sma_win > 9)
      return fail(SMILEHIP_ERR_INVALID, "IS09 chain needs 12 MFCC, one delta stage and an odd smaWin in 3..9");
  } else if (is_compare_ab_like(p->cfg)) {
    if (mask != SMILEHIP_STAGE_ALL || p->dct.n_mfcc != 14 || p->mel.n_bands != 26 || p->cfg.n_delta != 1 ||
        p->cfg.delta_win != 2 || p->cfg.sma_win != 3 || !p->cfg.use_power || p->cfg.preemph ||
        (p->geo.Nfft != 256 && p->geo.Nfft != 512 && p->geo.Nfft != 1024))
      return fail(SMILEHIP_ERR_INVALID, "ComParE A+B chain: unsupported parameter set (20 ms frames at 8 .. 48 kHz)");
  } else if (p->cfg.chain_kind == SMILEHIP_CHAIN_EGEMAPS) {
    if (mask != SMILEHIP_STAGE_ALL || p->dct.n_mfcc != 4 || p->mel.n_bands != 26 || p->cfg.n_delta != 0 || p->cfg.sma_win != 3 ||
        !p->cfg.use_power || p->cfg.preemph || (p->geo.Nfft != 256 && p->geo.Nfft != 512 && p->geo.Nfft != 1024))
      return fail(SMILEHIP_ERR_INVALID, "eGeMAPS chain: unsupported parameter set (20 ms frames at 8 .. 48 kHz, 26 bands, MFCC 1..4)");
  } else if (p->cfg.chain_kind == SMILEHIP_CHAIN_PLP) {
    if (mask != SMILEHIP_STAGE_ALL || p->cfg.plp_lp_order < 1 || p->cfg.plp_lp_order > 15 || !p->cfg.mel_htk_compatible ||
        !p->cfg.use_power || p->mel.n_bands > 30 || p->cfg.plp_compression < 0.0f)
      return fail(SMILEHIP_ERR_INVALID, "PLP chain: lpOrder 1..15, HTK-scaled power mel bands (<= 30) required");
    if (p->cfg.first_mfcc != 0 && p->cfg.first_mfcc != 1) return fail(SMILEHIP_ERR_INVALID, "PLP chain: firstCC must be 0 or 1");
    p->dct.n_mfcc = p->cfg.plp_lp_order + (p->cfg.first_mfcc == 0 ? 1 : 0);
    p->dct.melfloor = 1.0f;
  } else if (p->cfg.chain_kind == SMILEHIP_CHAIN_COMPARE_F0) {
    if (mask != SMILEHIP_STAGE_ALL || p->cfg.preemph || p->cfg.n_delta != 0 || p->cfg.win_offset != 0.0)
      return fail(SMILEHIP_ERR_INVALID, "F0 chain: no pre-emphasis / deltas / window offset");
    if (p->geo.Nfft != 512 && p->geo.Nfft != 1024 && p->geo.Nfft != 2048 && p->geo.Nfft != 4096)
      return fail(SMILEHIP_ERR_INVALID, "F0 chain: the kernels are instantiated for spectra of 512 .. 4096 points (60 ms frames at 8 .. 48 kHz); "
                  "this configuration gives %lld points", (long long)p->geo.Nfft);
    if (p->cfg.shs_n_harmonics < 1 || p->cfg.shs_n_harmonics > 17 || !(p->cfg.pitch_max > p->cfg.pitch_min) || p->cfg.pitch_min < 40.0)
      return fail(SMILEHIP_ERR_INVALID, "F0 chain: nHarmonics 1..17, minPitch >= 40 Hz (period search window of the jitter kernel), "
                  "maxPitch > minPitch");
    if (p->cfg.shs_n_candidates < 0 || p->cfg.shs_n_candidates > 6)
      return fail(SMILEHIP_ERR_INVALID, "F0 chain: cPitchShs nCandidates 1 .. 6 (0 = 6)");
    if ((rc = make_f0_tables(p->geo.K, p->geo.fft_frame_size_sec, p->cfg.shs_n_harmonics, p->cfg.shs_compression,
                             p->cfg.specscale_min_f > 0.0 ? p->cfg.specscale_min_f : 25.0, p->f0)))
      return fail(rc, "F0 chain: spectrum geometry / nHarmonics not usable by cSpecScale / cPitchShs");
  } else if (p->cfg.chain_kind != SMILEHIP_CHAIN_MFCC) {
    return fail(SMILEHIP_ERR_INVALID, "unknown chain_kind %d", p->cfg.chain_kind);
  }
  if (p->cfg.n_delta > 0 && (p->cfg.delta_win < 1 || p->cfg.delta_win > 4))
    return fail(SMILEHIP_ERR_INVALID, "delta_win must be 1..4");

  std::vector<int32_t> rng((mask & SMILEHIP_STAGE_MEL) ? size_t(4) * p->mel.n_bands : 0);
  for (int b = 0; b < p->mel.n_bands && (mask & SMILEHIP_STAGE_MEL); ++b) {
    rng[4 * b + 0] = p->mel.rise_lo[b];
    rng[4 * b + 1] = p->mel.rise_hi[b];
    rng[4 * b + 2] = p->mel.fall_lo[b];
    rng[4 * b + 3] = p->mel.fall_hi[b];
  }
  std::vector<float> plp_eql(32, 0.0f), plp_sin(16, 1.0f);
  const bool is_plp = p->cfg.chain_kind == SMILEHIP_CHAIN_PLP;
  if (is_plp) {
    const int nB = p->mel.n_bands, nFreq = nB + 2, nAuto = p->cfg.plp_lp_order + 1;
    p->h_plp_cos.assign(size_t(nAuto) * nFreq, 0.0f);
    const float a = (float)M_PI / (float)(nFreq - 1);
    for (int i = 0; i < nAuto; i++) {
      const int ib = i * nFreq;
      int m;
      p->h_plp_cos[ib] = 1.0f;
      for (m = 1; m < (nFreq - 1); m++) p->h_plp_cos[m + ib] = (float)(2.0 * std::cos(a * (double)i * (double)m));
      p->h_plp_cos[m + ib] = (float)(std::cos(a * (double)i * (double)m));
    }
    const float L = (float)(int)p->cfg.cep_lifter;
    for (int i = 0; i < nAuto; i++)
      plp_sin[i] = (L > 0.0f) ? ((float)1.0 + L / (float)2.0 * std::sin((float)M_PI * ((float)(i)) / L)) : 1.0f;
    for (int m = 1; m <= nB; ++m) {
      const double hz = 700.0 * (std::exp(double(p->mel.centres[m]) / 1127.0) - 1.0);
      const double f2 = hz * hz, fs = f2 / (f2 + 1.6e5);
      plp_eql[m - 1] = (float)(fs * fs * ((f2 + 1.44e6) / (f2 + 9.61e6)));
    }
  }
  p->use_fast = false;
  if (mask == SMILEHIP_STAGE_ALL && (p->cfg.chain_kind == SMILEHIP_CHAIN_MFCC || (is_plp && p->mel.n_bands == 26 && p->cfg.use_power)) &&
      !p->force_generic && fast512_applicable((int)p->geo.Nfft, (int)p->geo.N)) {
    p->use_fast = fast512_build_host(p->cfg, p->geo, p->h_window, p->mel, p->dct, p->fast) == 0;
    if (p->use_fast && is_plp) {
      p->fast.dct28.assign(16 * 28, 0.0f);
      std::copy(p->h_plp_cos.begin(), p->h_plp_cos.end(), p->fast.dct28.begin());
    }
    if (p->ctx) p->fast.max_blocks = 2 * p->ctx->prop.multiProcessorCount;
  }
  if (!upload) return SMILEHIP_OK;
  if ((rc = p->d_window.upload(p->h_window))) return rc;
  if ((rc = p->d_mel_coef.upload(p->mel.coef))) return rc;
  if ((rc = p->d_mel_rng.upload(rng))) return rc;
  if ((rc = p->d_dct_rows.upload(p->dct.cos_rows))) return rc;
  if ((rc = p->d_dct_gain.upload(p->dct.gain))) return rc;
  if (p->geo.Nfft >= 64 && (rc = p->oo.build((int)p->geo.Nfft, true))) return rc;
  if (is_plp && ((rc = p->d_plp_eql.upload(plp_eql)) || (rc = p->d_plp_cos.upload(p->h_plp_cos)) || (rc = p->d_plp_sin.upload(plp_sin))))
    return rc;
  if (p->cfg.chain_kind == SMILEHIP_CHAIN_COMPARE_F0 &&
      ((rc = p->d_f0_rec.upload(p->f0.sp_rec)) || (rc = p->d_f0_d1.upload(p->f0.sp_d1)) || (rc = p->d_f0_d2.upload(p->f0.sp_d2)) ||
       (rc = p->d_f0_co.upload(p->f0.ip_co)) || (rc = p->d_f0_audw.upload(p->f0.audw)) || (rc = p->d_f0_k.upload(p->f0.ip_k)) ||
       (rc = p->d_f0_iprec.upload(p->f0.ip_rec)) || (rc = p->d_f0_swrec.upload(p->f0.sw_rec)) || (rc = p->d_f0_ipcnt.upload(p->f0.ip_cnt))))
    return rc;
  if (p->cfg.vit_buffer_len < 0 || p->cfg.vit_buffer_len == 1 || p->cfg.vit_buffer_len > 128)
    return fail(SMILEHIP_ERR_INVALID, "vit_buffer_len must be 0 (= 30) or 2..128");
  if (p->cfg.jitter_search_range < 0.0 || p->cfg.jitter_search_range >= 1.0)
    return fail(SMILEHIP_ERR_INVALID, "jitter_search_range must be in [0, 1)");
  if (p->cfg.chain_kind == SMILEHIP_CHAIN_EGEMAPS) {
    std::vector<float> eql(26);
    for (int m = 1; m <= 26; ++m) {
      const double hz = 700.0 * (std::exp(double(p->mel.centres[m]) / 1127.0) - 1.0);
      const double w = 2.0 * M_PI * hz, w2 = w * w, c = w2 + 6300000.0;
      eql[m - 1] = float((c > 0.0) ? (1e32 * ((w2 + 56.8e6) * w2 * w2) / (c * c * (w2 + 0.38e9) * (w2 * w2 * w2 * w + 1.7e31))) : 0.0);
    }
    if ((rc = p->d_eql.upload(eql))) return rc;
    const int Nsrc = (int)p->geo.K;
    const double F0 = 1.0 / p->geo.fft_frame_size_sec;
    const int lo_hz[2] = {0, 500}, hi_hz[2] = {500, 1500};
    for (int b = 0; b < 2; ++b) {
      int ii;
      double wghtL, wghtR, idxL, idxR;
      for (ii = 0; ii < Nsrc; ii++) if (F0 * ii > (double)lo_hz[b]) break;
      if ((ii < Nsrc) && (ii > 0)) wghtL = (F0 * ii - (double)lo_hz[b]) / (F0 * ii - F0 * (ii - 1)); else wghtL = 1.0;
      idxL = (double)ii - 1.0;
      if (idxL < 0) idxL = 0;
      if (idxL >= Nsrc) idxL = Nsrc;
      if (wghtL == 0.0) wghtL = 1.0;
      for (ii = 0; ii < Nsrc; ii++) if (F0 * ii >= (float)hi_hz[b]) break;
      if ((ii < Nsrc) && (ii > 0)) wghtR = ((double)hi_hz[b] - F0 * (ii - 1)) / (F0 * ii - F0 * (ii - 1)); else wghtR = 1.0;
      if ((ii < Nsrc) && (F0 * ii == (float)hi_hz[b])) idxR = (double)ii; else idxR = (double)ii - 1.0;
      if (idxR >= Nsrc) idxR = Nsrc - 1;
      if (wghtR == 0.0) wghtR = 1.0;
      int iL = (int)std::floor(idxL), iR = (int)std::floor(idxR);
      if (iL >= Nsrc) { iL = iR = Nsrc - 1; wghtR = 0.0; wghtL = 0.0; }
      if (iR >= Nsrc) { iR = Nsrc - 1; wghtR = 1.0; }
      if (iL < 0) iL = 0;
      if (iR < 0) iR = 0;
      if (iR - iL >= 64 || iR >= 64) return fail(SMILEHIP_ERR_INVALID, "eGeMAPS chain: slope band wider than the kernel's 64 bins");
      p->gm_sl_iL[b] = iL; p->gm_sl_iR[b] = iR; p->gm_sl_wL[b] = wghtL; p->gm_sl_wR[b] = wghtR; p->gm_sl_Nind[b] = idxR - idxL;
    }
    int lo = -1, hi = -1;
    for (int i = 0; i < Nsrc; i++) {
      if ((double)0 >= F0 * i) lo = i;
      if ((double)5000 > F0 * i) hi = i;
    }
    if (hi == -1 || hi >= Nsrc) hi = Nsrc - 1;
    if (lo < 0) lo = 0;
    p->gm_rng_lo = lo; p->gm_rng_hi = hi;
    {
      int n1 = 0, n2 = 0;
      while (n1 < Nsrc && F0 * (double)n1 < 1000.0) ++n1;
      n2 = n1;
      while (n2 < Nsrc && !(F0 * (double)n2 > 5000.0)) ++n2;
      p->gm_ar_n1 = n1; p->gm_ar_n2 = n2;
    }
    float specFloor = (float)0.0000001;
    specFloor = specFloor * specFloor;
    p->gm_spec_floor = specFloor;
    p->gm_log_spec_floor = (float)(10.0 * (double)std::log(specFloor) / std::log(10.0));
    p->gm_log_spec_factor = (float)(10.0 / std::log(10.0));
    {
      const long n_in = (long)p->geo.Nfft;
      const double fs_sec = p->geo.fft_frame_size_sec, last_fs_sec = (double)p->geo.N * p->geo.period, bT = p->geo.period;
      const double sr = 1.0 / bT;
      double target_fs = 11000.0, ratio = target_fs / sr, nd;
      long n_out;
      if ((fs_sec != last_fs_sec) && (last_fs_sec != 0.0) && (last_fs_sec != bT)) {
        const double nout0 = std::round((double)n_in * ratio * last_fs_sec / fs_sec);
        const double new_ratio = nout0 / ((double)n_in * (last_fs_sec / fs_sec));
        n_out = (long)nout0;
        if (new_ratio != ratio) { target_fs = sr * new_ratio; ratio = new_ratio; }
        nd = (double)n_in * ratio;
      } else {
        const double nout0 = std::round((double)n_in * ratio);
        const double new_ratio = nout0 / (double)n_in;
        n_out = (long)nout0;
        if (new_ratio != ratio) { target_fs = sr * new_ratio; ratio = new_ratio; }
        nd = nout0;
      }
      long kMax = n_in > n_out ? n_out : n_in;
      if (kMax & 1) kMax--;
      if (n_out != 220 || kMax / 2 - 1 != 109 || n_out >= n_in)
        return fail(SMILEHIP_ERR_INVALID, "eGeMAPS chain: cSpecResample geometry %ld -> %ld is not the one the kernel is built for", n_in, n_out);
      p->gm_target_fs = target_fs;
      std::vector<float> ct(size_t(109) * 220), st(size_t(109) * 220);
      const double pi2 = 2.0 * M_PI;
      for (long i = 0; i < n_out; i++)
        for (long k = 2; k < kMax; k += 2) {
          const double kn = pi2 * (double)(k / 2 * i) / nd;
          ct[size_t(k / 2 - 1) * 220 + i] = (float)std::cos(kn);
          st[size_t(k / 2 - 1) * 220 + i] = (float)std::sin(kn);
        }
      if ((rc = p->d_rs_cos.upload(ct)) || (rc = p->d_rs_sin.upload(st))) return rc;
    }
  }
  if (is_compare_ab_like(p->cfg)) {
    std::vector<float> eql(26), eqll(26);
    for (int m = 1; m <= 26; ++m) {
      const double hz = 700.0 * (std::exp(double(p->mel.centres[m]) / 1127.0) - 1.0);
      const double w = 2.0 * M_PI * hz, w2 = w * w, c = w2 + 6300000.0;
      const double e = (c > 0.0) ? (1e32 * ((w2 + 56.8e6) * w2 * w2) / (c * c * (w2 + 0.38e9) * (w2 * w2 * w2 * w + 1.7e31))) : 0.0;
      eql[m - 1] = float(e);
      eqll[m - 1] = std::log(eql[m - 1]);
    }
    const double Tl = p->geo.frame_period;
    const float lower = 1.0f, upper = 29.0f;
    p->rasta_iir = float(1.0 - std::sin(2.0 * M_PI * lower * Tl));
    const float om = float(std::cos(2.0 * M_PI * upper * Tl));
    const float norm = float(std::sqrt(10.0 * (32.0 * om * om + 8.0)));
    p->rasta_fir[0] = float(2.0 / norm);
    p->rasta_fir[1] = float(-4.0 * om / norm);
    p->rasta_fir[2] = 0.0f;
    p->rasta_fir[3] = -p->rasta_fir[1];
    p->rasta_fir[4] = -p->rasta_fir[0];
    if ((rc = p->d_eql.upload(eql)) || (rc = p->d_eql_log.upload(eqll))) return rc;
  }
  if (is_compare_ab_like(p->cfg) || (mask & SMILEHIP_STAGE_SPECTRAL)) {
    std::vector<double> sw(size_t(p->geo.K - 1));
    const double F0 = 1.0 / p->geo.fft_frame_size_sec;
    for (int64_t j = 1; j < p->geo.K; ++j) {
      const double x = F0 * double(j);
      double zz = 0.0;
      if (x > 0) {
        zz = (26.81 / (1.0 + 1960.0 / x)) - 0.53;
        if (zz < 2) zz = 0.85 * zz + 0.3;
        else if (zz > 20.1) zz = 1.22 * zz - 0.22 * 20.1;
      }
      const double g = (zz <= 16.0) ? 1.0 : std::pow((zz - 16.0) / 4.0, 1.5849625) + 1.0;
      sw[size_t(j - 1)] = zz * g;
    }
    int band_lo[2] = {250, 1000}, band_hi[2] = {650, 4000};
    if (p->cfg.spectral_band_lo[0] || p->cfg.spectral_band_lo[1] || p->cfg.spectral_band_hi[0] || p->cfg.spectral_band_hi[1])
      for (int b = 0; b < 2; ++b) {
        band_lo[b] = p->cfg.spectral_band_lo[b];
        band_hi[b] = p->cfg.spectral_band_hi[b];
        if (band_lo[b] < 0 || band_hi[b] <= band_lo[b]) return fail(SMILEHIP_ERR_INVALID, "cSpectral bands[%d] = %d-%d", b, band_lo[b], band_hi[b]);
      }
    const int Nsrc = (int)p->geo.K;
    for (int b = 0; b < 2; ++b) {
      int ii;
      double wghtL, wghtR, idxL, idxR;
// ... 177 lines not shown
```

Before: 2.882 billion.

## Add span-based work schedule with seam exchange for fused-delta MFCC kernel

Replaces the grid-stride loop over fused-delta tiles with per-wave spans of work pieces, described by a new piece-record table and span index. An optional, env-gated layout cuts utterances into cost-balanced spans. Adjacent waves in a block then share seam frames through LDS with flags, avoiding recomputing overlap frames. By default the old tiles are just regrouped round-robin into spans. The kernel still gains extra LDS, register pinning and flag logic, which could cut occupancy or constrain scheduling.

Result: no change. 2.866 billion (-0.6%).

```diff
diff --git a/include/smilehip.h b/include/smilehip.h
--- a/include/smilehip.h
+++ b/include/smilehip.h
@@ -265,6 +265,7 @@
 int64_t smilehip_batch_total_frames(const smilehip_batch *batch);
 int64_t smilehip_batch_total_rows(const smilehip_batch *batch);
 int  smilehip_batch_delta_fused(const smilehip_batch *batch);
+int  smilehip_batch_span_schedule(const smilehip_batch *batch);
 int  smilehip_batch_frame_offsets(const smilehip_batch *batch, int64_t *h_row_offsets);
 
 int  smilehip_mfcc_run(smilehip_plan *plan, smilehip_batch *batch, const int16_t *d_pcm,
diff --git a/opensmile_amd/capi.py b/opensmile_amd/capi.py
--- a/opensmile_amd/capi.py
+++ b/opensmile_amd/capi.py
@@ -162,6 +162,7 @@
     "smilehip_config_plp_0_d_a": (None, [C.POINTER(LldConfig)]),
     "smilehip_batch_total_rows": (_i64, [_vp]),
     "smilehip_batch_delta_fused": (C.c_int, [_vp]),
+    "smilehip_batch_span_schedule": (C.c_int, [_vp]),
     "smilehip_functionals_is09_mask": (C.c_uint32, []),
     "smilehip_functionals_count": (C.c_int, [C.c_uint32]),
     "smilehip_functionals_matrix": (C.c_int, [_vp, _vp, _i64, _i64, C.c_int32, C.c_uint32, _vp, _vp]),
@@ -638,6 +639,7 @@
         self.total_frames = int(load().smilehip_batch_total_frames(self._h))
         self.total_rows = int(load().smilehip_batch_total_rows(self._h))
         self.delta_fused = bool(load().smilehip_batch_delta_fused(self._h))
+        self.span_schedule = bool(load().smilehip_batch_span_schedule(self._h))
         fo = np.zeros(self.n_utt + 1, np.int64)
         _check(load().smilehip_batch_frame_offsets(self._h, fo.ctypes.data))
         self.frame_offsets = fo
diff --git a/opensmile_amd/csrc/batch_layout.hpp b/opensmile_amd/csrc/batch_layout.hpp
--- a/opensmile_amd/csrc/batch_layout.hpp
+++ b/opensmile_amd/csrc/batch_layout.hpp
@@ -22,6 +22,9 @@
   int short_T = 0;
   int jitter_chunk = 0;
   int run_frames_override = 0;
+  bool spans = true;
+  bool span_exchange = false;
+  int64_t span_slots = 0;
 };
 
 struct BatchLayout {
@@ -35,6 +38,9 @@
   std::vector<int32_t> run_utt, run_t0;
   int32_t run_frames = 8;
   std::vector<FTileRec> ftiles;
+  std::vector<FPieceRec> fpieces;
+  std::vector<int32_t> fspan_first;
+  bool fspans_balanced = false;
   std::vector<int32_t> jit_utt, jit_t0;
   std::vector<int32_t> frame_utt;
 };
@@ -95,6 +101,178 @@
   std::stable_sort(out.ftiles.begin(), out.ftiles.end(), [](const FTileRec &a, const FTileRec &c) { return a.n_frames > c.n_frames; });
 }
 
+constexpr double kVirtualPassCost = 0.2;
+constexpr int64_t kMinSpanPasses = 8;
+
+inline void layout_fused_spans(const BatchLayoutSpec &s, const int64_t *h_off, int32_t n_utt, BatchLayout &out) {
+  struct Utt { int32_t u; int64_t T, P, start; bool cuttable; };
+  std::vector<Utt> U;
+  std::vector<int64_t> starts, ends;
+  int64_t R = 0;
+  for (int32_t u = 0; u < n_utt; ++u) {
+    const int64_t T = out.frame_off[u + 1] - out.frame_off[u];
+    if (T <= 0) continue;
+    U.push_back({u, T, (T + 3) / 4, R, T > s.short_T});
+    starts.push_back(R);
+    R += (T + 3) / 4;
+    ends.push_back(R);
+  }
+  out.fspan_first.assign(1, 0);
+  if (U.empty()) return;
+  const double cv = kVirtualPassCost;
+  const auto utt_at = [&](int64_t g) { return size_t(std::upper_bound(starts.begin(), starts.end(), g) - starts.begin()) - 1; };
+  const auto inside = [&](int64_t g) { return g < R && starts[utt_at(g)] != g; };
+  const auto cost = [&](int64_t a, int64_t b) {
+    const auto lo = std::upper_bound(ends.begin(), ends.end(), a), hi = std::upper_bound(ends.begin(), ends.end(), b);
+    return double(b - a) + cv * double(hi - lo);
+  };
+  const auto allowed = [&](int64_t g) {
+    if (!inside(g)) return true;
+    const Utt &t = U[utt_at(g)];
+    return t.cuttable && g - t.start >= 2 && t.start + t.P - g >= 2;
+  };
+  const auto pick = [&](int64_t a, double target, int64_t lo_g, int64_t hi_g, double seam, bool seam_only = false) -> int64_t {
+    if (lo_g > hi_g) return -1;
+    int64_t l = lo_g, h = hi_g;
+    while (l < h) { const int64_t m = (l + h) / 2; if (cost(a, m) >= target) h = m; else l = m + 1; }
+    int64_t best = -1;
+    double best_d = 1e300;
+    const auto consider = [&](int64_t g) {
+      const double d = std::fabs(cost(a, g) + (inside(g) ? seam : 0.0) - target);
+      if (d < best_d) { best_d = d; best = g; }
+    };
+    for (int only = seam_only ? 1 : 0; only >= 0 && best < 0; --only) {
+      int found = 0;
+      for (int64_t g = l; g <= hi_g && found < 2; ++g) if (allowed(g) && (!only || inside(g))) { consider(g); ++found; }
+      found = 0;
+      for (int64_t g = l - 1; g >= lo_g && found < 2; --g) if (allowed(g) && (!only || inside(g))) { consider(g); ++found; }
+    }
+    return best;
+  };
+  const int64_t slots = s.span_slots > 0 ? s.span_slots : s.fast_slots;
+  const int64_t n_spans = std::max<int64_t>(1, std::min<int64_t>(slots, R / kMinSpanPasses));
+  const int64_t nb = (n_spans + 7) / 8;
+  const auto spans_of = [&](int64_t b) { return std::min<int64_t>(8, n_spans - 8 * b); };
+  std::vector<int64_t> block_end;
+  if (nb > 1) {
+    std::vector<int32_t> D((size_t)R + 1, 0);
+    std::vector<uint8_t> ok(size_t(R) + 1, 0), in(size_t(R) + 1, 0);
+    for (int64_t g = 0, e = 0; g <= R; ++g) {
+      while (size_t(e) < ends.size() && ends[size_t(e)] <= g) ++e;
+      D[size_t(g)] = (int32_t)e;
+      ok[size_t(g)] = allowed(g);
+      in[size_t(g)] = inside(g);
+    }
+    const auto bcost = [&](int64_t a, int64_t g) { return double(g - a) + cv * double(D[size_t(g)] - D[size_t(a)]) + (in[size_t(g)] ? 2.0 : 0.0); };
+    const double mean = (double(R) + cv * double(U.size()) + 2.0 * double(nb - 1)) * 8.0 / double(n_spans);
+    std::vector<int32_t> stamp(size_t(R) + 1, -1);
+    std::vector<double> Ws;
+    for (int i = 0; i <= 4; ++i)
+      for (int d = 0; d <= 8; ++d) Ws.push_back(std::floor(mean) + double(i) + cv * double(d));
+    std::sort(Ws.begin(), Ws.end());
+    for (size_t wi = 0; wi < Ws.size() && block_end.empty(); ++wi) {
+      const double W = Ws[wi];
+      if (W < mean) continue;
+      std::vector<std::vector<std::pair<int64_t, int64_t>>> reach((size_t)nb);
+      std::vector<int64_t> cur(1, 0);
+      std::fill(stamp.begin(), stamp.end(), -1);
+      int64_t left = n_spans;
+      for (int64_t b = 0; b + 1 < nb && !cur.empty(); ++b) {
+        left -= 8;
+        for (const int64_t a : cur)
+          for (int64_t g = std::max<int64_t>(a + 8 * kMinSpanPasses, a + (int64_t)W - 5); g <= a + (int64_t)W + 1 && g <= R - kMinSpanPasses * left; ++g) {
+            const double c = bcost(a, g);
+            if (!ok[size_t(g)] || stamp[size_t(g)] == (int32_t)b || c > W + 1e-9 || c < W - 1.0 - 1e-9) continue;
+            stamp[size_t(g)] = (int32_t)b;
+            reach[size_t(b)].push_back({g, a});
+          }
+        cur.clear();
+        for (const auto &r : reach[size_t(b)]) cur.push_back(r.first);
+        std::sort(cur.begin(), cur.end());
+      }
+      const double kl = double(spans_of(nb - 1)) / 8.0;
+      int64_t at = -1;
+      for (const int64_t a : cur) {
+        const double c = bcost(a, R);
+        if (R - a >= kMinSpanPasses * spans_of(nb - 1) && c <= W * kl + 1e-9 && (kl < 1.0 || c >= W - 1.0 - 1e-9)) { at = a; break; }
+      }
+      if (at < 0) continue;
+      block_end.assign(size_t(nb), R);
+      for (int64_t b = nb - 2; b >= 0; --b) {
+        block_end[size_t(b)] = at;
+        for (const auto &r : reach[size_t(b)]) if (r.first == at) { at = r.second; break; }
+      }
+    }
+  }
+  const auto emit_span = [&](int64_t c, int64_t e, bool mate_in_front, bool mate_behind) {
+    for (size_t i = utt_at(c); i < U.size() && U[i].start < e; ++i) {
+      const Utt &t = U[i];
+      const int64_t qa = std::max(c, t.start) - t.start, qb = std::min(e, t.start + t.P) - t.start;
+      const bool to_end = qb == t.P;
+      const int64_t p0 = 4 * qa, t0 = qa > 0 ? p0 + 4 : 0, t1 = to_end ? t.T : 4 * (qb + 1);
+      FPieceRec r;
+      r.samp0 = h_off[t.u] + p0 * s.H;
+      r.row0 = out.frame_off[t.u] + p0;
+      r.n_frames = (int32_t)((to_end ? 4 * t.P : t1) - p0 + 4);
+      r.live_n = (int32_t)(t.T - p0);
+      r.e0 = (int32_t)(t0 - p0);
+      r.e1 = (int32_t)(t1 - p0);
+      r.lo = (int32_t)(-p0);
+      r.delta_on = t.T > s.short_T;
+      r.virt = to_end ? 1 : (mate_behind ? 2 : 0);
+      r.publish = qa > 0 && mate_in_front;
+      out.fpieces.push_back(r);
+    }
+    out.fspan_first.push_back((int32_t)out.fpieces.size());
+  };
+  int64_t spans_left = n_spans;
+  int64_t a = 0;
+  for (int64_t b = 0; b < nb && a < R; ++b) {
+    const int64_t k = std::min<int64_t>(8, spans_left);
+    int64_t end = R;
+    if (!block_end.empty()) end = block_end[size_t(b)];
+    else if (b + 1 < nb) {
+      const double left = cost(a, R) + 2.0 * double(nb - 1 - b) + 2.0 * cv * double(spans_left - (nb - b));
+      end = pick(a, left * double(k) / double(spans_left) - 2.0 * cv * double(k - 1), a + kMinSpanPasses * k,
+                 R - kMinSpanPasses * (spans_left - k), 2.0);
+      if (end < 0) end = R;
+    }
+    int64_t c = a;
+    for (int64_t w = 0; w < 8; ++w) {
+      int64_t e = end;
+      if (c < end && w + 1 < k) {
+        const double left = cost(c, end) + (inside(end) ? 2.0 : 0.0) + 2.0 * cv * double(k - 1 - w);
+        e = pick(c, left / double(k - w), c + kMinSpanPasses, end - kMinSpanPasses * (k - 1 - w), 2.0 * cv, true);
+        if (e < 0) e = end;
+      }
+      if (c < e) emit_span(c, e, w > 0, e < end);
+      else out.fspan_first.push_back((int32_t)out.fpieces.size());
+      c = e;
+    }
+    a = end;
+    spans_left -= k;
+  }
+  while (out.fspan_first.size() > 1 && out.fspan_first[out.fspan_first.size() - 1] == out.fspan_first[out.fspan_first.size() - 2])
+    out.fspan_first.pop_back();
+  out.fspans_balanced = true;
+}
+
+inline void layout_tiles_as_spans(const BatchLayoutSpec &s, BatchLayout &out) {
+  const int64_t n = (int64_t)out.ftiles.size();
+  const int64_t slots = std::min<int64_t>(((n + 7) / 8) * 8, std::max<int64_t>(8, s.fast_slots / 8 * 8));
+  out.fspan_first.assign(1, 0);
+  for (int64_t sl = 0; sl < slots && sl < n; ++sl) {
+    for (int64_t i = sl; i < n; i += slots) {
+      const FTileRec &t = out.ftiles[(size_t)i];
+      FPieceRec r;
+      r.samp0 = t.samp0; r.row0 = t.row0; r.n_frames = t.n_frames; r.live_n = t.live_n; r.e0 = t.e0; r.e1 = t.e1; r.lo = t.lo;
+      r.delta_on = t.delta_on; r.virt = 0; r.publish = 0;
+      out.fpieces.push_back(r);
+    }
+    out.fspan_first.push_back((int32_t)out.fpieces.size());
+  }
+}
+
 inline int batch_layout(const BatchLayoutSpec &s, const int64_t *h_off, int32_t n_utt, BatchLayout &out) {
   out = BatchLayout();
   out.samp_off.assign(h_off, h_off + (n_utt ? n_utt + 1 : 0));
@@ -145,8 +323,11 @@
     out.frame_utt.resize((size_t)out.total_frames);
     for (int32_t u = 0; u < n_utt; ++u) std::fill(out.frame_utt.begin() + out.frame_off[u], out.frame_utt.begin() + out.frame_off[u + 1], u);
   }
-  if (s.fused_delta_eligible && out.total_frames > 0 && out.all_even)
+  if (s.fused_delta_eligible && out.total_frames > 0 && out.all_even) {
     layout_fused_tiles(s, h_off, n_utt, out);
+    if (s.spans && s.span_exchange) layout_fused_spans(s, h_off, n_utt, out);
+    else layout_tiles_as_spans(s, out);
+  }
   if (s.chain_kind == SMILEHIP_CHAIN_COMPARE_F0) {
     int64_t maxT = 0;
     for (int32_t u = 0; u < n_utt; ++u) maxT = std::max(maxT, out.frame_off[u + 1] - out.frame_off[u]);
diff --git a/opensmile_amd/csrc/lld_launch.hpp b/opensmile_amd/csrc/lld_launch.hpp
--- a/opensmile_amd/csrc/lld_launch.hpp
+++ b/opensmile_amd/csrc/lld_launch.hpp
@@ -29,12 +29,15 @@
   float mel_scale = 1.0f;
   int max_blocks = 512;
   bool force_padded = false;
+  bool span_exchange = false;
 };
 bool fast512_applicable(int Nfft, int N);
 int fast512_tile_frames();
 int fast512_build_host(const smilehip_lld_config &cfg, const Geometry &geo, const std::vector<float> &window,
                        const MelBank &mel, const DctTables &dct, Fast512Host &h);
-hipError_t launch_mfcc512(const LldParams &P, const Fast512Tables &F, const Fast512Host &h, bool aligned, bool fused_delta, hipStream_t s);
+hipError_t launch_mfcc512(const LldParams &P, const Fast512Tables &F, const Fast512Host &h, bool aligned, bool fused_delta, hipStream_t s,
+                          int *blocks_per_cu = nullptr);
+bool mfcc512_exchange_fits(const Fast512Host &h, bool preemph, bool use_power, bool plp, int pad_left);
 hipError_t launch_mfcc_generic(const LldParams &P, hipStream_t s);
 hipError_t launch_chain(const ChainParams &P, hipStream_t s);
 hipError_t launch_log_energy(const LldParams &P, const int32_t *d_tile_utt, const int32_t *d_tile_t0, int n_tiles, float *dst,
diff --git a/opensmile_amd/csrc/lld_mfcc512.hip b/opensmile_amd/csrc/lld_mfcc512.hip
--- a/opensmile_amd/csrc/lld_mfcc512.hip
+++ b/opensmile_amd/csrc/lld_mfcc512.hip
@@ -162,6 +162,13 @@
   }
 }
 
+constexpr int kXchgWaveFloats = 128;
+constexpr int kXchgFloats = kWavesPerBlock * kXchgWaveFloats + kWavesPerBlock;
+template <bool PREEMPH, bool PLP>
+constexpr bool seam_exchange() {
+  return PREEMPH || !PLP;
+}
+
 SMILEHIP_PHASE_COUNTERS(g_phase, 16, smilehip_debug_phase)
 
 template <int MP, bool PREEMPH, bool USE_POWER, bool ALIGNED, bool PLP, int UC, bool DELTA, bool PAD0>
@@ -193,6 +200,13 @@
     for (int i = threadIdx.x; i < 32; i += blockDim.x) s_plp[i] = F.plp_eql[i];
     for (int i = threadIdx.x; i < 16; i += blockDim.x) s_plp[32 + i] = F.plp_sin[i];
   }
+  constexpr bool XCHG = DELTA && seam_exchange<PREEMPH, PLP>();
+  float *s_xchg = smem + shared_floats + kWavesPerBlock * kWaveFloats;
+  typedef volatile __attribute__((address_space(3))) int *LdsFlag;
+  const LdsFlag s_xflag = (LdsFlag)(s_xchg + kWavesPerBlock * kXchgWaveFloats);
+  if constexpr (XCHG) {
+    if (P.span_exchange && threadIdx.x < kWavesPerBlock) s_xflag[threadIdx.x] = 0;
+  }
   __syncthreads();
 
   uint32_t mo[UC];
@@ -212,19 +226,31 @@
   float *pb_m = s_pb + pb_pos(256 - j);
 
   const Dft16K dk;
-  PhaseTimer<12> PH;
-  const int tile_stride = __builtin_amdgcn_readfirstlane((int)gridDim.x) * kWavesPerBlock;
+  PhaseTimer<14> PH;
+  const int tile_stride = DELTA ? 1 : __builtin_amdgcn_readfirstlane((int)gridDim.x) * kWavesPerBlock;
   int tile = blockIdx.x * kWavesPerBlock + wave;
-  const int n_tiles = DELTA ? P.n_ftiles : P.n_tiles;
+  int n_tiles = P.n_tiles;
+  if constexpr (DELTA) {
+    if (tile >= P.n_fspans) return;
+    typedef const __attribute__((address_space(4))) int32_t *ConstI32Ptr;
+    const ConstI32Ptr first = (ConstI32Ptr)(uintptr_t)P.fspan_first;
+    n_tiles = first[tile + 1];
+    tile = first[tile];
+  }
   if (tile >= n_tiles) return;
-  typedef typename std::conditional<DELTA, FTileRec, TileRec>::type Rec;
+  typedef typename std::conditional<DELTA, FPieceRec, TileRec>::type Rec;
   typedef const __attribute__((address_space(4))) Rec *ConstRecPtr;
-  const ConstRecPtr recs = DELTA ? (ConstRecPtr)(uintptr_t)P.ftile_rec : (ConstRecPtr)(uintptr_t)P.tile_rec;
+  const ConstRecPtr recs = DELTA ? (ConstRecPtr)(uintptr_t)P.fpiece_rec : (ConstRecPtr)(uintptr_t)P.tile_rec;
   int64_t cur_samp0 = recs[tile].samp0, cur_row0 = recs[tile].row0;
   int cur_n = recs[tile].n_frames;
   int cur_live = 0, cur_e0 = 0, cur_e1 = 0, cur_lo = 0, cur_don = 0;
+  int cur_virt = 0, cur_real = cur_n, cur_pub = 0;
   if constexpr (DELTA) {
     cur_live = recs[tile].live_n; cur_e0 = recs[tile].e0; cur_e1 = recs[tile].e1; cur_lo = recs[tile].lo; cur_don = recs[tile].delta_on;
+    if constexpr (XCHG) {
+      cur_virt = recs[tile].virt; cur_pub = P.span_exchange ? recs[tile].publish : 0;
+      cur_real = cur_virt == 1 ? cur_n - 4 : cur_n;
+    }
   }
   bool has_next = tile + tile_stride < n_tiles;
   int64_t nxt_samp0 = cur_samp0;
@@ -237,7 +263,7 @@
   float pend_val = 0.0f;
   bool pend_live = false;
   float s_prev = 0.0f, d_cur = 0.0f;
-  int b_tp = 0, b_lo = 0, b_live = 0, b_e0 = 0, b_e1 = 0, b_don = 0;
+  int b_tp = 0, b_lo = 0, b_live = 0, b_e0 = 0, b_e1 = 0, b_don = 0, b_pub = 0;
   const auto from_group = [&](int grp, float v) {
     return __int_as_float(__builtin_amdgcn_ds_bpermute(4 * ((grp << 4) | j), __float_as_int(v)));
   };
@@ -276,9 +302,21 @@
                   fetch(fdd + 2, hi1, btp - 2, dn, dp)) / norm;
     drow = from_group((g + 2) & 3, g >= 2 ? dp : dn);
   };
+  const auto publish = [&](float s_cur) {
+    if (XCHG && b_pub && b_tp < 8) {
+      wave_lds_fence();
+      s_xchg[wave * kXchgWaveFloats + (b_tp >> 2) * 64 + lane] = s_cur;
+      wave_lds_fence();
+      if (b_tp == 4) s_xflag[wave] = 1;
+      wave_lds_fence();
+    }
+  };
 
   for (;;) {
     const bool live = tp + g < (DELTA ? cur_live : cur_n);
+    const bool virt_now = XCHG && tp >= cur_real;
+    int ntp = tp + 4;
+    const unsigned long long ph_t0 = PH.stamp();
     PH(0);
     if constexpr (!DELTA) {
       if (pend_row != nullptr && pend_live) {
@@ -325,6 +363,10 @@
         }
       }
     }
+    if constexpr (XCHG) {
+#pragma unroll
+      for (int m = 0; m < MP; ++m) asm volatile("" : "+v"(re[m]), "+v"(im[m]));
+    }
     PH(1);
     if constexpr (DELTA) {
       const bool clamped = !(b_tp - 6 >= b_lo && b_tp + 3 <= b_live - 1);
@@ -344,10 +386,12 @@
         asm volatile("" : "+v"(oo));
         *reinterpret_cast<float *>(pend_row + oo) = st_ddn;
       }
+      publish(pend_val);
       s_prev = pend_val;
       d_cur = st_dn;
     }
 
+    if (__builtin_expect(!virt_now, true)) {
     float2 *tbw = reinterpret_cast<float2 *>(wbase) + g * 16 + j;
     const float2 *tbr = reinterpret_cast<const float2 *>(wbase) + g * 16 + j * kTB2Row;
     {
@@ -433,18 +477,30 @@
     wave_lds_fence();
 
     PH(6);
-    int ntp = tp + 4;
-    const bool advance = ntp >= cur_n;
-    const bool more = !advance || has_next;
-    if (advance) ntp = 0;
-    if (more)
-      pcm_prefetch<MP, ALIGNED, TYPED>(P.pcm, P.pcm_total, (advance ? nxt_samp0 : cur_samp0) + (int64_t)ntp * P.H - P.pad_left, P.H, lane, R);
+    }
+    if constexpr (XCHG) {
+      if (cur_virt == 2 && ntp == cur_n - 8 && P.span_exchange && !P.seam_recompute) {
+        wave_lds_fence();
+        if (__builtin_amdgcn_readfirstlane(s_xflag[wave + 1]) != 0) cur_real = ntp;
+      }
+    }
+    const bool piece_done = ntp >= cur_n;
+    if (piece_done ? has_next : ntp < (XCHG ? cur_real : cur_n))
+      pcm_prefetch<MP, ALIGNED, TYPED>(P.pcm, P.pcm_total, (piece_done ? nxt_samp0 : cur_samp0 + (int64_t)ntp * P.H) - P.pad_left, P.H, lane, R);
     else if constexpr (TYPED) {
 #pragma unroll
       for (int m = 0; m < 2 * MP; ++m) R.v[m] = 0u;
     }
 
     PH(7);
+    if (__builtin_expect(virt_now, false)) {
+      pend_val = 0.0f;
+      if (cur_virt == 2) {
+        wave_lds_fence();
+        pend_val = s_xchg[(wave + 1) * kXchgWaveFloats + ((tp - cur_real) >> 2) * 64 + lane];
+        wave_lds_fence();
+      }
+    } else {
     {
       float a0 = 0.0f, a1 = 0.0f;
 #pragma unroll
@@ -499,17 +555,28 @@
       }
       pend_val = acc * dgain;
     }
+    }
     pend_live = live && j < P.n_mfcc;
     pend_row = reinterpret_cast<unsigned char *>(P.out + (cur_row0 + tp - (DELTA ? 4 : 0)) * P.ld_out);
-    if constexpr (DELTA) { b_tp = tp; b_lo = cur_lo; b_live = cur_live; b_e0 = cur_e0; b_e1 = cur_e1; b_don = cur_don; }
+    if constexpr (DELTA) { b_tp = tp; b_lo = cur_lo; b_live = cur_live; b_e0 = cur_e0; b_e1 = cur_e1; b_don = cur_don; b_pub = cur_pub; }
     wave_lds_fence();
     PH(10);
-    if (!more) break;
+    if (virt_now) { PH.since(11, ph_t0); PH.count(12); }
+    else PH.count(13);
+    const bool advance = ntp >= cur_n;
+    if (advance && !has_next) break;
     if (advance) {
+      ntp = 0;
       tile += tile_stride;
       cur_samp0 = nxt_samp0; cur_row0 = recs[tile].row0; cur_n = recs[tile].n_frames;
       if constexpr (DELTA) {
         cur_live = recs[tile].live_n; cur_e0 = recs[tile].e0; cur_e1 = recs[tile].e1; cur_lo = recs[tile].lo; cur_don = recs[tile].delta_on;
+        if constexpr (XCHG) {
+          cur_virt = recs[tile].virt; cur_pub = P.span_exchange ? recs[tile].publish : 0;
+          cur_real = cur_virt == 1 ? cur_n - 4 : cur_n;
+        } else {
+          cur_real = cur_n;
+        }
       }
       has_next = tile + tile_stride < n_tiles;
       if (has_next) nxt_samp0 = recs[tile + tile_stride].samp0;
@@ -708,12 +775,16 @@
 }
 
 template <int MP, bool PREEMPH, bool USE_POWER, bool ALIGNED, bool PLP, int UC, bool DELTA = false>
-static hipError_t launch_mfcc512_one(bool padded, unsigned grid, size_t lds, hipStream_t s, const LldParams &P, const Fast512Tables &F) {
+static hipError_t launch_mfcc512_one(bool padded, unsigned grid, size_t lds, hipStream_t s, const LldParams &P, const Fast512Tables &F,
+                                     int *blocks_per_cu) {
   if constexpr (PREEMPH) {
     if (padded) {
       hipError_t e = hipFuncSetAttribute(reinterpret_cast<const void *>(&lld_mfcc512_padded<MP, PREEMPH, USE_POWER, ALIGNED, PLP, UC, DELTA>),
                                          hipFuncAttributeMaxDynamicSharedMemorySize, (int)lds);
       if (e != hipSuccess) return e;
+      if (blocks_per_cu)
+        return hipOccupancyMaxActiveBlocksPerMultiprocessor(blocks_per_cu, reinterpret_cast<const void *>(&lld_mfcc512_padded<MP, PREEMPH, USE_POWER, ALIGNED, PLP, UC, DELTA>),
+                                                            kWavesPerBlock * 64, lds);
       SMILEHIP_KLAUNCH((lld_mfcc512_padded<MP, PREEMPH, USE_POWER, ALIGNED, PLP, UC, DELTA>), dim3(grid), dim3(kWavesPerBlock * 64), lds, s, P, F);
       return hipSuccess;
     }
@@ -721,24 +792,30 @@
   hipError_t e = hipFuncSetAttribute(reinterpret_cast<const void *>(&lld_mfcc512<MP, PREEMPH, USE_POWER, ALIGNED, PLP, UC, DELTA>),
                                      hipFuncAttributeMaxDynamicSharedMemorySize, (int)lds);
   if (e != hipSuccess) return e;
+  if (blocks_per_cu)
+    return hipOccupancyMaxActiveBlocksPerMultiprocessor(blocks_per_cu, reinterpret_cast<const void *>(&lld_mfcc512<MP, PREEMPH, USE_POWER, ALIGNED, PLP, UC, DELTA>),
+                                                        kWavesPerBlock * 64, lds);
   SMILEHIP_KLAUNCH((lld_mfcc512<MP, PREEMPH, USE_POWER, ALIGNED, PLP, UC, DELTA>), dim3(grid), dim3(kWavesPerBlock * 64), lds, s, P, F);
   return hipSuccess;
 }
 
-hipError_t launch_mfcc512(const LldParams &P, const Fast512Tables &F, const Fast512Host &h, bool aligned, bool fused_delta, hipStream_t s) {
+hipError_t launch_mfcc512(const LldParams &P, const Fast512Tables &F, const Fast512Host &h, bool aligned, bool fused_delta, hipStream_t s,
+                          int *blocks_per_cu) {
   const int shared_floats = 256 * 2 + h.mp * 16 * 2 + 256 * 2 + h.mel_units * 16 * 8 + 16 * 28 + 48;
-  const size_t lds = sizeof(float) * (size_t(shared_floats) + size_t(kWavesPerBlock) * kWaveFloats);
-  if (fused_delta && (!aligned || !P.ftile_rec || P.n_ftiles <= 0)) return hipErrorInvalidValue;
-  unsigned grid = (unsigned)(((fused_delta ? P.n_ftiles : P.n_tiles) + kWavesPerBlock - 1) / kWavesPerBlock);
+  const size_t lds = sizeof(float) * (size_t(shared_floats) + size_t(kWavesPerBlock) * kWaveFloats + (fused_delta && P.span_exchange ? kXchgFloats : 0));
+  if (fused_delta && !blocks_per_cu && (!aligned || !P.fpiece_rec || !P.fspan_first || P.n_fspans <= 0))
+    return hipErrorInvalidValue;
+  unsigned grid = (unsigned)(((fused_delta ? P.n_fspans : P.n_tiles) + kWavesPerBlock - 1) / kWavesPerBlock);
+  if (fused_delta && !blocks_per_cu && grid > (unsigned)h.max_blocks) return hipErrorInvalidValue;
   if (grid > (unsigned)h.max_blocks) grid = (unsigned)h.max_blocks;
 #ifdef SMILEHIP_DEBUG_KNOBS
-  if (const char *e = getenv("SMILEHIP_DEBUG_GRID")) grid = (unsigned)atoi(e);
+  if (const char *e = getenv("SMILEHIP_DEBUG_GRID")) if (!fused_delta) grid = (unsigned)atoi(e);
 #endif
   bool launched = false;
   const bool padded = P.pad_left != 0 || h.force_padded;
 #define SMILEHIP_LAUNCH(...)                                                                                    \
   {                                                                                                             \
-    hipError_t e = launch_mfcc512_one<__VA_ARGS__>(padded, grid, lds, s, P, F);                                 \
+    hipError_t e = launch_mfcc512_one<__VA_ARGS__>(padded, grid, lds, s, P, F, blocks_per_cu);                  \
     if (e != hipSuccess) return e;                                                                              \
     launched = true;                                                                                            \
   }
@@ -771,4 +848,20 @@
   return hipGetLastError();
 }
 
-}
+bool mfcc512_exchange_fits(const Fast512Host &h, bool preemph, bool use_power, bool plp, int pad_left) {
+  LldParams P;
+  std::memset(&P, 0, sizeof(P));
+  P.preemph = preemph; P.use_power = use_power; P.plp = plp; P.pad_left = pad_left;
+  P.span_exchange = 1;
+  const bool built = plp ? (preemph ? seam_exchange<true, true>() : seam_exchange<false, true>())
+                         : (preemph ? seam_exchange<true, false>() : seam_exchange<false, false>());
+  if (!built) return false;
+  int per_cu = 0;
+  if (launch_mfcc512(P, Fast512Tables(), h, true, true, nullptr, &per_cu) != hipSuccess) {
+    (void)hipGetLastError();
+    return false;
+  }
+  return per_cu >= 2;
+}
+
+}
diff --git a/opensmile_amd/csrc/lld_params.hpp b/opensmile_amd/csrc/lld_params.hpp
--- a/opensmile_amd/csrc/lld_params.hpp
+++ b/opensmile_amd/csrc/lld_params.hpp
@@ -23,8 +23,11 @@
   const TileRec *tile_rec;
   int32_t n_utt;
   int32_t n_tiles;
-  const FTileRec *ftile_rec;
-  int32_t n_ftiles;
+  const FPieceRec *fpiece_rec;
+  const int32_t *fspan_first;
+  int32_t n_fspans;
+  int32_t span_exchange;
+  int32_t seam_recompute;
   int64_t total_frames;
   float *out;
   int64_t ld_out;
diff --git a/opensmile_amd/csrc/lld_tile_rec.hpp b/opensmile_amd/csrc/lld_tile_rec.hpp
--- a/opensmile_amd/csrc/lld_tile_rec.hpp
+++ b/opensmile_amd/csrc/lld_tile_rec.hpp
@@ -20,4 +20,16 @@
   int32_t delta_on;
 };
 
+struct FPieceRec {
+  int64_t samp0;
+  int64_t row0;
+  int32_t n_frames;
+  int32_t live_n;
+  int32_t e0, e1;
+  int32_t lo;
+  int32_t delta_on;
+  int32_t virt;
+  int32_t publish;
+};
+
 }
diff --git a/opensmile_amd/csrc/phase_timing.hpp b/opensmile_amd/csrc/phase_timing.hpp
--- a/opensmile_amd/csrc/phase_timing.hpp
+++ b/opensmile_amd/csrc/phase_timing.hpp
@@ -24,6 +24,8 @@
     last = t;
   }
   __device__ __forceinline__ void count(int i) { acc[i] += 1; }
+  __device__ __forceinline__ unsigned long long stamp() const { return last; }
+  __device__ __forceinline__ void since(int i, unsigned long long t0) { acc[i] += last - t0; }
   __device__ __forceinline__ void flush(unsigned long long *counters, int first = 0) {
     if ((threadIdx.x & 63) == 0)
       for (int i = 0; i < N; ++i) atomicAdd(&counters[first + i], acc[i]);
@@ -36,6 +38,8 @@
 struct PhaseTimer {
   __device__ __forceinline__ void operator()(int) {}
   __device__ __forceinline__ void count(int) {}
+  __device__ __forceinline__ unsigned long long stamp() const { return 0; }
+  __device__ __forceinline__ void since(int, unsigned long long) {}
   __device__ __forceinline__ void flush(unsigned long long *, int = 0) {}
 };
 __device__ __forceinline__ void phase_wait_vm() {}
diff --git a/opensmile_amd/csrc/smilehip_batch.cpp b/opensmile_amd/csrc/smilehip_batch.cpp
--- a/opensmile_amd/csrc/smilehip_batch.cpp
+++ b/opensmile_amd/csrc/smilehip_batch.cpp
@@ -16,6 +16,10 @@
   s.fused_delta_eligible = plan->use_fast && mfcc_like(plan) && c.n_delta == 2 && c.delta_win == 2 && !c.append_log_energy && !c.cms &&
                            !getenv("SMILEHIP_NO_FUSED_DELTA");
   s.fast_slots = std::max<int64_t>(1, plan->fast.max_blocks) * 8;
+  s.spans = false;
+  if (const char *e = getenv("SMILEHIP_MFCC512_SPANS")) s.spans = e[0] != '0';
+  s.span_exchange = plan->fast.span_exchange;
+  if (const char *e = getenv("SMILEHIP_MFCC512_SPAN_SLOTS")) { const long v = atol(e); if (v >= 1 && v <= (long)s.fast_slots) s.span_slots = v; }
   s.tile_frames = plan->use_fast ? fast512_tile_frames() : (c.chain_kind == SMILEHIP_CHAIN_COMPARE_F0 ? f0_tile_frames() : (int64_t(1) << 40));
   s.dtile_rows = chain_tile_rows(); s.short_T = chain_short_max(); s.jitter_chunk = jitter_chunk_frames();
   if (const char *rf = getenv("SMILEHIP_RUN_FRAMES")) { const int v = atoi(rf); if (v >= 1 && v <= 4096) s.run_frames_override = v; }
@@ -26,7 +30,14 @@
 
 static int alloc_mfcc_scratch(const smilehip_plan *plan, smilehip_batch *b, const BatchLayout &L) {
   b->n_ftiles = (int32_t)L.ftiles.size();
-  if (b->n_ftiles) return b->d_ftile_rec.upload(L.ftiles);
+  if (b->n_ftiles) {
+    b->n_fspans = (int32_t)L.fspan_first.size() - 1;
+    b->span_exchange = L.fspans_balanced;
+    const char *e = getenv("SMILEHIP_MFCC512_SEAM_RECOMPUTE");
+    b->seam_recompute = e && e[0] != '0';
+    if (int rc = b->d_fpiece_rec.upload(L.fpieces)) return rc;
+    return b->d_fspan_first.upload(L.fspan_first);
+  }
   if (plan->cfg.n_delta > 0 && b->total_frames > 0 && b->d_static.alloc(size_t(b->total_frames) * size_t(plan_n_static(plan))))
     return fail(SMILEHIP_ERR_HIP, "hipMalloc of the static-block scratch failed");
   return SMILEHIP_OK;
@@ -155,6 +166,7 @@
 extern "C" int64_t smilehip_batch_total_frames(const smilehip_batch *b) { return b ? b->total_frames : 0; }
 extern "C" int64_t smilehip_batch_total_rows(const smilehip_batch *b) { return b ? b->total_rows : 0; }
 extern "C" int smilehip_batch_delta_fused(const smilehip_batch *b) { return b && b->n_ftiles > 0 ? 1 : 0; }
+extern "C" int smilehip_batch_span_schedule(const smilehip_batch *b) { return b && b->n_ftiles > 0 && b->span_exchange ? 1 : 0; }
 extern "C" int smilehip_batch_frame_offsets(const smilehip_batch *b, int64_t *o) {
   if (!b || !o) return fail(SMILEHIP_ERR_INVALID, "smilehip_batch_frame_offsets: null argument");
   std::memcpy(o, b->h_row_off.data(), b->h_row_off.size() * sizeof(int64_t));
@@ -181,8 +193,11 @@
   P.tile_utt = b->d_tile_utt.p;
   P.tile_t0 = b->d_tile_t0.p;
   P.tile_rec = b->d_tile_rec.p;
-  P.ftile_rec = b->d_ftile_rec.p;
-  P.n_ftiles = b->n_ftiles;
+  P.fpiece_rec = b->d_fpiece_rec.p;
+  P.fspan_first = b->d_fspan_first.p;
+  P.n_fspans = b->n_fspans;
+  P.span_exchange = b->span_exchange;
+  P.seam_recompute = b->seam_recompute;
   P.n_utt = b->n_utt;
   P.n_tiles = b->n_tiles;
   P.total_frames = b->total_frames;
diff --git a/opensmile_amd/csrc/smilehip_internal.hpp b/opensmile_amd/csrc/smilehip_internal.hpp
--- a/opensmile_amd/csrc/smilehip_internal.hpp
+++ b/opensmile_amd/csrc/smilehip_internal.hpp
@@ -224,8 +224,12 @@
   DevBuf<int32_t> d_frame_utt;
   DevBuf<int32_t> d_tile_utt, d_tile_t0, d_short, d_dtile_utt, d_dtile_t0;
   DevBuf<TileRec> d_tile_rec;
-  DevBuf<FTileRec> d_ftile_rec;
   int32_t n_ftiles = 0;
+  DevBuf<FPieceRec> d_fpiece_rec;
+  DevBuf<int32_t> d_fspan_first;
+  int32_t n_fspans = 0;
+  bool span_exchange = false;
+  bool seam_recompute = false;
   int32_t n_tiles = 0, n_dtiles = 0;
   bool all_even = true;
 };
diff --git a/opensmile_amd/csrc/smilehip_plan.cpp b/opensmile_amd/csrc/smilehip_plan.cpp
--- a/opensmile_amd/csrc/smilehip_plan.cpp
+++ b/opensmile_amd/csrc/smilehip_plan.cpp
@@ -246,6 +246,9 @@
       std::copy(p->h_plp_cos.begin(), p->h_plp_cos.end(), p->fast.dct28.begin());
     }
     if (p->ctx) p->fast.max_blocks = 2 * p->ctx->prop.multiProcessorCount;
+    if (p->ctx && p->use_fast)
+      p->fast.span_exchange = mfcc512_exchange_fits(p->fast, p->cfg.preemph != 0, p->cfg.use_power != 0, is_plp,
+                                                    p->cfg.zero_pad_symmetric ? (int)((p->geo.Nfft - p->geo.N) / 2) : 0);
   }
   if (!upload) return SMILEHIP_OK;
   if ((rc = p->d_window.upload(p->h_window))) return rc;
```
